# loli/medpy

Hardware: NVIDIA H100
Metric: Mvoxels/sec to min-cut (higher is better)
Workload: dtype f64

## Files before the change

### include/medpy_b200_graphcut.h

```cpp
#ifndef MEDPY_B200_GRAPHCUT_H
#define MEDPY_B200_GRAPHCUT_H

#include <stddef.h>
#include <stdint.h>

#ifdef __cplusplus
extern "C" {
#endif

#define MGC_ABI_VERSION 3
#define MGC_MAX_NDIM 4

#define MGC_OK 0
#define MGC_E_ARG (-1)
#define MGC_E_CUDA (-2)
#define MGC_E_NOMEM (-3)
#define MGC_E_STATE (-4)
#define MGC_E_WEIGHT (-5)
#define MGC_E_NOCONV (-6)
#define MGC_E_LABELS (-7)

#define MGC_F32 0
#define MGC_F64 1
#define MGC_U8 2
#define MGC_I16 3
#define MGC_I32 4

#define MGC_MEM_HOST 0
#define MGC_MEM_DEVICE 1

#define MGC_BOUNDARY_DIFFERENCE_LINEAR 0
#define MGC_BOUNDARY_DIFFERENCE_EXPONENTIAL 1
#define MGC_BOUNDARY_DIFFERENCE_DIVISION 2
#define MGC_BOUNDARY_DIFFERENCE_POWER 3
#define MGC_BOUNDARY_MAXIMUM_LINEAR 4
#define MGC_BOUNDARY_MAXIMUM_EXPONENTIAL 5
#define MGC_BOUNDARY_MAXIMUM_DIVISION 6
#define MGC_BOUNDARY_MAXIMUM_POWER 7

#define MGC_SOURCE 0
#define MGC_SINK 1

typedef struct mgc_graph mgc_graph;

typedef struct mgc_array {
    const void* data;
    int32_t dtype;
    int32_t mem;
    int64_t strides[MGC_MAX_NDIM];
} mgc_array;

typedef struct mgc_stats {
    int64_t n_voxels;
    int64_t push_sweeps;
    int64_t global_relabels;
    int64_t relabel_sweeps;
    int64_t kernel_launches;
    int64_t active_last;
    double ms_terms;
    double ms_solve;
    double ms_readout;
    double flow_const;
    double energy;
    int64_t device_bytes;
    double ms_push;
    double ms_relabel;
    double ms_boundary;
    double ms_init;
    int64_t tiles_materialised;
    double ms_caps;
    int64_t seed_folds;
    double ms_seeds;
    double ms_seeds_host;
    int64_t tiles_deferred;
    int64_t tiles_dropped;
    int64_t relabel_passes;
    double ms_relabel_first;
    int64_t relabel_passes_first;
    int64_t build_blocks_refused;
} mgc_stats;


int mgc_create(int32_t ndim, const int64_t* shape, int32_t device, mgc_graph** out);
int mgc_create_slab(int32_t ndim, const int64_t* shape, int64_t z0, int64_t z1, int32_t device, mgc_graph** out);
void mgc_destroy(mgc_graph* g);
int mgc_reset(mgc_graph* g);
const char* mgc_last_error(const mgc_graph* g);
int mgc_abi_version(void);
int mgc_host_alloc(size_t bytes, void** out);
void mgc_host_free(void* p);
int mgc_trim_pools(void);
#define MGC_OPT_DEFER_WEIGHT_CHECK 1
#define MGC_OPT_WARM 2
#define MGC_OPT_KEEP_DEVICE_INPUTS 3
int mgc_set_option(mgc_graph* g, int32_t option, int64_t value);
int mgc_check(mgc_graph* g);
int mgc_set_stream(mgc_graph* g, void* cuda_stream);
int mgc_synchronize(mgc_graph* g);


int mgc_add_regional_probability(mgc_graph* g, const mgc_array* prob, double alpha, int32_t compute_dtype);
int mgc_add_tweights_dense(mgc_graph* g, const mgc_array* src, const mgc_array* snk);
int mgc_add_markers(mgc_graph* g, const mgc_array* fg, const mgc_array* bg);


int mgc_add_boundary(mgc_graph* g, int32_t kind, const mgc_array* image, double sigma,
                     const double* spacing, double norm);
int mgc_add_nweights_dense(mgc_graph* g, int32_t axis, const mgc_array* fwd, const mgc_array* bwd);


typedef struct mgc_voxel_terms {
    const mgc_array* prob;
    double alpha;
    int32_t compute_dtype;
    int32_t boundary_kind;
    const mgc_array* image;
    double sigma;
    const double* spacing;
    double norm;
    const mgc_array* fg;
    const mgc_array* bg;
    const uint32_t* fg_bits;
    const uint32_t* bg_bits;
    int32_t bits_mem;
    const volatile int64_t* bits_ready_words;
} mgc_voxel_terms;
int mgc_build_voxel_graph(mgc_graph* g, const mgc_voxel_terms* terms);
int mgc_can_fuse(const mgc_graph* g);


int mgc_maxflow(mgc_graph* g, double* energy);
int mgc_add_seeds(mgc_graph* g, const int64_t* fg_ids, int64_t n_fg, const int64_t* bg_ids, int64_t n_bg, int32_t mem);
int mgc_remove_seeds(mgc_graph* g, const int64_t* fg_ids, int64_t n_fg, const int64_t* bg_ids, int64_t n_bg, int32_t mem);
int mgc_add_tweights_warm(mgc_graph* g, const int64_t* ids, const double* src, const double* snk, int64_t count, int32_t mem);
int mgc_add_nweights_warm(mgc_graph* g, const int64_t* i, const int64_t* j, const double* cap, const double* rev_cap,
                          int64_t count, int32_t mem);
int mgc_add_nweights_dense_warm(mgc_graph* g, int32_t axis, const mgc_array* fwd, const mgc_array* bwd);
int mgc_remove_nweights_warm(mgc_graph* g, const int64_t* i, const int64_t* j, const double* cap, const double* rev_cap,
                             int64_t count, int32_t mem);
int mgc_remove_nweights_dense_warm(mgc_graph* g, int32_t axis, const mgc_array* fwd, const mgc_array* bwd);
int mgc_get_mask(mgc_graph* g, uint8_t* out, int32_t mem);
int mgc_what_segment(mgc_graph* g, int64_t node, int32_t* segment);
int mgc_get_edge(mgc_graph* g, int64_t i, int64_t j, double* cap);
int mgc_get_trcap(mgc_graph* g, int64_t node, double* trcap);
int mgc_get_node_num(const mgc_graph* g, int64_t* n);
int mgc_get_arc_num(const mgc_graph* g, int64_t* n);
int mgc_get_stats(const mgc_graph* g, mgc_stats* out);


int mgc_gradient_magnitude_prewitt(int32_t ndim, const int64_t* shape, const mgc_array* image, float* out,
                                   int32_t out_mem, int32_t device);


int mgc_slab_plane_elems(const mgc_graph* g, int64_t* n);
int mgc_slab_begin(mgc_graph* g);
int mgc_slab_push(mgc_graph* g, int32_t n);
int mgc_slab_pack(mgc_graph* g, int32_t* h_lo, double* f_lo, int32_t* h_hi, double* f_hi);
int mgc_slab_unpack(mgc_graph* g, const int32_t* h_lo, const double* f_lo, const int32_t* h_hi, const double* f_hi,
                    int32_t* changed_dev);
int mgc_slab_relabel_begin(mgc_graph* g);
int mgc_slab_relabel_relax(mgc_graph* g, int32_t* changed_out);
int mgc_slab_count_active(mgc_graph* g, int64_t* active_out);
// ... 54 lines not shown
```

### medpy_b200/csrc/gc_api.cu

```cuda
#include "gc_handle.cuh"
#include "gc_api_kernels.cuh"
#include "gc_gradient.cuh"

#include <cmath>
#include <cstring>
#include <map>
#include <mutex>
#include <string>
#include <type_traits>
#include <vector>

thread_local std::string g_create_error;

namespace {
std::mutex g_pool_mu;
std::map<std::pair<int, size_t>, std::vector<void*>> g_pool;

size_t round_up(size_t b) { const size_t g = size_t(1) << 21; return (b + g - 1) / g * g; }

cudaError_t pool_alloc(int dev, size_t bytes, void** out)
{
    bytes = round_up(bytes);
    {
        std::lock_guard<std::mutex> lk(g_pool_mu);
        auto it = g_pool.find({dev, bytes});
        if (it != g_pool.end() && !it->second.empty()) {
            *out = it->second.back();
            it->second.pop_back();
            return cudaSuccess;
        }
    }
    cudaError_t e = cudaMalloc(out, bytes);
    if (e != cudaSuccess) {
        std::lock_guard<std::mutex> lk(g_pool_mu);
        for (auto& kv : g_pool) if (kv.first.first == dev) { for (void* p : kv.second) cudaFree(p); kv.second.clear(); }
        cudaGetLastError();
        e = cudaMalloc(out, bytes);
    }
    return e;
}

void pool_free(int dev, size_t bytes, void* p)
{
    if (!p) return;
    std::lock_guard<std::mutex> lk(g_pool_mu);
    g_pool[{dev, round_up(bytes)}].push_back(p);
}

std::map<size_t, std::vector<void*>> g_host_pool;
std::map<void*, size_t> g_host_live;

}

size_t dtype_size(int dt)
{
    switch (dt) {
        case MGC_F32: return 4;
        case MGC_F64: return 8;
        case MGC_U8: return 1;
        case MGC_I16: return 2;
        case MGC_I32: return 4;
        default: return 0;
    }
}

int alloc_buf(mgc_graph* g, size_t bytes, void** out)
{
    void* p = nullptr;
    cudaError_t e = pool_alloc(g->device, bytes, &p);
    if (e != cudaSuccess) {
        cudaGetLastError();
        g->err = std::string("device allocation of ") + std::to_string(bytes) + " bytes failed: " + cudaGetErrorString(e);
        return MGC_E_NOMEM;
    }
    g->owned_bufs.push_back({p, bytes});
    g->device_bytes += (int64_t)round_up(bytes);
    *out = p;
    return MGC_OK;
}

int ensure_scratch(mgc_graph* g, Buf& b, size_t bytes)
{
    if (b.bytes >= bytes) return MGC_OK;
    if (b.p) {
        if (g->stream) cudaStreamSynchronize(g->stream);
        if (g->up_stream) cudaStreamSynchronize(g->up_stream);
        pool_free(g->device, b.bytes, b.p);
        g->device_bytes -= (int64_t)round_up(b.bytes);
    }
    b.p = nullptr; b.bytes = 0;
    void* p = nullptr;
    cudaError_t e = pool_alloc(g->device, bytes, &p);
    if (e != cudaSuccess) { cudaGetLastError(); g->err = "scratch allocation failed"; return MGC_E_NOMEM; }
    b.p = p; b.bytes = bytes;
    g->device_bytes += (int64_t)round_up(bytes);
    return MGC_OK;
}

namespace {
template <typename E>
int gather_launch(mgc_graph* g, const char* src, const Strides4& st, E* dst)
{
    const int Z = g->L.dim[0], Y = g->L.dim[1], X = g->L.dim[2];
    if (g->nd == 3 && Z > 1 && X > 1 && Y <= 65535 && (Z + 31) / 32 <= 65535 &&
        st.s[0] == (long long)sizeof(E) && (Y == 1 || st.s[1] == (long long)sizeof(E) * Z) && st.s[2] == (long long)sizeof(E) * Z * Y) {
        const dim3 grid((unsigned)((X + 31) / 32), (unsigned)Y, (unsigned)((Z + 31) / 32));
        k_gather_fortran3<E><<<grid, 256, 0, g->stream>>>(Z, Y, X, reinterpret_cast<const E*>(src), dst);
        g->st.kernel_launches++;
        return MGC_OK;
    }
    if (g->nd == 3) k_gather<E, 3><<<nblocks(g), 256, 0, g->stream>>>(g->L, src, st, dst);
    else            k_gather<E, 4><<<nblocks(g), 256, 0, g->stream>>>(g->L, src, st, dst);
    g->st.kernel_launches++;
    return MGC_OK;
}
}

int upload(mgc_graph* g, void* dst, const void* src, size_t bytes, int slot)
{
    if (g->slot_used[slot]) CK(cudaStreamWaitEvent(g->up_stream, g->ev_slot[slot], 0));
    CK(cudaMemcpyAsync(dst, src, bytes, cudaMemcpyHostToDevice, g->up_stream));
    CK(cudaEventRecord(g->ev_up, g->up_stream));
    CK(cudaStreamWaitEvent(g->stream, g->ev_up, 0));
    CK(cudaEventSynchronize(g->ev_up));
    return MGC_OK;
}

void slots_release(mgc_graph* g, unsigned mask)
{
    for (int i = 0; i < 5; ++i)
        if (mask & (1u << i)) { cudaEventRecord(g->ev_slot[i], g->stream); g->slot_used[i] = true; }
}

int stage_input(mgc_graph* g, const mgc_array* a, int slot, const void** out)
{
    const size_t es = dtype_size(a->dtype);
    if (!es) FAIL(MGC_E_ARG, "unsupported dtype");
    if (!a->data) FAIL(MGC_E_ARG, "null array");
    Strides4 st{};
    bool contiguous = true;
    long long span = (long long)es;
    long long expect = (long long)es;
    for (int d = g->nd - 1; d >= 0; --d) {
        long long s = 0;
        int ud = d - g->shift;
        if (ud >= 0) s = (long long)a->strides[ud];
        if (g->L.dim[d] > 1) {
            if (s <= 0) FAIL(MGC_E_ARG, "array strides must be positive (pass a contiguous copy)");
            if (s != expect) contiguous = false;
            span += (long long)(g->L.dim[d] - 1) * s;
        } else {
            s = 0;
        }
        st.s[d] = s;
        expect *= g->L.dim[d];
    }
    const size_t bytes = (size_t)g->L.n * es;
    if (contiguous && a->mem == MGC_MEM_DEVICE) { *out = a->data; return MGC_OK; }
    int rc = ensure_scratch(g, g->scratch[slot], bytes);
    if (rc) return rc;
    if (contiguous) {
        rc = upload(g, g->scratch[slot].p, a->data, bytes, slot);
        if (rc) return rc;
        *out = g->scratch[slot].p;
        return MGC_OK;
    }
    const char* src = (const char*)a->data;
    if (a->mem == MGC_MEM_HOST) {
        rc = ensure_scratch(g, g->raw, (size_t)span);
        if (rc) return rc;
        rc = upload(g, g->raw.p, a->data, (size_t)span, 3);
        if (rc) return rc;
        src = (const char*)g->raw.p;
    }
    else if (g->slot_used[slot]) CK(cudaStreamWaitEvent(g->stream, g->ev_slot[slot], 0));
    switch (a->dtype) {
        case MGC_F32: gather_launch<float>(g, src, st, (float*)g->scratch[slot].p); break;
        case MGC_F64: gather_launch<double>(g, src, st, (double*)g->scratch[slot].p); break;
        case MGC_U8: gather_launch<uint8_t>(g, src, st, (uint8_t*)g->scratch[slot].p); break;
        case MGC_I16: gather_launch<int16_t>(g, src, st, (int16_t*)g->scratch[slot].p); break;
        case MGC_I32: gather_launch<int32_t>(g, src, st, (int32_t*)g->scratch[slot].p); break;
    }
    CK(cudaGetLastError());
    if (a->mem == MGC_MEM_HOST) { CK(cudaEventRecord(g->ev_slot[3], g->stream)); g->slot_used[3] = true; }
    *out = g->scratch[slot].p;
    return MGC_OK;
}

void sum_partials(mgc_graph* g, const double* partials, unsigned n, double* out)
{
    k_sum_partials<<<1, 256, 0, g->stream>>>(partials, n, out);
}

namespace {
int finish_flow_const(mgc_graph* g)
{
    sum_partials(g, g->partials, rblocks(g), g->d_scalars);
    g->st.kernel_launches++;
    CK(cudaGetLastError());
    return MGC_OK;
}

void invalidate(mgc_graph* g)
{
    g->lazy_built = false;
    g->caps_img = nullptr;
    g->caps_tin.prob = nullptr;
    g->state_init = false;
    g->warm_state = false;
    g->solved = false;
    g->host_mask_valid = false;
}
}

void resolve_term_span(mgc_graph* g)
{
    if (!g->terms_open) return;
    if (cudaEventSynchronize(g->ev_terms[1]) == cudaSuccess) {
        float ms = 0;
        if (cudaEventElapsedTime(&ms, g->ev_terms[0], g->ev_terms[1]) == cudaSuccess) g->st.ms_terms += ms;
        if (g->boundary_timed && cudaEventElapsedTime(&ms, g->ev_b[0], g->ev_b[1]) == cudaSuccess) g->st.ms_boundary = ms;
        g->boundary_timed = false;
    }
    g->terms_open = false;
}

int check_pending(mgc_graph* g)
{
    if (!g->bad_pending) return MGC_OK;
    g->bad_pending = false;
    CK(cudaEventSynchronize(g->ev_bad));
    if (*g->h_bad) FAIL(MGC_E_WEIGHT, "Negative or zero weights are not allowed.");
    return MGC_OK;
}

namespace {
int create_impl(int32_t ndim, const int64_t* shape, int64_t z0, int64_t z1, bool slab, int32_t device, mgc_graph** out)
{
    if (!out) return MGC_E_ARG;
    *out = nullptr;
    if (ndim < 1 || ndim > MGC_MAX_NDIM || !shape) { g_create_error = "ndim must be 1..4"; return MGC_E_ARG; }
    int ndev = 0;
    cudaError_t e = cudaGetDeviceCount(&ndev);
    if (e != cudaSuccess || ndev == 0) {
        cudaGetLastError();
        g_create_error = std::string("no usable CUDA device (this library has no CPU path): ") + cudaGetErrorString(e);
        return MGC_E_CUDA;
    }
    if (device < 0) cudaGetDevice(&device);
    if (device >= ndev) { g_create_error = "bad device ordinal"; return MGC_E_ARG; }
    e = cudaSetDevice(device);
    if (e != cudaSuccess) { g_create_error = cudaGetErrorString(e); return MGC_E_CUDA; }

    mgc_graph* g = new mgc_graph();
    g->device = device;
    g->user_ndim = ndim;
    g->nd = ndim == 4 ? 4 : 3;
    g->shift = g->nd - ndim;
    for (int d = 0; d < ndim; ++d) {
        if (shape[d] < 1) { g_create_error = "extents must be >= 1"; delete g; return MGC_E_ARG; }
        g->user_shape[d] = shape[d];
    }
    int64_t dims[4] = {1, 1, 1, 1};
    for (int d = 0; d < ndim; ++d) dims[d + g->shift] = shape[d];
    g->slab = slab;
    int own0 = 0, own1 = (int)dims[0];
    if (slab) {
        if (g->shift != 0 || z0 < 0 || z1 > shape[0] || z0 >= z1) { g_create_error = "bad slab"; delete g; return MGC_E_ARG; }
        g->global_dim0 = shape[0]; g->z0 = z0; g->z1 = z1;
        g->ghost_lo = z0 > 0; g->ghost_hi = z1 < shape[0];
        dims[0] = (z1 - z0) + (g->ghost_lo ? 1 : 0) + (g->ghost_hi ? 1 : 0);
        own0 = g->ghost_lo ? 1 : 0;
        own1 = own0 + (int)(z1 - z0);
    }
    int64_t n = 1;
    for (int d = 0; d < g->nd; ++d) n *= dims[d];
    if (n >= (int64_t(1) << 31)) { g_create_error = "lattice too large for one device handle (>= 2^31 voxels)"; delete g; return MGC_E_ARG; }
    g->L.nd = g->nd;
    unsigned s = (unsigned)n;
    for (int d = 0; d < 4; ++d) { g->L.dim[d] = 1; g->L.stride[d] = 1; }
    for (int d = 0; d < g->nd; ++d) { g->L.dim[d] = (int)dims[d]; s /= (unsigned)dims[d]; g->L.stride[d] = s; }
    for (int d = 0; d < 4; ++d) {
        const unsigned long long st = g->L.stride[d];
        g->L.magic[d] = st <= 1 ? 0ull : (~0ull / st) + 1ull;
    }
    g->L.n = (unsigned)n;
    g->L.plane = g->L.stride[0];
    g->L.own0 = own0; g->L.own1 = own1;

    int rc = MGC_OK;
    const size_t nb = (size_t)n;
    void* p = nullptr;
    for (int k = 0; k < 2 * g->nd && !rc; ++k) { rc = alloc_buf(g, nb * sizeof(double), &p); g->S.cap[k] = (double*)p; }
    if (!rc) { rc = alloc_buf(g, nb * sizeof(double), &p); g->S.excess = (double*)p; }
    if (!rc) { rc = alloc_buf(g, nb * sizeof(double), &p); g->S.sink = (double*)p; }
    if (!rc) { rc = alloc_buf(g, nb * sizeof(double), &p); g->S.tr = (double*)p; }
    if (!rc) { rc = alloc_buf(g, nb * sizeof(int), &p); g->S.height = (int*)p; }
    if (!rc) { rc = alloc_buf(g, nb, &p); g->S.rmask = (uint8_t*)p; }
    if (!rc) { rc = alloc_buf(g, nb, &p); g->mask_dev = (uint8_t*)p; }
    g->n_partials = nblocks(g);
    if (g->nd == 3) {
        const unsigned nbuild = (unsigned)((g->L.dim[0] + 7) / 8) * (unsigned)((g->L.dim[1] + 7) / 8) * (unsigned)((g->L.dim[2] + 31) / 32);
        if (nbuild > g->n_partials) g->n_partials = nbuild;
        if (!rc) { rc = alloc_buf(g, (size_t)nbuild * sizeof(int), &p); g->build_refused = (int*)p; }
    }
    if (!rc) { rc = alloc_buf(g, (size_t)g->n_partials * sizeof(double), &p); g->partials = (double*)p; }
    if (!rc) { rc = alloc_buf(g, 3 * 1024 * sizeof(double), &p); g->minmax_buf = p; }
    if (!rc) { rc = alloc_buf(g, 64, &p); g->d_scalars = (double*)p; }
    if (!rc) { rc = alloc_buf(g, 64, &p); g->d_flags = (int*)p; }
    if (!rc) { rc = alloc_buf(g, 64, &p); g->d_count = (unsigned long long*)p; }
    if (!rc && g->nd == 3) {
        for (int d = 0; d < 3; ++d) g->TL.nt[d] = (g->L.dim[d] + TILE - 1) / TILE;
        g->TL.ntiles = g->TL.nt[0] * g->TL.nt[1] * g->TL.nt[2];
        const size_t tb = (size_t)g->TL.ntiles * sizeof(int);
// ... 45 lines not shown
    for (auto& ev : g->ev_chunk) cudaEventCreateWithFlags(&ev, cudaEventDisableTiming);
    for (auto& ev : g->ev_terms) cudaEventCreate(&ev);
    if (const char* f0 = getenv("MEDPY_GC_DEBUG")) g->debug_checks = atoi(f0) != 0;
    if (const char* f3 = getenv("MEDPY_GC_FIRST_TEST")) g->skip_first_test = atoi(f3) == 0;
    if (const char* f5 = getenv("MEDPY_GC_FIRST_CAP")) g->first_cap = atoi(f5) >= 2 ? atoi(f5) : 0;
    if (const char* f1 = getenv("MEDPY_GC_FUSE")) g->fuse_build = atoi(f1) != 0;
    if (const char* f4 = getenv("MEDPY_GC_LAZY_CAPS")) g->lazy_caps = atoi(f4) != 0;
    if (const char* f2 = getenv("MEDPY_GC_CHUNKS")) if (atoi(f2) > 0) g->build_chunks = atoi(f2);
    cudaEventCreateWithFlags(&g->ev_bad, cudaEventDisableTiming);
    for (auto& ev : g->ev_b) cudaEventCreate(&ev);
    { void* hp = nullptr; g->h_bad = (mgc_host_alloc(64, &hp) == MGC_OK) ? (int*)hp : nullptr; }
    g->st.n_voxels = (int64_t)n;
    rc = mgc_reset(g);
    if (rc) { g_create_error = g->err; mgc_destroy(g); return rc; }
    *out = g;
    return MGC_OK;
}

template <typename E, int ND, bool FRESH>
void boundary_launch_nd(mgc_graph* g, const E* img, const BoundaryParams& P)
{
    const dim3 grid(nblocks(g)), block(256);
    if (P.fn == 1 && P.inv_spacing_on == 0.0 && (sizeof(E) == 4 || sizeof(E) == 8) && !std::is_integral<E>::value) {
        if (P.use_max) k_boundary<E, ND, double, FRESH, 1, 1, 0><<<grid, block, 0, g->stream>>>(g->L, g->S, img, P, g->d_flags);
        else           k_boundary<E, ND, double, FRESH, 1, 0, 0><<<grid, block, 0, g->stream>>>(g->L, g->S, img, P, g->d_flags);
        return;
    }
    k_boundary<E, ND, double, FRESH><<<grid, block, 0, g->stream>>>(g->L, g->S, img, P, g->d_flags);
}

template <typename E>
int boundary_launch(mgc_graph* g, const E* img, const BoundaryParams& P)
{
    if (g->caps_fresh) {
        if (g->nd == 3) boundary_launch_nd<E, 3, true>(g, img, P);
        else            boundary_launch_nd<E, 4, true>(g, img, P);
    } else {
        if (g->nd == 3) boundary_launch_nd<E, 3, false>(g, img, P);
        else            boundary_launch_nd<E, 4, false>(g, img, P);
    }
    g->caps_fresh = false;
    g->st.kernel_launches++;
    return MGC_OK;
}

template <typename E>
int minmax_launch(mgc_graph* g, const E* img)
{
    unsigned nb = g->n_partials < 1024u ? g->n_partials : 1024u;
    E* pm = (E*)g->minmax_buf;
    E* px = pm + 1024;
    E* pa = px + 1024;
    k_minmax_partial<E><<<nb, 256, 0, g->stream>>>(img, g->L.n, pm, px, pa);
    k_minmax_final<E><<<1, 32, 0, g->stream>>>(pm, px, pa, nb, g->d_scalars + 2);
    g->st.kernel_launches += 2;
    return MGC_OK;
}
}

int boundary_params(mgc_graph* g, int kind, int dtype, const void* img, double sigma, const double* spacing, double norm, BoundaryParams* out)
{
    BoundaryParams P{};
    P.fn = kind & 3;
    P.use_max = (kind >= 4 && kind != MGC_BOUNDARY_MAXIMUM_DIVISION) ? 1 : 0;
    P.sigma = (P.fn == 1) ? pow(sigma, 2) : sigma;
    P.inv_sigma2 = (P.fn == 1 && P.sigma != 0.0) ? 1.0 / P.sigma : 0.0;
    P.inv_spacing_on = spacing ? 1.0 : 0.0;
    for (int d = 0; d < 4; ++d) P.spacing[d] = 1.0;
    if (spacing) for (int d = 0; d < g->user_ndim; ++d) P.spacing[d + g->shift] = spacing[d];
    P.norm = norm;
    if (P.fn == 0 && std::isnan(norm)) {
        if (g->slab) FAIL(MGC_E_ARG, "z-slab handles need the global normaliser of the linear terms");
        int rc = MGC_OK;
        switch (dtype) {
            case MGC_F32: rc = minmax_launch<float>(g, (const float*)img); break;
            case MGC_F64: rc = minmax_launch<double>(g, (const double*)img); break;
            case MGC_U8: rc = minmax_launch<uint8_t>(g, (const uint8_t*)img); break;
            case MGC_I16: rc = minmax_launch<int16_t>(g, (const int16_t*)img); break;
            case MGC_I32: rc = minmax_launch<int32_t>(g, (const int32_t*)img); break;
        }
        if (rc) return rc;
        double mm[2];
        CK(cudaMemcpyAsync(mm, g->d_scalars + 2, sizeof(mm), cudaMemcpyDeviceToHost, g->stream));
        CK(cudaStreamSynchronize(g->stream));
        P.norm = (kind == MGC_BOUNDARY_MAXIMUM_LINEAR) ? mm[1] : mm[0];
    }
    *out = P;
    return MGC_OK;
}

template <typename E, int ND>
static cudaError_t gradient_launch(const int64_t* shape, const E* img, float* out, long long n)
{
    GradCtx<ND> G;
    long long st = 1;
    for (int d = ND - 1; d >= 0; --d) { G.dim[d] = (int)shape[d]; G.stride[d] = st; st *= shape[d]; }
    k_gradient_magnitude<E, ND><<<(unsigned)((n + 255) / 256), 256>>>(G, n, img, out);
    return cudaGetLastError();
}

template <typename E>
static cudaError_t gradient_dispatch(int nd, const int64_t* shape, const E* img, float* out, long long n)
{
    switch (nd) {
        case 1: return gradient_launch<E, 1>(shape, img, out, n);
        case 2: return gradient_launch<E, 2>(shape, img, out, n);
        case 3: return gradient_launch<E, 3>(shape, img, out, n);
        default: return gradient_launch<E, 4>(shape, img, out, n);
    }
}

extern "C" {

int mgc_abi_version(void) { return MGC_ABI_VERSION; }

const char* mgc_last_error(const mgc_graph* g) { return g ? g->err.c_str() : g_create_error.c_str(); }

int mgc_create(int32_t ndim, const int64_t* shape, int32_t device, mgc_graph** out)
{
    return create_impl(ndim, shape, 0, 0, false, device, out);
}

int mgc_create_slab(int32_t ndim, const int64_t* shape, int64_t z0, int64_t z1, int32_t device, mgc_graph** out)
{
    if (ndim < 3) { g_create_error = "z-slab handles need ndim >= 3"; return MGC_E_ARG; }
    return create_impl(ndim, shape, z0, z1, true, device, out);
}

void mgc_destroy(mgc_graph* g)
{
    if (!g) return;
    cudaSetDevice(g->device);
    if (g->stream) cudaStreamSynchronize(g->stream);
    for (auto& b : g->owned_bufs) pool_free(g->device, b.bytes, b.p);
    for (auto& b : g->scratch) if (b.p) pool_free(g->device, b.bytes, b.p);
    if (g->raw.p) pool_free(g->device, g->raw.bytes, g->raw.p);
    if (g->img_copy.p) pool_free(g->device, g->img_copy.bytes, g->img_copy.p);
    if (g->prob_copy.p) pool_free(g->device, g->prob_copy.bytes, g->prob_copy.p);
    for (auto& b : g->mark_planes) if (b.p) pool_free(g->device, b.bytes, b.p);
    if (g->fold_buf.p) pool_free(g->device, g->fold_buf.bytes, g->fold_buf.p);
    for (auto& ev : g->ev_fold) if (ev) cudaEventDestroy(ev);
    for (auto& ev : g->ev) if (ev) cudaEventDestroy(ev);
    for (auto& ev : g->caps_ev) if (ev) cudaEventDestroy(ev);
    for (auto& ev : g->ev_slot) if (ev) cudaEventDestroy(ev);
    for (auto& ev : g->ev_terms) if (ev) cudaEventDestroy(ev);
    for (auto& ev : g->ev_chunk) if (ev) cudaEventDestroy(ev);
    if (g->ev_up) cudaEventDestroy(g->ev_up);
    if (g->ev_bad) cudaEventDestroy(g->ev_bad);
    for (auto& ev : g->ev_b) if (ev) cudaEventDestroy(ev);
    for (auto& ev : g->ph_events) if (ev) cudaEventDestroy(ev);
    if (g->h_bad) mgc_host_free(g->h_bad);
    if (g->h_stat) mgc_host_free(g->h_stat);
    slab_comm_release(g);
    if (g->up_stream) { cudaStreamSynchronize(g->up_stream); cudaStreamDestroy(g->up_stream); }
    if (g->own_stream && g->stream) cudaStreamDestroy(g->stream);
    delete g;
}

int mgc_reset(mgc_graph* g)
{
    if (!g) return MGC_E_ARG;
    CK(cudaSetDevice(g->device));
    g->caps_fresh = true;
    g->tr_fresh = true;
    g->caps_lazy = false;
    CK(cudaMemsetAsync(g->d_scalars, 0, 64, g->stream));
    CK(cudaMemsetAsync(g->d_flags, 0, 64, g->stream));
    invalidate(g);
    g->flow_started = false;
    g->has_nlinks = false;
    g->energy = 0.0;
    int64_t n = g->st.n_voxels;
    g->st = mgc_stats{};
    g->st.n_voxels = n;
    g->terms_open = false;
    g->bad_pending = false;
    return MGC_OK;
}

int mgc_gradient_magnitude_prewitt(int32_t ndim, const int64_t* shape, const mgc_array* image, float* out,
                                   int32_t out_mem, int32_t device)
{
    if (ndim < 1 || ndim > 4 || !shape || !image || !image->data || !out) { g_create_error = "bad arguments"; return MGC_E_ARG; }
    const size_t es = dtype_size(image->dtype);
    if (!es) { g_create_error = "unsupported dtype"; return MGC_E_ARG; }
    int ndev = 0;
    if (cudaGetDeviceCount(&ndev) != cudaSuccess || ndev == 0) {
        cudaGetLastError();
        g_create_error = "no usable CUDA device (this library has no CPU path)";
        return MGC_E_CUDA;
    }
    if (device < 0) cudaGetDevice(&device);
    cudaSetDevice(device);
    long long n = 1;
    bool contiguous = true;
    long long expect = (long long)es;
    for (int d = ndim - 1; d >= 0; --d) {
        if (shape[d] < 1) { g_create_error = "extents must be >= 1"; return MGC_E_ARG; }
        if (shape[d] > 1 && image->strides[d] != expect) contiguous = false;
        expect *= shape[d];
        n *= shape[d];
    }
    if (!contiguous) { g_create_error = "gradient input must be C-contiguous (the host layer copies otherwise)"; return MGC_E_ARG; }
    void* d_in = nullptr;
    void* d_out = nullptr;
    const size_t in_bytes = (size_t)n * es, out_bytes = (size_t)n * sizeof(float);
    cudaError_t e = cudaSuccess;
    if (image->mem == MGC_MEM_HOST) {
        if ((e = pool_alloc(device, in_bytes, &d_in)) != cudaSuccess) { cudaGetLastError(); g_create_error = "device allocation failed"; return MGC_E_NOMEM; }
        e = cudaMemcpy(d_in, image->data, in_bytes, cudaMemcpyHostToDevice);
    }
    const void* src = image->mem == MGC_MEM_HOST ? d_in : image->data;
    float* dst = out;
    if (e == cudaSuccess && out_mem == MGC_MEM_HOST) {
        if ((e = pool_alloc(device, out_bytes, &d_out)) == cudaSuccess) dst = (float*)d_out;
    }
    if (e == cudaSuccess) {
        switch (image->dtype) {
            case MGC_F32: e = gradient_dispatch<float>(ndim, shape, (const float*)src, dst, n); break;
            case MGC_F64: e = gradient_dispatch<double>(ndim, shape, (const double*)src, dst, n); break;
            case MGC_U8: e = gradient_dispatch<uint8_t>(ndim, shape, (const uint8_t*)src, dst, n); break;
            case MGC_I16: e = gradient_dispatch<int16_t>(ndim, shape, (const int16_t*)src, dst, n); break;
            default: e = gradient_dispatch<int32_t>(ndim, shape, (const int32_t*)src, dst, n); break;
        }
    }
    if (e == cudaSuccess && out_mem == MGC_MEM_HOST) e = cudaMemcpy(out, d_out, out_bytes, cudaMemcpyDeviceToHost);
    if (e == cudaSuccess) e = cudaDeviceSynchronize();
    if (d_in) pool_free(device, in_bytes, d_in);
    if (d_out) pool_free(device, out_bytes, d_out);
    if (e != cudaSuccess) { cudaGetLastError(); g_create_error = std::string("gradient kernel failed: ") + cudaGetErrorString(e); return MGC_E_CUDA; }
    return MGC_OK;
}

int mgc_host_alloc(size_t bytes, void** out)
{
    if (!out || !bytes) return MGC_E_ARG;
    const size_t rb = round_up(bytes);
    std::lock_guard<std::mutex> lk(g_pool_mu);
    auto it = g_host_pool.find(rb);
    void* p = nullptr;
    if (it != g_host_pool.end() && !it->second.empty()) { p = it->second.back(); it->second.pop_back(); }
    else if (cudaHostAlloc(&p, rb, cudaHostAllocDefault) != cudaSuccess) { cudaGetLastError(); g_create_error = "pinned host allocation failed"; return MGC_E_NOMEM; }
    g_host_live[p] = rb;
    *out = p;
    return MGC_OK;
}

void mgc_host_free(void* p)
{
    if (!p) return;
    std::lock_guard<std::mutex> lk(g_pool_mu);
    auto it = g_host_live.find(p);
    if (it == g_host_live.end()) return;
    g_host_pool[it->second].push_back(p);
    g_host_live.erase(it);
}

int mgc_trim_pools(void)
{
    std::lock_guard<std::mutex> lk(g_pool_mu);
    int cur = 0;
    cudaGetDevice(&cur);
    for (auto& kv : g_pool) {
        if (kv.second.empty()) continue;
        cudaSetDevice(kv.first.first);
        for (void* p : kv.second) cudaFree(p);
        kv.second.clear();
    }
    cudaSetDevice(cur);
    for (auto& kv : g_host_pool) { for (void* p : kv.second) cudaFreeHost(p); kv.second.clear(); }
    cudaGetLastError();
    return MGC_OK;
}

int mgc_set_option(mgc_graph* g, int32_t option, int64_t value)
{
    if (!g) return MGC_E_ARG;
    if (option == MGC_OPT_DEFER_WEIGHT_CHECK) { g->defer_check = value != 0; return MGC_OK; }
    if (option == MGC_OPT_KEEP_DEVICE_INPUTS) { g->keep_device_inputs = value != 0; return MGC_OK; }
    if (option == MGC_OPT_WARM) {
        const bool on = value != 0;
        if (on != g->warm_opt && g->flow_started && !g->lazy_built)
            FAIL(MGC_E_STATE, "MGC_OPT_WARM is set before the first solve (the residual source capacities are recorded at "
                              "its start): reset() the handle and rebuild the graph to change it");
        g->warm_opt = on;
        return MGC_OK;
    }
    FAIL(MGC_E_ARG, "unknown option");
}

int mgc_check(mgc_graph* g)
{
    if (!g) return MGC_E_ARG;
    return check_pending(g);
}

int mgc_set_stream(mgc_graph* g, void* cuda_stream)
{
    if (!g) return MGC_E_ARG;
    CK(cudaStreamSynchronize(g->stream));
    if (g->own_stream) { cudaStreamDestroy(g->stream); g->own_stream = false; }
    g->stream = (cudaStream_t)cuda_stream;
    return MGC_OK;
}

int mgc_synchronize(mgc_graph* g)
{
    if (!g) return MGC_E_ARG;
    CK(cudaStreamSynchronize(g->stream));
    return MGC_OK;
}

int mgc_add_regional_probability(mgc_graph* g, const mgc_array* prob, double alpha, int32_t compute_dtype)
{
    if (!g || !prob) return MGC_E_ARG;
    if (g->flow_started) FAIL(MGC_E_STATE, "the graph has been solved (its capacities hold residuals): reset() it before adding terms");
    if (prob->dtype != MGC_F32 && prob->dtype != MGC_F64) FAIL(MGC_E_ARG, "probability map must be float32 or float64");
    if (compute_dtype != MGC_F32 && compute_dtype != MGC_F64) FAIL(MGC_E_ARG, "compute dtype must be float32 or float64");
    CK(cudaSetDevice(g->device));
    { int rc0 = push_state_all(g); if (rc0) return rc0; }
    TermSpan t(g);
    const void* p = nullptr;
    int rc = stage_input(g, prob, 0, &p);
    if (rc) return rc;
    rc = check_pending(g);
    if (rc) return rc;
    if (prob->dtype == MGC_F32 && (g->L.n % 4u) == 0u && ((uintptr_t)p % 16u) == 0u)
        k_regional_f32x4<double><<<rblocks(g), 256, 0, g->stream>>>(g->L, g->S, (const float4*)p, alpha, compute_dtype == MGC_F32, g->tr_fresh ? 1 : 0, g->partials);
    else if (prob->dtype == MGC_F32)
        k_regional<float, double><<<rblocks(g), 256, 0, g->stream>>>(g->L, g->S, (const float*)p, alpha, compute_dtype == MGC_F32, g->tr_fresh ? 1 : 0, g->partials);
    else
        k_regional<double, double><<<rblocks(g), 256, 0, g->stream>>>(g->L, g->S, (const double*)p, alpha, 0, g->tr_fresh ? 1 : 0, g->partials);
    g->tr_fresh = false;
    g->st.kernel_launches++;
    CK(cudaGetLastError());
    rc = finish_flow_const(g);
    if (rc) return rc;
    invalidate(g);
    t.stop(1u);
    return MGC_OK;
}

int mgc_add_tweights_dense(mgc_graph* g, const mgc_array* src, const mgc_array* snk)
{
    if (!g || !src || !snk) return MGC_E_ARG;
    if (g->flow_started) FAIL(MGC_E_STATE, "the graph has been solved (its capacities hold residuals): reset() it before adding terms");
    if (src->dtype != MGC_F64 || snk->dtype != MGC_F64) FAIL(MGC_E_ARG, "dense t-weights must be float64");
    CK(cudaSetDevice(g->device));
    { int rc0 = push_state_all(g); if (rc0) return rc0; }
    TermSpan t(g);
    const void *ps = nullptr, *pk = nullptr;
    int rc = stage_input(g, src, 0, &ps);
    if (rc) return rc;
    rc = stage_input(g, snk, 1, &pk);
    if (rc) return rc;
    rc = check_pending(g);
    if (rc) return rc;
    k_tweights_dense<double><<<rblocks(g), 256, 0, g->stream>>>(g->L, g->S, (const double*)ps, (const double*)pk, g->tr_fresh ? 1 : 0, g->partials);
    g->tr_fresh = false;
    g->st.kernel_launches++;
    CK(cudaGetLastError());
    rc = finish_flow_const(g);
    if (rc) return rc;
    invalidate(g);
    t.stop(3u);
    return MGC_OK;
}

int mgc_add_markers(mgc_graph* g, const mgc_array* fg, const mgc_array* bg)
{
    if (!g) return MGC_E_ARG;
    if (!fg && !bg) return MGC_OK;
    if (g->flow_started) FAIL(MGC_E_STATE, "the graph has been solved (its capacities hold residuals): reset() it before adding terms");
    if ((fg && fg->dtype != MGC_U8) || (bg && bg->dtype != MGC_U8)) FAIL(MGC_E_ARG, "markers must be uint8 / bool");
    CK(cudaSetDevice(g->device));
    { int rc0 = push_state_all(g); if (rc0) return rc0; }
    TermSpan t(g);
    const void *pf = nullptr, *pb = nullptr;
    int rc = MGC_OK;
    if (fg) { rc = stage_input(g, fg, 1, &pf); if (rc) return rc; }
    if (bg) { rc = stage_input(g, bg, 4, &pb); if (rc) return rc; }
    rc = check_pending(g);
    if (rc) return rc;
    const bool vec16 = !g->tr_fresh && (g->L.n % 16u) == 0u && ((uintptr_t)pf % 16u) == 0u && ((uintptr_t)pb % 16u) == 0u;
    if (vec16)
        k_markers16<double><<<rblocks(g), 256, 0, g->stream>>>(g->L, g->S, (const uint4*)pf, (const uint4*)pb, g->partials);
    else
        k_markers<double><<<rblocks(g), 256, 0, g->stream>>>(g->L, g->S, (const uint8_t*)pf, (const uint8_t*)pb, g->tr_fresh ? 1 : 0, g->partials);
    g->tr_fresh = false;
    g->st.kernel_launches++;
    CK(cudaGetLastError());
    rc = finish_flow_const(g);
    if (rc) return rc;
    invalidate(g);
    t.stop(0x12u);
    return MGC_OK;
}

int mgc_add_boundary(mgc_graph* g, int32_t kind, const mgc_array* image, double sigma, const double* spacing, double norm)
{
    if (!g || !image) return MGC_E_ARG;
    if (kind < 0 || kind > 7) FAIL(MGC_E_ARG, "unknown boundary term");
    if (g->flow_started) FAIL(MGC_E_STATE, "the graph has been solved (its capacities hold residuals): reset() it before adding terms");
    CK(cudaSetDevice(g->device));
    { int rc0 = check_pending(g); if (rc0) return rc0; }
    { int rc0 = push_state_all(g); if (rc0) return rc0; }
    TermSpan t(g);
    const void* img = nullptr;
    int rc = stage_input(g, image, 2, &img);
    if (rc) return rc;
    BoundaryParams P{};
    rc = boundary_params(g, kind, image->dtype, img, sigma, spacing, norm, &P);
    if (rc) return rc;
    CK(cudaMemsetAsync(g->d_flags, 0, sizeof(int), g->stream));
    cudaEventRecord(g->ev_b[0], g->stream);
    switch (image->dtype) {
        case MGC_F32: boundary_launch<float>(g, (const float*)img, P); break;
        case MGC_F64: boundary_launch<double>(g, (const double*)img, P); break;
        case MGC_U8: boundary_launch<uint8_t>(g, (const uint8_t*)img, P); break;
        case MGC_I16: boundary_launch<int16_t>(g, (const int16_t*)img, P); break;
        case MGC_I32: boundary_launch<int32_t>(g, (const int32_t*)img, P); break;
    }
    cudaEventRecord(g->ev_b[1], g->stream);
    CK(cudaGetLastError());
    invalidate(g);
    g->has_nlinks = true;
    g->boundary_timed = true;
    if (g->defer_check && g->h_bad && image->mem == MGC_MEM_HOST) {
        CK(cudaMemcpyAsync(g->h_bad, g->d_flags, sizeof(int), cudaMemcpyDeviceToHost, g->stream));
        CK(cudaEventRecord(g->ev_bad, g->stream));
        g->bad_pending = true;
        t.stop(4u);
        return MGC_OK;
    }
    int bad = 0;
    CK(cudaMemcpyAsync(&bad, g->d_flags, sizeof(int), cudaMemcpyDeviceToHost, g->stream));
    t.stop(4u);
    CK(cudaStreamSynchronize(g->stream));
    if (bad) FAIL(MGC_E_WEIGHT, "Negative or zero weights are not allowed.");
    return MGC_OK;
}

int mgc_add_nweights_dense(mgc_graph* g, int32_t axis, const mgc_array* fwd, const mgc_array* bwd)
{
    if (!g || !fwd || !bwd) return MGC_E_ARG;
    if (g->flow_started) FAIL(MGC_E_STATE, "the graph has been solved (its capacities hold residuals): reset() it before adding terms");
    if (axis < 0 || axis >= g->user_ndim) FAIL(MGC_E_ARG, "bad axis");
    if (fwd->dtype != MGC_F64 || bwd->dtype != MGC_F64) FAIL(MGC_E_ARG, "dense n-weights must be float64");
    CK(cudaSetDevice(g->device));
    { int rc0 = check_pending(g); if (rc0) return rc0; }
    { int rc0 = push_state_all(g); if (rc0) return rc0; }
    TermSpan t(g);
    const void *pf = nullptr, *pb = nullptr;
    int rc = stage_input(g, fwd, 0, &pf);
    if (rc) return rc;
    rc = stage_input(g, bwd, 1, &pb);
    if (rc) return rc;
    if (g->caps_fresh) {
        const size_t nbz = (size_t)g->L.n;
        for (int k = 0; k < 2 * g->nd; ++k) CK(cudaMemsetAsync(g->S.cap[k], 0, nbz * sizeof(double), g->stream));
        g->caps_fresh = false;
    }
    CK(cudaMemsetAsync(g->d_flags, 0, sizeof(int), g->stream));
    const int ca = axis + g->shift;
    if (g->nd == 3) k_nweights_dense<3, double><<<nblocks(g), 256, 0, g->stream>>>(g->L, g->S, ca, (const double*)pf, (const double*)pb, g->d_flags);
    else            k_nweights_dense<4, double><<<nblocks(g), 256, 0, g->stream>>>(g->L, g->S, ca, (const double*)pf, (const double*)pb, g->d_flags);
    g->st.kernel_launches++;
    CK(cudaGetLastError());
    int bad = 0;
    CK(cudaMemcpyAsync(&bad, g->d_flags, sizeof(int), cudaMemcpyDeviceToHost, g->stream));
    t.stop(3u);
    CK(cudaStreamSynchronize(g->stream));
    invalidate(g);
    g->has_nlinks = true;
    if (bad) FAIL(MGC_E_WEIGHT, "Negative or zero weights are not allowed.");
    return MGC_OK;
}

int mgc_get_mask(mgc_graph* g, uint8_t* out, int32_t mem)
{
    if (!g || !out) return MGC_E_ARG;
    if (!g->solved) FAIL(MGC_E_STATE, "call maxflow first");
    CK(cudaSetDevice(g->device));
    const size_t owned_n = (size_t)(g->L.own1 - g->L.own0) * g->L.plane;
    const uint8_t* src = g->mask_dev + (size_t)g->L.own0 * g->L.plane;
    CK(cudaMemcpyAsync(out, src, owned_n, mem == MGC_MEM_DEVICE ? cudaMemcpyDeviceToDevice : cudaMemcpyDeviceToHost, g->stream));
    CK(cudaStreamSynchronize(g->stream));
    return MGC_OK;
}

int mgc_what_segment(mgc_graph* g, int64_t node, int32_t* segment)
{
    if (!g || !segment) return MGC_E_ARG;
    if (!g->solved) FAIL(MGC_E_STATE, "call maxflow first");
    if (node < 0 || node >= (int64_t)g->L.n) FAIL(MGC_E_ARG, "node id out of range");
    if (!g->host_mask_valid) {
        g->host_mask.resize(g->L.n);
        CK(cudaMemcpyAsync(g->host_mask.data(), g->mask_dev, g->L.n, cudaMemcpyDeviceToHost, g->stream));
        CK(cudaStreamSynchronize(g->stream));
        g->host_mask_valid = true;
    }
    *segment = g->host_mask[(size_t)node] ? MGC_SOURCE : MGC_SINK;
    return MGC_OK;
}

int mgc_get_edge(mgc_graph* g, int64_t i, int64_t j, double* cap)
{
    if (!g || !cap) return MGC_E_ARG;
    const int64_t n = (int64_t)g->L.n;
    if (i < 0 || j < 0 || i >= n || j >= n || i == j) FAIL(MGC_E_ARG, "bad node ids");
    *cap = 0.0;
    if (g->caps_fresh) return MGC_OK;
    CK(cudaSetDevice(g->device));
    { int rc0 = push_state_all(g); if (rc0) return rc0; }
    int c[4] = {0, 0, 0, 0};
    unsigned r = (unsigned)i;
    for (int d = 0; d < g->nd; ++d) { c[d] = (int)(r / g->L.stride[d]); r %= g->L.stride[d]; }
    for (int k = 0; k < 2 * g->nd; ++k) {
        const int d = k >> 1;
        const int64_t off = (k & 1) ? (int64_t)g->L.stride[d] : -(int64_t)g->L.stride[d];
        const int cn = c[d] + ((k & 1) ? 1 : -1);
        if (cn < 0 || cn >= g->L.dim[d]) continue;
        if (i + off == j) {
            CK(cudaMemcpyAsync(cap, g->S.cap[k] + i, sizeof(double), cudaMemcpyDeviceToHost, g->stream));
            CK(cudaStreamSynchronize(g->stream));
            caps_resolve(g);
            return MGC_OK;
        }
    }
    return MGC_OK;
}

int mgc_get_trcap(mgc_graph* g, int64_t node, double* trcap)
{
    if (!g || !trcap) return MGC_E_ARG;
    if (node < 0 || node >= (int64_t)g->L.n) FAIL(MGC_E_ARG, "node id out of range");
    if (g->tr_fresh) { *trcap = 0.0; return MGC_OK; }
    CK(cudaSetDevice(g->device));
    { int rc0 = push_state_all(g); if (rc0) return rc0; }
    if (!g->state_init || !g->flow_started) {
        CK(cudaMemcpyAsync(trcap, g->S.tr + node, sizeof(double), cudaMemcpyDeviceToHost, g->stream));
        CK(cudaStreamSynchronize(g->stream));
        return MGC_OK;
    }
    double e = 0, s = 0;
    uint8_t rm = 0x80u;
    CK(cudaMemcpyAsync(&e, g->S.excess + node, sizeof(double), cudaMemcpyDeviceToHost, g->stream));
    CK(cudaMemcpyAsync(&s, g->S.sink + node, sizeof(double), cudaMemcpyDeviceToHost, g->stream));
    if (g->nd == 3) CK(cudaMemcpyAsync(&rm, g->S.rmask + node, 1, cudaMemcpyDeviceToHost, g->stream));
    CK(cudaStreamSynchronize(g->stream));
    if (!(rm & 0x80u)) s = 0;
    double tr = 0;
    CK(cudaMemcpyAsync(&tr, g->S.tr + node, sizeof(double), cudaMemcpyDeviceToHost, g->stream));
    CK(cudaStreamSynchronize(g->stream));
    *trcap = (tr < 0 && -tr - s > 0) ? -(-tr - s) : e;
    return MGC_OK;
}

int mgc_get_node_num(const mgc_graph* g, int64_t* n)
{
    if (!g || !n) return MGC_E_ARG;
    *n = (int64_t)g->L.n;
    return MGC_OK;
}

int mgc_get_arc_num(const mgc_graph* g, int64_t* n)
{
    if (!g || !n) return MGC_E_ARG;
    int64_t e = 0;
    if (g->has_nlinks)
        for (int d = 0; d < g->nd; ++d)
            if (g->L.dim[d] > 1) e += ((int64_t)g->L.n / g->L.dim[d]) * (g->L.dim[d] - 1);
    *n = 2 * e;
    return MGC_OK;
}

int mgc_get_stats(const mgc_graph* g, mgc_stats* out)
{
    if (!g || !out) return MGC_E_ARG;
    *out = g->st;
    out->device_bytes = g->device_bytes;
    return MGC_OK;
}

}
```

### medpy_b200/csrc/gc_build.cuh

```cuda
#pragma once
#include <climits>
#include <type_traits>
#include "gc_terms.cuh"
#include "gc_tiles.cuh"
#include "gc_tma.cuh"

#define BUILD_TZ 8
#define BUILD_TY 8
#define BUILD_TX 32
#define BUILD_THREADS 256
#define BUILD_TIN_OFFSET(img_pad) ((((img_pad) + (2 * 9 * 32 + 2 * 8 * 33 + 8 * 32 + 8 * 8) * 8 + 8 + 32 + 64) + 127) / 128 * 128)
template <typename E> struct BuildBox {
    static constexpr int PAD = 16 / (int)sizeof(E);
    static constexpr int BX = (PAD + 33 + PAD - 1) / PAD * PAD;
};
#define BUILD_HY 10
#define BUILD_HZ 10

struct BuildMaps {
    CUtensorMap img, prob, fg, bg;
};

struct BuildArgs {
    const void* img;
// ... 695 lines not shown
        const int lx = tid & 31, ly = tid >> 5;
        const bool col_in = y0 + ly < L.dim[1] && x0 + lx < L.dim[2];
        double msum = 0.0;
#pragma unroll
        for (int lz = 0; lz < BUILD_TZ; ++lz) {
            const int cz2 = z0 + lz;
            if (col_in && cz2 < L.dim[0] && cz2 >= L.own0 && cz2 < L.own1)
                msum = __dadd_rn(msum, s_mm[(lz * BUILD_TY + ly) * BUILD_TX + (lx ^ ly)]);
        }
#pragma unroll
        for (int o = 16; o > 0; o >>= 1) msum = __dadd_rn(msum, __shfl_down_sync(0xffffffffu, msum, o));
        double* s_red = reinterpret_cast<double*>(s_scr);
        if (lx == 0) s_red[ly] = msum;
        __syncthreads();
        if (tid == 0) {
            double t = s_red[0];
#pragma unroll
            for (int w = 1; w < 8; ++w) t = __dadd_rn(t, s_red[w]);
            partials[((A.z_tile0 + (int)blockIdx.z) * (int)gridDim.y + (int)blockIdx.y) * (int)gridDim.x + (int)blockIdx.x] = t;
        }
    }
    if (tid < 4) {
        const int tx = (x0 >> 3) + tid, tyy = y0 >> 3, tzz = z0 >> 3;
        if (tx < TL.nt[2] && tyy < TL.nt[1] && tzz < TL.nt[0]) {
            const int t = (tzz * TL.nt[1] + tyy) * TL.nt[2] + tx;
            const int any_needs = s_flags[tid], any_exc = s_flags[4 + tid];
            rflag[t] = any_needs;
            if (any_needs) rl.items[atomicAdd(rl.count, 1)] = t;
            pflag[t] = any_exc;
            A.cmat[t] = 0;
            if (any_exc) {
                const WorkList& pl = ((tzz + tyy + tx) & 1) ? pl1 : pl0;
                pl.items[atomicAdd(pl.count, 1)] = t;
            }
        }
    }
}

__device__ __forceinline__ unsigned tile_pairs(const Lattice& L, const TileCtx& c)
{
    const int gz = c.tz * TILE + c.lz, gy = c.ty * TILE + c.ly, gx = c.tx * TILE + c.lx;
    return (gz > 0 ? 1u : 0u) | (gz + 1 < L.dim[0] ? 2u : 0u) | (gy > 0 ? 4u : 0u) | (gy + 1 < L.dim[1] ? 8u : 0u) |
           (gx > 0 ? 16u : 0u) | (gx + 1 < L.dim[2] ? 32u : 0u);
}

__device__ __forceinline__ void lazy_tin_load(const Lattice& L, const LazyTin& tin, const TileCtx& c, double& p, unsigned& fb)
{
    const int gz = c.tz * TILE + c.lz, gy = c.ty * TILE + c.ly, gx = c.tx * TILE + c.lx;
    if (tin.prob) p = tin.prob_f64 ? reinterpret_cast<const double*>(tin.prob)[c.v] : (double)reinterpret_cast<const float*>(tin.prob)[c.v];
    const unsigned w = ((unsigned)gz * (unsigned)L.dim[1] + (unsigned)gy) * (unsigned)tin.words + ((unsigned)gx >> 5);
    if (tin.fg) fb |= (tin.fg[w] >> (gx & 31)) & 1u;
    if (tin.bg) fb |= ((tin.bg[w] >> (gx & 31)) & 1u) << 1;
}

__device__ __forceinline__ double lazy_tr(const LazyTin& tin, double p, unsigned fb)
{
    double tr = 0.0;
    tlink_replay<double>(tr, tin.prob != nullptr, p, tin.compute_f32 != 0, tin.alpha, fb);
    return tr;
}

__device__ __forceinline__ bool lazy_has_excess(const Lattice& L, const LazyTin& tin, const TileCtx& c)
{
    double p = 0.0;
    unsigned fb = 0u;
    lazy_tin_load(L, tin, c, p, fb);
    return source_active(lazy_tr(tin, p, fb), tile_pairs(L, c));
}

template <typename T>
__device__ __forceinline__ bool voxel_active(const Lattice& L, const State<T>& S, const LazyTin& tin, const TileCtx& c, int h, bool mat)
{
    if (!c.own || h >= MGC_HINF) return false;
    return mat ? S.excess[c.v] > 0 : lazy_has_excess(L, tin, c);
}

#define PUSH_WINDOW 8
#define FIRST_RELABEL_CAP 12
#define WIN_GMIN 0
#define WIN_NOW 1
#define WIN_DEFERRED 2
#define WIN_DROPPED 3
#define WIN_NDROP 4
```

### medpy_b200/csrc/gc_build_api.cu

```cuda
#include "gc_handle.cuh"

#include <atomic>
#include <cmath>
#include <cstdlib>
#include <thread>
#include <type_traits>
#include <utility>

namespace {
bool make_image_map(mgc_graph* g, const void* img, int dtype, CUtensorMap* out)
{
    tmap_encode_fn encode = tensor_map_encoder();
    if (!encode) return false;
    const size_t es = dtype_size(dtype);
    const cuuint64_t X = (cuuint64_t)g->L.dim[2], Y = (cuuint64_t)g->L.dim[1], Z = (cuuint64_t)g->L.dim[0];
    if ((X * es) % 16 || ((uintptr_t)img & 15)) return false;
    CUtensorMapDataType dt;
    switch (dtype) {
        case MGC_F32: dt = CU_TENSOR_MAP_DATA_TYPE_FLOAT32; break;
        case MGC_F64: dt = CU_TENSOR_MAP_DATA_TYPE_FLOAT64; break;
        case MGC_U8: dt = CU_TENSOR_MAP_DATA_TYPE_UINT8; break;
        case MGC_I16: dt = CU_TENSOR_MAP_DATA_TYPE_UINT16; break;
        default: dt = CU_TENSOR_MAP_DATA_TYPE_INT32; break;
    }
// ... 175 lines not shown
                   !(( t->boundary_kind & 3) == 0 && std::isnan(t->norm));
    if (t->prob) chunked = chunked && t->prob->mem == MGC_MEM_HOST && c_contiguous(g, t->prob);
    if (t->fg) chunked = chunked && t->fg->mem == MGC_MEM_HOST && c_contiguous(g, t->fg);
    if (t->bg) chunked = chunked && t->bg->mem == MGC_MEM_HOST && c_contiguous(g, t->bg);
    if (has_bits) chunked = chunked && t->bits_mem == MGC_MEM_HOST;

    const void *d_img = nullptr, *d_prob = nullptr, *d_fg = nullptr, *d_bg = nullptr;
    int rc = MGC_OK;
    if (!chunked) {
        rc = stage_input(g, t->image, 2, &d_img); if (rc) return rc;
        if (t->prob) { rc = stage_input(g, t->prob, 0, &d_prob); if (rc) return rc; }
        if (t->fg) { rc = stage_input(g, t->fg, 1, &d_fg); if (rc) return rc; }
        if (t->bg) { rc = stage_input(g, t->bg, 4, &d_bg); if (rc) return rc; }
        if (has_bits) {
            if (t->bits_ready_words && t->bits_mem == MGC_MEM_HOST) {
                while (*t->bits_ready_words < (int64_t)words) std::this_thread::yield();
                std::atomic_thread_fence(std::memory_order_acquire);
            }
            const uint32_t* src[2] = {t->fg_bits, t->bg_bits};
            const void** dst[2] = {&d_fg, &d_bg};
            const int slot[2] = {1, 4};
            for (int i = 0; i < 2; ++i) {
                if (!src[i]) continue;
                if (t->bits_mem == MGC_MEM_DEVICE) { *dst[i] = src[i]; continue; }
                rc = ensure_scratch(g, g->scratch[slot[i]], words * 4); if (rc) return rc;
                rc = upload(g, g->scratch[slot[i]].p, src[i], words * 4, slot[i]); if (rc) return rc;
                *dst[i] = g->scratch[slot[i]].p;
            }
        }
    } else {
        rc = ensure_scratch(g, g->scratch[2], n * es_img); if (rc) return rc;
        if (t->prob) { rc = ensure_scratch(g, g->scratch[0], n * es_prob); if (rc) return rc; }
        if (t->fg || t->fg_bits) { rc = ensure_scratch(g, g->scratch[1], has_bits ? words * 4 : n); if (rc) return rc; }
        if (t->bg || t->bg_bits) { rc = ensure_scratch(g, g->scratch[4], has_bits ? words * 4 : n); if (rc) return rc; }
        d_img = g->scratch[2].p;
        if (t->prob) d_prob = g->scratch[0].p;
        if (t->fg || t->fg_bits) d_fg = g->scratch[1].p;
        if (t->bg || t->bg_bits) d_bg = g->scratch[4].p;
        const int slots[4] = {0, 1, 2, 4};
        for (int i = 0; i < 4; ++i) if (g->slot_used[slots[i]]) CK(cudaStreamWaitEvent(g->up_stream, g->ev_slot[slots[i]], 0));
    }

    BoundaryParams P{};
    rc = boundary_params(g, t->boundary_kind, t->image->dtype, d_img, t->sigma, t->spacing, t->norm, &P);
    if (rc) return rc;

    BuildArgs A{};
    A.img = d_img;
    A.prob = d_prob;
    A.prob_f64 = (t->prob && t->prob->dtype == MGC_F64) ? 1 : 0;
    A.compute_f32 = (t->prob && t->compute_dtype == MGC_F32) ? 1 : 0;
    A.alpha = t->alpha;
    if (has_bits) { A.fg_bits = (const unsigned*)d_fg; A.bg_bits = (const unsigned*)d_bg; }
    else { A.fg = (const uint8_t*)d_fg; A.bg = (const uint8_t*)d_bg; }
    BuildMaps imap{};
    A.use_tma = make_image_map(g, d_img, t->image->dtype, &imap.img) ? 1 : 0;
    if (const char* e = getenv("MEDPY_GC_BUILD_TMA")) if (atoi(e) == 0) A.use_tma = 0;
    int tin_tma = A.use_tma;
    if (const char* e = getenv("MEDPY_GC_BUILD_TMA")) if (atoi(e) == 2) tin_tma = 0;
    if (tin_tma) {
        if (d_prob && make_block_map(g, d_prob, t->prob->dtype, &imap.prob)) A.tma_prob = 1;
        if (!has_bits) {
            if (d_fg && make_block_map(g, d_fg, MGC_U8, &imap.fg)) A.tma_mark |= 1;
            if (d_bg && make_block_map(g, d_bg, MGC_U8, &imap.bg)) A.tma_mark |= 2;
        }
    }
    if (const char* e = getenv("MEDPY_GC_BUILD_DBG")) A.dbg = atoi(e);
    const bool lazy = can_lazy(g);
    const int mark_words = (g->L.dim[2] + 31) / 32;
    enum { COPIED, STAGED, BORROWED };
    auto source_of = [&](const mgc_array* a, const void* d, int slot) {
        if (d == g->scratch[slot].p) return STAGED;
        return (g->keep_device_inputs && a->mem == MGC_MEM_DEVICE && d == a->data) ? BORROWED : COPIED;
    };
    const int img_src = lazy ? source_of(t->image, d_img, 2) : COPIED;
    const int prob_src = (lazy && t->prob && !(A.dbg & 1)) ? source_of(t->prob, d_prob, 0) : COPIED;
    if (lazy) {
        if (img_src == COPIED) { rc = ensure_scratch(g, g->img_copy, n * es_img); if (rc) return rc; A.img_copy = g->img_copy.p; }
        if (t->prob && prob_src == COPIED) { rc = ensure_scratch(g, g->prob_copy, n * es_prob); if (rc) return rc; A.prob_copy = g->prob_copy.p; }
        const size_t plane_bytes = (size_t)g->L.dim[0] * (size_t)g->L.dim[1] * (size_t)mark_words * 4;
        if (t->fg || t->fg_bits) { rc = ensure_scratch(g, g->mark_planes[0], plane_bytes); if (rc) return rc; A.fg_plane = (unsigned*)g->mark_planes[0].p; }
        if (t->bg || t->bg_bits) { rc = ensure_scratch(g, g->mark_planes[1], plane_bytes); if (rc) return rc; A.bg_plane = (unsigned*)g->mark_planes[1].p; }
        A.cmat = g->cmat;
        CK(cudaMemsetAsync(g->d_flags + 3, 0, sizeof(int), g->stream));
        CK(cudaMemsetAsync(g->win_ctl + WIN_NDROP, 0, sizeof(int), g->stream));
    }

    CK(cudaMemsetAsync(g->d_tcount, 0, 256, g->stream));
    CK(cudaMemsetAsync(g->d_flags, 0, sizeof(int), g->stream));
    CK(cudaMemsetAsync(g->d_flags + 7, 0, sizeof(int), g->stream));
    { int rcd = dirty_clear(g); if (rcd) return rcd; }
    g->pl_sel[0] = g->pl_sel[1] = 0;
    cudaEventRecord(g->ev_b[0], g->stream);
    if (!chunked) {
        A.z_tile0 = 0;
        rc = build_launch_any(g, lazy, t->image->dtype, imap, A, P, nzt);
        if (rc) return rc;
    } else {
        int nchunks = g->build_chunks < nzt ? g->build_chunks : nzt;
        const int per = (nzt + nchunks - 1) / nchunks;
        nchunks = (nzt + per - 1) / per;
        const char* h_img = (const char*)t->image->data;
        int prev_l0 = 0, prev_nl = 0;
        for (int c = 0; c < nchunks; ++c) {
            const int l0 = c * per, l1 = (l0 + per < nzt) ? l0 + per : nzt;
            const size_t z0 = (size_t)l0 * BUILD_TZ, z1 = ((size_t)l1 * BUILD_TZ < (size_t)Z) ? (size_t)l1 * BUILD_TZ : (size_t)Z;
            const size_t v0 = z0 * plane, nv = (z1 - z0) * plane;
            CK(cudaMemcpyAsync((char*)g->scratch[2].p + v0 * es_img, h_img + v0 * es_img, nv * es_img, cudaMemcpyHostToDevice, g->up_stream));
            if (c > 0) {
                CK(cudaEventRecord(g->ev_chunk[c & 1], g->up_stream));
                CK(cudaStreamWaitEvent(g->stream, g->ev_chunk[c & 1], 0));
                A.z_tile0 = prev_l0;
                rc = build_launch_any(g, lazy, t->image->dtype, imap, A, P, prev_nl);
                if (rc) { cudaStreamSynchronize(g->up_stream); return rc; }
            }
            if (t->prob) CK(cudaMemcpyAsync((char*)g->scratch[0].p + v0 * es_prob, (const char*)t->prob->data + v0 * es_prob, nv * es_prob, cudaMemcpyHostToDevice, g->up_stream));
            if (has_bits) {
                const size_t w0 = v0 / 32, w1 = (v0 + nv + 31) / 32;
                if (t->bits_ready_words) {
                    const int64_t need = (int64_t)(w1 < words ? w1 : words);
                    while (*t->bits_ready_words < need) std::this_thread::yield();
                    std::atomic_thread_fence(std::memory_order_acquire);
                }
                if (t->fg_bits) CK(cudaMemcpyAsync((uint32_t*)g->scratch[1].p + w0, t->fg_bits + w0, (w1 - w0) * 4, cudaMemcpyHostToDevice, g->up_stream));
                if (t->bg_bits) CK(cudaMemcpyAsync((uint32_t*)g->scratch[4].p + w0, t->bg_bits + w0, (w1 - w0) * 4, cudaMemcpyHostToDevice, g->up_stream));
            } else {
                if (t->fg) CK(cudaMemcpyAsync((char*)g->scratch[1].p + v0, (const char*)t->fg->data + v0, nv, cudaMemcpyHostToDevice, g->up_stream));
                if (t->bg) CK(cudaMemcpyAsync((char*)g->scratch[4].p + v0, (const char*)t->bg->data + v0, nv, cudaMemcpyHostToDevice, g->up_stream));
            }
            prev_l0 = l0; prev_nl = l1 - l0;
        }
        CK(cudaEventRecord(g->ev_up, g->up_stream));
        CK(cudaStreamWaitEvent(g->stream, g->ev_up, 0));
        A.z_tile0 = prev_l0;
        rc = build_launch_any(g, lazy, t->image->dtype, imap, A, P, prev_nl);
        if (rc) { cudaStreamSynchronize(g->up_stream); return rc; }
        CK(cudaEventSynchronize(g->ev_up));
    }
    cudaEventRecord(g->ev_b[1], g->stream);
    {
        const unsigned nbuild = (unsigned)nzt * (unsigned)((g->L.dim[1] + BUILD_TY - 1) / BUILD_TY) * (unsigned)((g->L.dim[2] + BUILD_TX - 1) / BUILD_TX);
        sum_partials(g, g->partials, nbuild, g->d_scalars);
        g->st.kernel_launches++;
        CK(cudaGetLastError());
    }
    g->caps_fresh = false;
    g->tr_fresh = false;
    g->caps_lazy = lazy;
    g->lazy_built = lazy;
    g->warm_state = false;
    g->st.seed_folds = 0;
    g->st.ms_seeds = 0.0;
    g->st.ms_seeds_host = 0.0;
    g->caps_dtype = t->image->dtype;
    g->caps_P = P;
    if (img_src == STAGED) std::swap(g->scratch[2], g->img_copy);
    if (prob_src == STAGED) std::swap(g->scratch[0], g->prob_copy);
    g->caps_img = !lazy ? nullptr : (img_src == BORROWED ? d_img : g->img_copy.p);
    const void* caps_prob = !(lazy && t->prob) ? nullptr : (prob_src == BORROWED ? d_prob : g->prob_copy.p);
    g->caps_tin = LazyTin{caps_prob, A.prob_f64, A.compute_f32, A.alpha, A.fg_plane, A.bg_plane, mark_words};
    g->has_nlinks = true;
    g->boundary_timed = true;
    g->state_init = true;
    g->solved = false;
    g->host_mask_valid = false;
    g->labels_fresh = true;
    g->sweep_mode = -1;
    g->init_timed = false;
    g->st.ms_init = 0.0;
    span.stop(0x17u);
    if (g->defer_check && g->h_bad) {
        CK(cudaMemcpyAsync(g->h_bad, g->d_flags, sizeof(int), cudaMemcpyDeviceToHost, g->stream));
        CK(cudaEventRecord(g->ev_bad, g->stream));
        g->bad_pending = true;
        return MGC_OK;
    }
    int bad = 0;
    CK(cudaMemcpyAsync(&bad, g->d_flags, sizeof(int), cudaMemcpyDeviceToHost, g->stream));
    CK(cudaStreamSynchronize(g->stream));
    if (bad) FAIL(MGC_E_WEIGHT, "Negative or zero weights are not allowed.");
    return MGC_OK;
}

}
```

### medpy_b200/csrc/gc_fold.cu

```cuda
#include "gc_handle.cuh"
#include "gc_nlinks_remove.cuh"

#include <cub/cub.cuh>

#include <algorithm>
#include <chrono>
#include <functional>
#include <map>
#include <mutex>
#include <tuple>
#include <type_traits>
#include <vector>

int warm_prepare(mgc_graph* g)
{
    if (!warm_wanted(g) || g->warm_state) return MGC_OK;
    if (g->flow_started) FAIL(MGC_E_STATE, "MGC_OPT_WARM was set after the first solve: reset() the graph and rebuild it");
    if (!g->state_init || g->nd == 4) {
        int rc = materialise_zeros(g);
        if (rc) return rc;
        return init_tiles(g);
    }
    Nvtx range("mgc:warm_convert");
    unsigned grid = nblocks(g);
// ... 37 lines not shown
    if (sort == FOLD_SORT_PAIRS) e = cub::DeviceRadixSort::SortPairs(tmp, tb, keys, skeys, vals, svals, n, 0, end_bit, s);
    if (!tmp && sort != FOLD_SCAN) *bytes = tb;
    return e;
}

static cudaError_t fold_scan(void* tmp, size_t* bytes, int* head, int* pos, int n, cudaStream_t s)
{
    size_t tb = *bytes;
    const cudaError_t e = cub::DeviceScan::InclusiveSum(tmp, tb, head, pos, n, s);
    if (!tmp) *bytes = std::max(*bytes, tb);
    return e;
}

static int cub_launches(mgc_graph* g, const std::tuple<int, int, int, int, int>& key,
                        const std::function<cudaError_t(cudaStream_t)>& enqueue, int* out)
{
    static std::mutex mu;
    static std::map<int, cudaStream_t> streams;
    static std::map<std::tuple<int, int, int, int, int>, int> counts;
    std::lock_guard<std::mutex> lock(mu);
    auto it = counts.find(key);
    if (it != counts.end()) { *out = it->second; return MGC_OK; }
    cudaStream_t& s = streams[g->device];
    if (!s) CK(cudaStreamCreateWithFlags(&s, cudaStreamNonBlocking));
    cudaGraph_t graph = nullptr;
    cudaError_t e = cudaStreamBeginCapture(s, cudaStreamCaptureModeRelaxed);
    if (e == cudaSuccess) {
        const cudaError_t e2 = enqueue(s);
        e = cudaStreamEndCapture(s, &graph);
        if (e == cudaSuccess) e = e2;
    }
    size_t nn = 0;
    std::vector<cudaGraphNode_t> nodes;
    if (e == cudaSuccess) e = cudaGraphGetNodes(graph, nullptr, &nn);
    if (e == cudaSuccess) { nodes.resize(nn); e = cudaGraphGetNodes(graph, nodes.data(), &nn); }
    int k = 0;
    for (size_t i = 0; e == cudaSuccess && i < nn; ++i) {
        cudaGraphNodeType t;
        e = cudaGraphNodeGetType(nodes[i], &t);
        if (e == cudaSuccess && t == cudaGraphNodeTypeKernel) ++k;
    }
    if (graph) cudaGraphDestroy(graph);
    CK(e);
    if (counts.size() > 4096) counts.clear();
    counts[key] = k;
    *out = k;
    return MGC_OK;
}

template <typename Key>
static int fold_cub_launches(mgc_graph* g, int sort, int n, int end_bit, void* tmp, size_t tmp_bytes, Key* keys, Key* skeys,
                             int* vals, int* svals, int* head, int* pos, int* out)
{
    return cub_launches(g, std::make_tuple(g->device, sort, (int)sizeof(Key), n, end_bit), [&](cudaStream_t s) {
        size_t tb = tmp_bytes;
        const cudaError_t e1 = fold_sort(sort, tmp, &tb, keys, skeys, vals, svals, n, end_bit, s);
        tb = tmp_bytes;
        return e1 == cudaSuccess ? fold_scan(tmp, &tb, head, pos, n, s) : e1;
    }, out);
}

static cudaError_t tails_sort(void* tmp, size_t* bytes, const unsigned* tails, unsigned* stails, int count, int end_bit,
                              cudaStream_t s)
{
    return cub::DeviceRadixSort::SortKeys(tmp, *bytes, tails, stails, count, 0, end_bit, s);
}

static int warm_check(mgc_graph* g, bool* eager)
{
    *eager = false;
    if (!g->slab && g->lazy_built && g->state_init && g->nd == 3) return MGC_OK;
    if (warm_wanted(g)) { *eager = true; return MGC_OK; }
    FAIL(MGC_E_STATE, "a warm re-solve needs a lazily built 3-D handle (mgc_build_voxel_graph on a 1-D..3-D lattice with a "
                      "boundary term, tile solver, lazy capacities); on this handle reset() it and rebuild the graph with "
                      "the seeds instead");
}

static int fold_items(mgc_graph* g, int* d_ctl, int* tiles, const std::function<int(unsigned, int)>& fold,
                      const char* nonfinite, const char* negative, const std::function<int()>* check)
{
    CK(cudaEventRecord(g->ev_fold[1], g->stream));
    int h_ctl[2] = {0, 0};
    CK(cudaMemcpyAsync(h_ctl, d_ctl, sizeof(h_ctl), cudaMemcpyDeviceToHost, g->stream));
    CK(cudaStreamSynchronize(g->stream));
    if (h_ctl[1] & FOLD_ERR_RANGE) FAIL(MGC_E_ARG, "node id out of range");
    if (h_ctl[1] & FOLD_ERR_PAIR) FAIL(MGC_E_ARG, "node ids are not lattice neighbours");
    if (h_ctl[1] & FOLD_ERR_NONFINITE) FAIL(MGC_E_ARG, nonfinite);
    if (h_ctl[1] & FOLD_ERR_NEGATIVE) FAIL(MGC_E_WEIGHT, negative);
    const int ni = h_ctl[0];
    if (ni == 0) return MGC_OK;
    const bool eager = !g->lazy_built;
    if (eager) {
        int rc = warm_prepare(g);
        if (rc) return rc;
    }
    if (check) {
        int rc = (*check)();
        if (rc) return rc;
        int bits = 0;
        CK(cudaMemcpyAsync(&bits, d_ctl + 1, sizeof(int), cudaMemcpyDeviceToHost, g->stream));
        CK(cudaStreamSynchronize(g->stream));
        if (bits & FOLD_ERR_PAIRSUM)
            FAIL(MGC_E_WEIGHT, "an n-link decrement exceeds what its arc pair holds: r(i->j) + r(j->i), which equals "
                               "c(i->j) + c(j->i), is below cap + rev_cap");
    }
    CK(cudaEventRecord(g->ev_fold[2], g->stream));
    if (g->caps_lazy) {
        int rc;
        for (int color = 0; color < 2; ++color) { rc = caps_launch(g, pl(g, color, g->pl_sel[color])); if (rc) return rc; }
        rc = caps_launch(g, WorkList{g->drop_items, g->win_ctl + WIN_NDROP});
        if (rc) return rc;
        CK(cudaMemsetAsync(g->win_ctl + WIN_NDROP, 0, sizeof(int), g->stream));
        rc = caps_launch(g, WorkList{tiles, d_ctl + 2});
        if (rc) return rc;
    }
    unsigned grid = (unsigned)((ni + 255) / 256);
    if (grid > REDUCE_BLOCKS) grid = REDUCE_BLOCKS;
    { int rc = fold(grid, ni); if (rc) return rc; }
    sum_partials(g, g->partials, grid, g->d_scalars);
    CK(cudaMemsetAsync(g->d_tcount, 0, 256, g->stream));
    CK(cudaMemsetAsync(g->pflag, 0, (size_t)g->TL.ntiles * sizeof(int), g->stream));
    g->pl_sel[0] = g->pl_sel[1] = 0;
    {
        unsigned lgrid = (unsigned)g->n_ctas * 4u;
        if (lgrid > (unsigned)g->TL.ntiles) lgrid = (unsigned)g->TL.ntiles;
        if (g->nd == 4) k_seed_lists4<<<lgrid, T4_VOX, 0, g->stream>>>(g->L, g->TL4, g->S, g->pflag, pl(g, 0, 0), pl(g, 1, 0));
        else k_seed_lists<<<lgrid, TILE_VOX, 0, g->stream>>>(g->L, g->TL, g->S, eager ? nullptr : g->cmat, g->pflag,
                                                             pl(g, 0, 0), pl(g, 1, 0));
    }
    g->st.kernel_launches += 3;
    CK(cudaGetLastError());
    CK(cudaEventRecord(g->ev_fold[3], g->stream));
    CK(cudaEventSynchronize(g->ev_fold[3]));
    {
        float ms0 = 0, ms1 = 0;
        if (cudaEventElapsedTime(&ms0, g->ev_fold[0], g->ev_fold[1]) == cudaSuccess &&
            cudaEventElapsedTime(&ms1, g->ev_fold[2], g->ev_fold[3]) == cudaSuccess)
            g->st.ms_seeds += ms0 + ms1;
        g->st.ms_caps -= caps_resolve(g);
    }
    g->labels_fresh = false;
    g->sweep_mode = -1;
    g->solved = false;
    g->host_mask_valid = false;
    g->st.seed_folds++;
    return MGC_OK;
}

struct FoldCall {
    const char* range;
    const char* bad;
    const char* too_many;
    const char* negative;
    int64_t count;
    int32_t mem;
    bool dense;
    const void* in[4];
    int64_t in_n[4];
    const mgc_array* arrays[2];
    int sort;
    int key_shift;
    int axis;
    bool item_flows;
};

template <typename Key, typename Item>
struct FoldBufs {
    int* ctl;
    const void* in[4];
    Key* keys;
    Key* skeys;
    int* vals;
    int* svals;
    int* head;
    int* pos;
    int* tflag;
    int* tiles;
    Item* items;
    unsigned* tbits;
    unsigned* tails;
    double* dx;
    unsigned* stails;
    void* tmp;
    size_t tmp_bytes;
};

struct Bump {
    char* base;
    size_t used;
    template <typename T>
    T* take(size_t count)
    {
        T* p = base ? (T*)(base + used) : nullptr;
        used += (count * sizeof(T) + 15) / 16 * 16;
        return p;
    }
};

template <typename Key, typename Item, typename Group, typename Fold, typename Check = std::nullptr_t>
static int fold_run(mgc_graph* g, const FoldCall& c, Group&& group, Fold&& fold, Check&& check = nullptr)
{
    constexpr bool arcs = std::is_same<Item, NlinkItem>::value;
    if (!g) return MGC_E_ARG;
    if (c.bad) FAIL(MGC_E_ARG, c.bad);
    if (c.count > (int64_t)INT32_MAX) FAIL(MGC_E_ARG, c.too_many);
    if (c.mem != MGC_MEM_HOST && c.mem != MGC_MEM_DEVICE) FAIL(MGC_E_ARG, "bad memory space");
    bool eager = false;
    { int rc0 = warm_check(g, &eager); if (rc0) return rc0; }
    if (c.dense && c.count && c.count != (int64_t)g->L.n) FAIL(MGC_E_ARG, "the dense form takes one weight pair per voxel");
    CK(cudaSetDevice(g->device));
    { int rc0 = check_pending(g); if (rc0) return rc0; }
    const void* in[4] = {c.in[0], c.in[1], c.in[2], c.in[3]};
    for (int k = 0; k < 2; ++k)
        if (c.arrays[k]) { int rc0 = stage_input(g, c.arrays[k], k, &in[2 + k]); if (rc0) return rc0; }
    int rc = MGC_OK;
    if (c.count) {
        const auto host_t0 = std::chrono::steady_clock::now();
        const int n = (int)c.count;
        const int end_bit = bits_for(((uint64_t)g->L.n << c.key_shift) - 1ull);
        size_t tmp_bytes = 0;
        CK(fold_sort(c.sort, nullptr, &tmp_bytes, (Key*)nullptr, (Key*)nullptr, nullptr, nullptr, n, end_bit, g->stream));
        CK(fold_scan(nullptr, &tmp_bytes, nullptr, nullptr, n, g->stream));
        if (c.item_flows) {
            size_t tb = 0;
            CK(tails_sort(nullptr, &tb, nullptr, nullptr, (int)std::min(2 * (size_t)n, (size_t)g->L.n),
                          bits_for(g->L.n), g->stream));
            tmp_bytes = std::max(tmp_bytes, tb);
// ... 326 lines not shown
```

### medpy_b200/csrc/gc_handle.cuh

```cuda
#pragma once
#include "gc_host.hpp"
#include "gc_common.cuh"
#include "gc_terms.cuh"
#include "gc_tiles.cuh"
#include "gc_tiles4.cuh"
#include "gc_tma.cuh"
#include "gc_build.cuh"

#include <nccl.h>
#include <nvtx3/nvToolsExt.h>

#include <cstdint>
#include <string>
#include <type_traits>
#include <vector>

struct Buf {
    void* p = nullptr;
    size_t bytes = 0;
};

struct mgc_graph {
    int device = 0;
    int user_ndim = 0;
    int nd = 3;
    int shift = 0;
    int64_t user_shape[4] = {1, 1, 1, 1};
    Lattice L{};
    bool slab = false;
    bool ghost_lo = false, ghost_hi = false;
    int64_t global_dim0 = 0, z0 = 0, z1 = 0;

    State<double> S{};
    std::vector<Buf> owned_bufs;
    Buf scratch[5];
    Buf raw;
    uint8_t* mask_dev = nullptr;
    double* partials = nullptr;
    unsigned n_partials = 0;
    void* minmax_buf = nullptr;
    double* d_scalars = nullptr;
    int* d_flags = nullptr;
    unsigned long long* d_count = nullptr;
    int64_t device_bytes = 0;

    cudaStream_t stream = nullptr;
    bool own_stream = false;
    cudaEvent_t ev[6] = {};
    cudaStream_t up_stream = nullptr;
    cudaEvent_t ev_up = nullptr;
    cudaEvent_t ev_slot[5] = {};
    bool slot_used[5] = {false, false, false, false, false};
    cudaEvent_t ev_chunk[2] = {};
    cudaEvent_t ev_terms[2] = {};
    bool terms_open = false;
    bool defer_check = false;
    bool bad_pending = false;
    int* h_bad = nullptr;
    cudaEvent_t ev_bad = nullptr;
    cudaEvent_t ev_b[2] = {};

    bool init_timed = false;
    bool boundary_timed = false;
    bool caps_fresh = true;
    bool tr_fresh = true;
    bool state_init = false;
    bool flow_started = false;
    bool debug_checks = false;
    double debug_excess0 = 0.0;
    bool fuse_build = true;
    bool build_refuse_all = false;
    int* build_refused = nullptr;
    bool lazy_caps = true;
    bool caps_lazy = false;
    bool lazy_built = false;
    bool warm_opt = false;
    bool warm_state = false;
    int* cmat = nullptr;
    int* caps_list = nullptr;
    Buf img_copy;
    Buf prob_copy;
    Buf mark_planes[2];
    const void* caps_img = nullptr;
    bool keep_device_inputs = false;
    Buf fold_buf;
    cudaEvent_t ev_fold[4] = {};
    int caps_dtype = MGC_F32;
    BoundaryParams caps_P{};
    LazyTin caps_tin{};
    std::vector<cudaEvent_t> caps_ev;
    size_t caps_ev_used = 0;
    int build_chunks = 8;
    bool solved = false;
    bool has_nlinks = false;
    double energy = 0.0;
    std::vector<uint8_t> host_mask;
    bool host_mask_valid = false;

    Tiles TL{};
    Tiles4 TL4{};
    uint8_t* smask = nullptr;
    int* pflag = nullptr;
    int* rflag = nullptr;
    int* rl_items[2] = {nullptr, nullptr};
    int* pl_items[2][2] = {{nullptr, nullptr}, {nullptr, nullptr}};
    int* d_tcount = nullptr;
    int pl_sel[2] = {0, 0};
    int* win_tmin = nullptr;
    int* win_items = nullptr;
    int* win_ctl = nullptr;
    int* drop_items = nullptr;
    bool labels_fresh = false;
    int n_ctas = 264;
    int coop_bfs_grid = 0;
    bool use_tma = false;
    PushMaps maps{};
    int tile_iters = 8;
    int tile_iters_first = 4;
    int iters_now = 8;
    int passes0 = 1, passes_max = 32;
    bool skip_first_test = true;
    int first_cap = FIRST_RELABEL_CAP;
    bool labels_capped = false;
    int relp_last = 0;
    bool relp_pending = false;
    int sweep_mode = -1;
    bool use_sweeps = true;
    int sweep_frac = 8;
    int sweep_rounds_min = 1;
    int sweep_rounds_max = 4;
    int sweep_done_frac = 16;

    int64_t max_rounds = 100000;

    ncclComm_t comm = nullptr;
    int comm_rank = 0, comm_world = 1;
    char* msg[4] = {nullptr, nullptr, nullptr, nullptr};
    size_t msg_h_bytes = 0, msg_bytes = 0;
    long long* d_stat = nullptr;
    long long* h_stat = nullptr;
    double* d_esum = nullptr;
    int64_t slab_exchanges = 0, slab_relabel_rounds = 0, slab_push_passes = 0, slab_global_relabels = 0;
    std::vector<cudaEvent_t> ph_events;
    std::vector<int> ph_kind;
    size_t ph_used = 0;
    double slab_phase_ms[6] = {0, 0, 0, 0, 0, 0};

    mgc_stats st{};
    std::string err;
};

extern thread_local std::string g_create_error;
size_t dtype_size(int dt);
int alloc_buf(mgc_graph* g, size_t bytes, void** out);
int ensure_scratch(mgc_graph* g, Buf& b, size_t bytes);
int upload(mgc_graph* g, void* dst, const void* src, size_t bytes, int slot);
void slots_release(mgc_graph* g, unsigned mask);
int stage_input(mgc_graph* g, const mgc_array* a, int slot, const void** out);
void sum_partials(mgc_graph* g, const double* partials, unsigned n, double* out);
void resolve_term_span(mgc_graph* g);
int check_pending(mgc_graph* g);
int boundary_params(mgc_graph* g, int kind, int dtype, const void* img, double sigma, const double* spacing, double norm, BoundaryParams* out);

typedef CUresult (*tmap_encode_fn)(CUtensorMap*, CUtensorMapDataType, cuuint32_t, void*, const cuuint64_t*, const cuuint64_t*,
                                   const cuuint32_t*, const cuuint32_t*, CUtensorMapInterleave, CUtensorMapSwizzle,
                                   CUtensorMapL2promotion, CUtensorMapFloatOOBfill);
tmap_encode_fn tensor_map_encoder();
int tile_solver_options(mgc_graph* g);
void push_tma_setup(mgc_graph* g);
int materialise_zeros(mgc_graph* g);
int caps_launch(mgc_graph* g, WorkList wl);
int push_state_all(mgc_graph* g);
double caps_resolve(mgc_graph* g);
int dirty_clear(mgc_graph* g);
int init_tiles(mgc_graph* g);
int relabel_tiles_begin(mgc_graph* g);
int relabel_tiles_run(mgc_graph* g, int* any, bool want_any = true, bool first = false);
int push_tiles(mgc_graph* g, int passes);
int count_active_tiles_enqueue(mgc_graph* g, unsigned long long* dst);
int count_active_tiles(mgc_graph* g, int64_t* out);
int readout(mgc_graph* g, double* energy_part);

int warm_prepare(mgc_graph* g);

void slab_comm_release(mgc_graph* g);

struct Nvtx {
    explicit Nvtx(const char* name) { nvtxRangePushA(name); }
    ~Nvtx() { nvtxRangePop(); }
};

inline unsigned nblocks(const mgc_graph* g) { return (g->L.n + 255u) / 256u; }
inline unsigned rblocks(const mgc_graph* g) { const unsigned nb = nblocks(g); return nb < REDUCE_BLOCKS ? nb : REDUCE_BLOCKS; }

inline WorkList rl(mgc_graph* g, int i) { return WorkList{g->rl_items[i], g->d_tcount + i}; }
inline WorkList pl(mgc_graph* g, int color, int buf) { return WorkList{g->pl_items[color][buf], g->d_tcount + 2 + color * 2 + buf}; }
inline int* cursor(mgc_graph* g) { return g->d_tcount + 8; }

inline bool warm_wanted(const mgc_graph* g) { return g->warm_opt && !g->slab && !g->lazy_built; }

struct TermSpan {
    mgc_graph* g;
    explicit TermSpan(mgc_graph* g_) : g(g_)
    {
        if (!g->terms_open) { cudaEventRecord(g->ev_terms[0], g->stream); g->terms_open = true; }
    }
    void stop(unsigned slot_mask) { slots_release(g, slot_mask); cudaEventRecord(g->ev_terms[1], g->stream); }
};

template <typename E_, int FN_, int USE_MAX_, int SPACING_>
struct LazyTerm {
    using E = E_;
    static constexpr int FN = FN_, USE_MAX = USE_MAX_, SPACING = SPACING_;
};

template <typename F>
void lazy_dispatch(const mgc_graph* g, F&& f)
{
    auto by_dtype = [&](auto e) {
        using E = decltype(e);
        const BoundaryParams& P = g->caps_P;
        if constexpr (!std::is_integral<E>::value) {
            if (P.fn == 1 && P.inv_spacing_on == 0.0) {
                if (P.use_max) f(LazyTerm<E, 1, 1, 0>{});
                else           f(LazyTerm<E, 1, 0, 0>{});
                return;
            }
        }
        f(LazyTerm<E, -1, -1, -1>{});
    };
    switch (g->caps_dtype) {
        case MGC_F32: by_dtype(float{}); break;
        case MGC_F64: by_dtype(double{}); break;
        case MGC_U8: by_dtype(uint8_t{}); break;
        case MGC_I16: by_dtype(int16_t{}); break;
        default: by_dtype(int32_t{}); break;
    }
}
```

### medpy_b200/csrc/gc_pybind.cpp

```cpp
#include <pybind11/numpy.h>
#include <pybind11/pybind11.h>
#include <pybind11/stl.h>

#include <algorithm>
#include <atomic>
#include <cmath>
#include <cstring>
#include <memory>
#include <stdexcept>
#include <thread>
#include <string>
#include <vector>

#if defined(__x86_64__)
#include <immintrin.h>
#endif

#include "../../include/medpy_b200_graphcut.h"
#include "host_pack.hpp"

namespace py = pybind11;

namespace {

void check(int rc, const mgc_graph* g)
{
    if (rc == MGC_OK) return;
    std::string msg = mgc_last_error(g);
    if (msg.empty()) msg = "medpy_b200 graph-cut error " + std::to_string(rc);
    if (rc == MGC_E_ARG || rc == MGC_E_WEIGHT) throw py::value_error(msg);
    throw std::runtime_error(msg);
}

int dtype_code(const std::string& kind_size)
{
    if (kind_size == "f4") return MGC_F32;
    if (kind_size == "f8") return MGC_F64;
    if (kind_size == "u1" || kind_size == "b1") return MGC_U8;
    if (kind_size == "i2") return MGC_I16;
    if (kind_size == "i4") return MGC_I32;
    return -1;
}

struct ArrayRef {
    mgc_array a{};
    py::object keep;
    std::vector<int64_t> shape;
};

ArrayRef make_ref(const py::object& obj, int want_dtype , const char* what)
{
    ArrayRef r;
    if (py::hasattr(obj, "__cuda_array_interface__")) {
        py::dict d = obj.attr("__cuda_array_interface__");
        py::tuple data = d["data"];
        r.a.data = reinterpret_cast<const void*>(data[0].cast<uintptr_t>());
        r.a.mem = MGC_MEM_DEVICE;
        std::string ts = d["typestr"].cast<std::string>();
        r.a.dtype = dtype_code(ts.substr(1));
        py::tuple shp = d["shape"];
        for (auto s : shp) r.shape.push_back(s.cast<int64_t>());
        size_t es = (size_t)std::stoi(ts.substr(2));
        if (d.contains("strides") && !d["strides"].is_none()) {
            py::tuple st = d["strides"];
            for (size_t i = 0; i < st.size() && i < MGC_MAX_NDIM; ++i) r.a.strides[i] = st[i].cast<int64_t>();
        } else {
            int64_t acc = (int64_t)es;
            for (int i = (int)r.shape.size() - 1; i >= 0; --i) { if (i < MGC_MAX_NDIM) r.a.strides[i] = acc; acc *= r.shape[i]; }
        }
        r.keep = obj;
    } else {
        py::array arr = py::array::ensure(obj);
        if (!arr) throw py::value_error(std::string(what) + ": expected an array");
        std::string ks(1, arr.dtype().kind());
        ks += std::to_string(arr.dtype().itemsize());
        r.a.dtype = dtype_code(ks);
        r.a.data = arr.data();
        r.a.mem = MGC_MEM_HOST;
        for (py::ssize_t i = 0; i < arr.ndim(); ++i) {
            r.shape.push_back(arr.shape(i));
            if (i < MGC_MAX_NDIM) r.a.strides[i] = arr.strides(i);
        }
        r.keep = arr;
    }
    if (r.a.dtype < 0) throw py::value_error(std::string(what) + ": unsupported dtype");
    if (want_dtype >= 0 && r.a.dtype != want_dtype) throw py::value_error(std::string(what) + ": wrong dtype");
    return r;
}

class PyGraph {
public:
    PyGraph(const std::vector<int64_t>& shape, int device) : shape_(shape)
    {
        int rc = mgc_create((int32_t)shape.size(), shape.data(), device, &g_);
        if (rc != MGC_OK) { std::string m = mgc_last_error(nullptr); if (rc == MGC_E_ARG) throw py::value_error(m); throw std::runtime_error(m); }
    }
    PyGraph(const std::vector<int64_t>& shape, int64_t z0, int64_t z1, int device) : shape_(shape)
    {
        int rc = mgc_create_slab((int32_t)shape.size(), shape.data(), z0, z1, device, &g_);
        if (rc != MGC_OK) { std::string m = mgc_last_error(nullptr); if (rc == MGC_E_ARG) throw py::value_error(m); throw std::runtime_error(m); }
        shape_[0] = (z1 - z0) + (z0 > 0 ? 1 : 0) + (z1 < shape[0] ? 1 : 0);
        owned_planes_ = z1 - z0;
    }
    ~PyGraph() { if (g_) mgc_destroy(g_); }
    PyGraph(const PyGraph&) = delete;
    PyGraph& operator=(const PyGraph&) = delete;

    void check_shape(const ArrayRef& r, const char* what) const
    {
        if (r.shape != shape_) throw py::value_error(std::string(what) + ": shape does not match the graph's lattice");
    }

    void add_regional_probability(const py::object& prob, double alpha, bool compute_f32)
    {
        ArrayRef r = make_ref(prob, -1, "probability_map");
        check_shape(r, "probability_map");
        check_inputs();
        int rc;
        { py::gil_scoped_release rel; rc = mgc_add_regional_probability(g_, &r.a, alpha, compute_f32 ? MGC_F32 : MGC_F64); }
        check(rc, g_);
        held_live_ = false;
    }
    void add_tweights_dense(const py::object& src, const py::object& snk)
    {
        ArrayRef a = make_ref(src, MGC_F64, "src"), b = make_ref(snk, MGC_F64, "snk");
        check_shape(a, "src"); check_shape(b, "snk");
        check_inputs();
        int rc;
        { py::gil_scoped_release rel; rc = mgc_add_tweights_dense(g_, &a.a, &b.a); }
        check(rc, g_);
        held_live_ = false;
    }
    void add_markers(const py::object& fg, const py::object& bg)
    {
        ArrayRef a, b;
        bool hf = !fg.is_none(), hb = !bg.is_none();
        if (hf) { a = make_ref(fg, MGC_U8, "fg_markers"); check_shape(a, "fg_markers"); }
// ... 166 lines not shown
        if (a.mem != b.mem || a.mem != c.mem || a.mem != r.mem)
            throw py::value_error("i, j, cap and rev_cap must all be host or all be device arrays");
        check_inputs();
        int rc;
        {
            py::gil_scoped_release rel;
            rc = fold(g_, (const int64_t*)a.p, (const int64_t*)b.p, (const double*)c.p, (const double*)r.p, a.n, a.mem);
        }
        check(rc, g_);
    }
    void add_nweights_dense_warm(int axis, const py::object& fwd, const py::object& bwd)
    {
        fold_nweights_dense(axis, fwd, bwd, mgc_add_nweights_dense_warm);
    }
    void remove_nweights_dense_warm(int axis, const py::object& fwd, const py::object& bwd)
    {
        fold_nweights_dense(axis, fwd, bwd, mgc_remove_nweights_dense_warm);
    }
    void fold_nweights_dense(int axis, const py::object& fwd, const py::object& bwd,
                             int (*fold)(mgc_graph*, int32_t, const mgc_array*, const mgc_array*))
    {
        ArrayRef a = make_ref(fwd, MGC_F64, "fwd"), b = make_ref(bwd, MGC_F64, "bwd");
        check_shape(a, "fwd"); check_shape(b, "bwd");
        check_inputs();
        int rc;
        { py::gil_scoped_release rel; rc = fold(g_, axis, &a.a, &b.a); }
        check(rc, g_);
    }
    double maxflow()
    {
        check_inputs();
        double e = 0;
        int rc;
        { py::gil_scoped_release rel; rc = mgc_maxflow(g_, &e); }
        check(rc, g_);
        return e;
    }
    py::array_t<uint8_t> get_mask()
    {
        std::vector<py::ssize_t> shp(shape_.begin(), shape_.end());
        if (owned_planes_ >= 0) shp[0] = owned_planes_;
        size_t n = 1;
        for (auto d : shp) n *= (size_t)d;
        void* mem = nullptr;
        if (mgc_host_alloc(n ? n : 1, &mem) != MGC_OK) throw std::runtime_error("pinned host allocation failed");
        py::capsule owner(mem, [](void* p) { mgc_host_free(p); });
        int rc;
        { py::gil_scoped_release rel; rc = mgc_get_mask(g_, (uint8_t*)mem, MGC_MEM_HOST); }
        check(rc, g_);
        return py::array_t<uint8_t>(shp, (const uint8_t*)mem, owner);
    }
    void get_mask_into(uintptr_t device_ptr)
    {
        int rc;
        { py::gil_scoped_release rel; rc = mgc_get_mask(g_, reinterpret_cast<uint8_t*>(device_ptr), MGC_MEM_DEVICE); }
        check(rc, g_);
    }
    int what_segment(int64_t i) { int32_t s = 0; check(mgc_what_segment(g_, i, &s), g_); return s; }
    double get_edge(int64_t i, int64_t j) { check_inputs(); double c = 0; check(mgc_get_edge(g_, i, j, &c), g_); return c; }
    double get_trcap(int64_t i) { check_inputs(); double c = 0; check(mgc_get_trcap(g_, i, &c), g_); return c; }
    int64_t get_node_num() { int64_t n = 0; check(mgc_get_node_num(g_, &n), g_); return n; }
    int64_t get_arc_num() { int64_t n = 0; check(mgc_get_arc_num(g_, &n), g_); return n; }
    void reset() { check(mgc_reset(g_), g_); held_live_ = false; }
    void set_option(int option, long long value) { check(mgc_set_option(g_, option, value), g_); }
    void check_deferred() { int rc; { py::gil_scoped_release rel; rc = mgc_check(g_); } check(rc, g_); }
    void set_stream(uintptr_t s) { check(mgc_set_stream(g_, reinterpret_cast<void*>(s)), g_); }
    void synchronize() { int rc; { py::gil_scoped_release rel; rc = mgc_synchronize(g_); } check(rc, g_); }
    py::dict stats()
    {
        mgc_stats s{};
        check(mgc_get_stats(g_, &s), g_);
        py::dict d;
        d["n_voxels"] = s.n_voxels; d["push_sweeps"] = s.push_sweeps; d["global_relabels"] = s.global_relabels;
        d["relabel_sweeps"] = s.relabel_sweeps; d["kernel_launches"] = s.kernel_launches; d["active_last"] = s.active_last;
        d["ms_terms"] = s.ms_terms; d["ms_solve"] = s.ms_solve; d["ms_readout"] = s.ms_readout;
        d["ms_push"] = s.ms_push; d["ms_relabel"] = s.ms_relabel; d["ms_boundary"] = s.ms_boundary; d["ms_init"] = s.ms_init;
        d["flow_const"] = s.flow_const; d["energy"] = s.energy; d["device_bytes"] = s.device_bytes;
        d["tiles_materialised"] = s.tiles_materialised; d["ms_caps"] = s.ms_caps;
        d["seed_folds"] = s.seed_folds; d["ms_seeds"] = s.ms_seeds; d["ms_seeds_host"] = s.ms_seeds_host;
        d["tiles_deferred"] = s.tiles_deferred; d["tiles_dropped"] = s.tiles_dropped;
        d["relabel_passes"] = s.relabel_passes; d["ms_relabel_first"] = s.ms_relabel_first;
        d["relabel_passes_first"] = s.relabel_passes_first;
        d["build_blocks_refused"] = s.build_blocks_refused;
        return d;
    }
    int64_t slab_plane_elems() { int64_t n = 0; check(mgc_slab_plane_elems(g_, &n), g_); return n; }
    void slab_begin() { int rc; { py::gil_scoped_release rel; rc = mgc_slab_begin(g_); } check(rc, g_); }
    void slab_push(int n) { int rc; { py::gil_scoped_release rel; rc = mgc_slab_push(g_, n); } check(rc, g_); }
    void slab_pack(uintptr_t hlo, uintptr_t flo, uintptr_t hhi, uintptr_t fhi)
    {
        int rc;
        { py::gil_scoped_release rel; rc = mgc_slab_pack(g_, (int32_t*)hlo, (double*)flo, (int32_t*)hhi, (double*)fhi); }
        check(rc, g_);
    }
    void slab_unpack(uintptr_t hlo, uintptr_t flo, uintptr_t hhi, uintptr_t fhi, uintptr_t changed_dev)
    {
        int rc;
        { py::gil_scoped_release rel; rc = mgc_slab_unpack(g_, (const int32_t*)hlo, (const double*)flo, (const int32_t*)hhi, (const double*)fhi, (int32_t*)changed_dev); }
        check(rc, g_);
    }
    void slab_count_active_dev(uintptr_t count_dev)
    {
        int rc;
        { py::gil_scoped_release rel; rc = mgc_slab_count_active_dev(g_, (unsigned long long*)count_dev); }
        check(rc, g_);
    }
    void slab_relabel_begin() { int rc; { py::gil_scoped_release rel; rc = mgc_slab_relabel_begin(g_); } check(rc, g_); }
    int slab_relabel_relax(bool want_changed)
    {
        int32_t c = 0;
        int rc;
        { py::gil_scoped_release rel; rc = mgc_slab_relabel_relax(g_, want_changed ? &c : nullptr); }
        check(rc, g_);
        return c;
    }
    int64_t slab_count_active() { int64_t a = 0; int rc; { py::gil_scoped_release rel; rc = mgc_slab_count_active(g_, &a); } check(rc, g_); return a; }
    double slab_finish() { double e = 0; int rc; { py::gil_scoped_release rel; rc = mgc_slab_finish(g_, &e); } check(rc, g_); return e; }

    static py::bytes slab_comm_unique_id()
    {
        char id[128];
        int rc = mgc_slab_comm_unique_id(id);
        if (rc != MGC_OK) throw std::runtime_error(mgc_last_error(nullptr));
        return py::bytes(id, 128);
    }
    void slab_comm_init(int rank, int world, const py::bytes& id)
    {
        std::string s = id;
        if (s.size() != 128) throw py::value_error("the NCCL unique id has 128 bytes");
        int rc;
        { py::gil_scoped_release rel; rc = mgc_slab_comm_init(g_, rank, world, s.data()); }
        check(rc, g_);
    }
    double slab_solve()
    {
        double e = 0;
        int rc;
        { py::gil_scoped_release rel; rc = mgc_slab_solve(g_, &e); }
        check(rc, g_);
        return e;
    }
    py::dict slab_solve_stats()
    {
        int64_t a = 0, b = 0, c = 0, d = 0;
        check(mgc_slab_solve_stats(g_, &a, &b, &c, &d), g_);
        py::dict out;
        out["exchanges"] = a; out["relabel_rounds"] = b; out["push_passes"] = c; out["global_relabels"] = d;
        double ph[6] = {0, 0, 0, 0, 0, 0};
        check(mgc_slab_solve_phase_ms(g_, ph), g_);
        py::dict phase;
        phase["local_bfs_ms"] = ph[0]; phase["exchange_ms"] = ph[1]; phase["stop_test_ms"] = ph[2]; phase["push_ms"] = ph[3];
        phase["readout_ms"] = ph[4]; phase["host_blocked_ms"] = ph[5];
        out["phase_ms"] = phase;
        return out;
    }

    std::vector<int64_t> shape() const { return shape_; }

private:
    struct Held { py::object obj; int64_t version; };
    static int64_t version_of(const py::object& o)
    {
        return py::hasattr(o, "_version") ? o.attr("_version").cast<int64_t>() : -1;
    }
    void hold_inputs(std::vector<Held> hold)
    {
// ... 324 lines not shown
```

### medpy_b200/csrc/gc_slab.cu

```cuda
#include "gc_handle.cuh"
#include "gc_slab_kernels.cuh"

#include <dlfcn.h>

#include <chrono>
#include <cstring>
#include <mutex>
#include <string>
#include <type_traits>

namespace {
struct NcclApi {
    ncclResult_t (*GetUniqueId)(ncclUniqueId*) = nullptr;
    ncclResult_t (*CommInitRank)(ncclComm_t*, int, ncclUniqueId, int) = nullptr;
    ncclResult_t (*CommDestroy)(ncclComm_t) = nullptr;
    ncclResult_t (*CommAbort)(ncclComm_t) = nullptr;
    ncclResult_t (*CommGetAsyncError)(ncclComm_t, ncclResult_t*) = nullptr;
    const char* (*GetErrorString)(ncclResult_t) = nullptr;
    ncclResult_t (*AllReduce)(const void*, void*, size_t, ncclDataType_t, ncclRedOp_t, ncclComm_t, cudaStream_t) = nullptr;
    ncclResult_t (*Send)(const void*, size_t, ncclDataType_t, int, ncclComm_t, cudaStream_t) = nullptr;
    ncclResult_t (*Recv)(void*, size_t, ncclDataType_t, int, ncclComm_t, cudaStream_t) = nullptr;
    ncclResult_t (*GroupStart)() = nullptr;
    ncclResult_t (*GroupEnd)() = nullptr;
    bool ok = false;
// ... 145 lines not shown
    const unsigned P = g->L.plane;
    const unsigned nb = (P + 255u) / 256u;
    if (g->ghost_lo && h_lo) {
        const size_t border = (size_t)g->L.own0 * P, ghost = border - P;
        k_slab_pack<double><<<nb, 256, 0, g->stream>>>(P, g->S.height + border, g->S.excess + ghost, h_lo, f_lo);
        g->st.kernel_launches++;
    }
    if (g->ghost_hi && h_hi) {
        const size_t border = (size_t)(g->L.own1 - 1) * P, ghost = border + P;
        k_slab_pack<double><<<nb, 256, 0, g->stream>>>(P, g->S.height + border, g->S.excess + ghost, h_hi, f_hi);
        g->st.kernel_launches++;
    }
    CK(cudaGetLastError());
    return MGC_OK;
}

int mgc_slab_unpack(mgc_graph* g, const int32_t* h_lo, const double* f_lo, const int32_t* h_hi, const double* f_hi,
                    int32_t* changed_dev)
{
    if (!g) return MGC_E_ARG;
    CK(cudaSetDevice(g->device));
    const unsigned P = g->L.plane;
    const unsigned nb = (P + 255u) / 256u;
    for (int side = 0; side < 2; ++side) {
        const bool have = side == 0 ? (g->ghost_lo && h_lo) : (g->ghost_hi && h_hi);
        if (!have) continue;
        const int zb = side == 0 ? g->L.own0 : g->L.own1 - 1;
        const int zg = side == 0 ? zb - 1 : zb + 1;
        const int k = side == 0 ? 0 : 1;
        const int32_t* hin = side == 0 ? h_lo : h_hi;
        const double* fin = side == 0 ? f_lo : f_hi;
        if (g->nd == 4)
            k_slab_unpack_tiles4<double><<<nb, 256, 0, g->stream>>>(g->L, g->TL4, g->S, zg, zb, k, hin, fin, g->rflag, rl(g, 0), rl(g, 1),
                                                                   g->d_tcount + CTL_RLCUR, g->pflag, pl(g, 0, g->pl_sel[0]),
                                                                   pl(g, 1, g->pl_sel[1]), changed_dev);
        else
            k_slab_unpack_tiles<double><<<nb, 256, 0, g->stream>>>(g->L, g->TL, g->S, zg, zb, k, hin, fin, g->rflag, rl(g, 0), rl(g, 1),
                                                                  g->d_tcount + CTL_RLCUR, g->pflag, pl(g, 0, g->pl_sel[0]),
                                                                  pl(g, 1, g->pl_sel[1]), changed_dev);
        g->st.kernel_launches++;
    }
    CK(cudaGetLastError());
    return MGC_OK;
}

int mgc_slab_relabel_begin(mgc_graph* g)
{
    if (!g) return MGC_E_ARG;
    if (!g->state_init) FAIL(MGC_E_STATE, "call mgc_slab_begin first");
    CK(cudaSetDevice(g->device));
    g->st.global_relabels++;
    return relabel_tiles_begin(g);
}

int mgc_slab_relabel_relax(mgc_graph* g, int32_t* changed_out)
{
    if (!g) return MGC_E_ARG;
    CK(cudaSetDevice(g->device));
    int any = 0;
    const int rc = relabel_tiles_run(g, &any, changed_out != nullptr);
    if (rc) return rc;
    if (changed_out) *changed_out = any ? 1 : 0;
    return MGC_OK;
}

int mgc_slab_count_active(mgc_graph* g, int64_t* active_out)
{
    if (!g || !active_out) return MGC_E_ARG;
    CK(cudaSetDevice(g->device));
    return count_active_tiles(g, active_out);
}

int mgc_slab_count_active_dev(mgc_graph* g, unsigned long long* count_dev)
{
    if (!g || !count_dev) return MGC_E_ARG;
    CK(cudaSetDevice(g->device));
    return count_active_tiles_enqueue(g, count_dev);
}

int mgc_slab_finish(mgc_graph* g, double* energy_part)
{
    if (!g || !energy_part) return MGC_E_ARG;
    CK(cudaSetDevice(g->device));
    int rc = readout(g, energy_part);
    if (rc) return rc;
    g->energy = *energy_part;
    g->st.energy = g->energy;
    g->solved = true;
    return MGC_OK;
}


int mgc_slab_comm_unique_id(void* out128)
{
    if (!out128) return MGC_E_ARG;
    NcclApi& N = nccl_api();
    if (!N.ok) { g_create_error = "libnccl.so.2 could not be loaded"; return MGC_E_CUDA; }
    static_assert(sizeof(ncclUniqueId) == 128, "ncclUniqueId is 128 bytes");
    ncclUniqueId id;
    if (N.GetUniqueId(&id) != ncclSuccess) { g_create_error = "ncclGetUniqueId failed"; return MGC_E_CUDA; }
    memcpy(out128, &id, sizeof(id));
    return MGC_OK;
}

int mgc_slab_comm_init(mgc_graph* g, int32_t rank, int32_t world, const void* unique_id128)
{
    if (!g || !unique_id128 || world < 1 || rank < 0 || rank >= world) return MGC_E_ARG;
    if (!g->slab) FAIL(MGC_E_STATE, "not a z-slab handle");
    NcclApi& N = nccl_api();
    if (!N.ok) FAIL(MGC_E_CUDA, "libnccl.so.2 could not be loaded");
    CK(cudaSetDevice(g->device));
    if ((rank > 0) != g->ghost_lo || (rank < world - 1) != g->ghost_hi) FAIL(MGC_E_ARG, "rank / world do not match the slab's position");
    slab_comm_release(g);
    ncclUniqueId id;
    memcpy(&id, unique_id128, sizeof(id));
    NK(N.CommInitRank(&g->comm, world, id, rank));
    g->comm_rank = rank; g->comm_world = world;
    const size_t P = g->L.plane;
    g->msg_h_bytes = (P * 4 + 7) / 8 * 8;
    g->msg_bytes = g->msg_h_bytes + P * 8;
    void* p = nullptr;
    for (int i = 0; i < 4; ++i) if (!g->msg[i]) { int rc = alloc_buf(g, g->msg_bytes, &p); if (rc) return rc; g->msg[i] = (char*)p; CK(cudaMemsetAsync(p, 0, g->msg_bytes, g->stream)); }
    if (!g->d_stat) { int rc = alloc_buf(g, 64, &p); if (rc) return rc; g->d_stat = (long long*)p; }
    if (!g->d_esum) { int rc = alloc_buf(g, 64, &p); if (rc) return rc; g->d_esum = (double*)p; }
    if (!g->h_stat) { void* hp = nullptr; if (mgc_host_alloc(64, &hp) != MGC_OK) FAIL(MGC_E_NOMEM, "pinned host allocation failed"); g->h_stat = (long long*)hp; }
    return MGC_OK;
}

int mgc_slab_solve(mgc_graph* g, double* energy_total)
{
    if (!g || !energy_total) return MGC_E_ARG;
    if (!g->slab || !g->comm) FAIL(MGC_E_STATE, "call mgc_slab_comm_init first");
    NcclApi& N = nccl_api();
    CK(cudaSetDevice(g->device));
    int rc = mgc_slab_begin(g);
    if (rc) return rc;
    g->slab_exchanges = g->slab_relabel_rounds = g->slab_push_passes = g->slab_global_relabels = 0;
    for (double& x : g->slab_phase_ms) x = 0.0;
    g->ph_used = 0; g->ph_kind.clear();
    auto timed_sync = [&]() -> cudaError_t {
        const auto t0 = std::chrono::steady_clock::now();
        const cudaError_t e = cudaStreamSynchronize(g->stream);
        g->slab_phase_ms[5] += std::chrono::duration<double, std::milli>(std::chrono::steady_clock::now() - t0).count();
        return e;
    };
    int passes = g->passes0 > 0 ? g->passes0 : 1;
    const int passes_cap = g->passes_max < 8 ? g->passes_max : 8;
    int64_t rounds = 0;
    for (;;) {
        phase_begin(g, 0);
        rc = mgc_slab_relabel_begin(g);
        phase_end(g);
        if (rc) return rc;
        for (;;) {
            CK(cudaMemsetAsync(g->d_stat, 0, 3 * sizeof(long long), g->stream));
            for (int k = 0; k < 2; ++k) {
                phase_begin(g, 0);
                rc = mgc_slab_relabel_relax(g, nullptr);
                phase_end(g);
                if (rc) return rc;
                rc = slab_exchange(g, g->d_stat + k, true);
                if (rc) return rc;
                g->slab_relabel_rounds++;
            }
            phase_begin(g, 2);
            rc = mgc_slab_count_active_dev(g, (unsigned long long*)(g->d_stat + 2));
            if (rc) return rc;
            if (g->comm_world > 1) NK(N.AllReduce(g->d_stat, g->d_stat, 3, ncclInt64, ncclSum, g->comm, g->stream));
            CK(cudaMemcpyAsync(g->h_stat, g->d_stat, 3 * sizeof(long long), cudaMemcpyDeviceToHost, g->stream));
            phase_end(g);
            CK(timed_sync());
            rc = slab_comm_poll(g);
            if (rc) return rc;
            if (g->h_stat[1] == 0) break;
        }
        g->slab_global_relabels++;
        if (g->h_stat[2] == 0) break;
        if (++rounds > g->max_rounds) FAIL(MGC_E_NOCONV, "push-relabel did not converge within the round cap");
        for (int p = 0; p < passes; ++p) {
            phase_begin(g, 3);
            rc = mgc_slab_push(g, 1);
            phase_end(g);
            if (rc) return rc;
            rc = slab_exchange(g, nullptr, false);
            if (rc) return rc;
            g->slab_push_passes++;
        }
        passes = passes * 2 > passes_cap ? passes_cap : passes * 2;
    }
    double part = 0.0;
    phase_begin(g, 4);
    rc = mgc_slab_finish(g, &part);
    if (rc) return rc;
    CK(cudaMemcpyAsync(g->d_esum, &part, sizeof(double), cudaMemcpyHostToDevice, g->stream));
    if (g->comm_world > 1) NK(N.AllReduce(g->d_esum, g->d_esum, 1, ncclFloat64, ncclSum, g->comm, g->stream));
    CK(cudaMemcpyAsync(energy_total, g->d_esum, sizeof(double), cudaMemcpyDeviceToHost, g->stream));
    phase_end(g);
    CK(timed_sync());
    phase_resolve(g);
    return slab_comm_poll(g);
}

int mgc_slab_solve_phase_ms(const mgc_graph* g, double* out6)
{
    if (!g || !out6) return MGC_E_ARG;
    for (int i = 0; i < 6; ++i) out6[i] = g->slab_phase_ms[i];
    return MGC_OK;
}

int mgc_slab_solve_stats(const mgc_graph* g, int64_t* exchanges, int64_t* relabel_rounds, int64_t* push_passes, int64_t* global_relabels)
{
    if (!g) return MGC_E_ARG;
    if (exchanges) *exchanges = g->slab_exchanges;
    if (relabel_rounds) *relabel_rounds = g->slab_relabel_rounds;
    if (push_passes) *push_passes = g->slab_push_passes;
    if (global_relabels) *global_relabels = g->slab_global_relabels;
    return MGC_OK;
}

}
```

### medpy_b200/csrc/gc_solve.cu

```cuda
#include "gc_handle.cuh"
#include "gc_solver.cuh"
#include "gc_persist.cuh"
#include "gc_sweep.cuh"
#include "gc_solve_kernels.cuh"

#include <cmath>
#include <cstdio>
#include <cstdlib>
#include <string>

tmap_encode_fn tensor_map_encoder()
{
    static tmap_encode_fn encode = nullptr;
    if (!encode) {
        void* fn = nullptr;
        cudaDriverEntryPointQueryResult qres;
        if (cudaGetDriverEntryPoint("cuTensorMapEncodeTiled", &fn, cudaEnableDefault, &qres) != cudaSuccess || !fn) {
            cudaGetLastError();
            return nullptr;
        }
        encode = (tmap_encode_fn)fn;
    }
    return encode;
}

namespace {
bool make_push_maps(mgc_graph* g)
{
    tmap_encode_fn encode = tensor_map_encoder();
    if (!encode) return false;
    const cuuint64_t X = (cuuint64_t)g->L.dim[2], Y = (cuuint64_t)g->L.dim[1], Z = (cuuint64_t)g->L.dim[0];
    if (X % 2) return false;
    const cuuint64_t dims[3] = {X, Y, Z};
    const cuuint64_t strides[2] = {X * 8, X * Y * 8};
    const cuuint32_t box[3] = {TILE, TILE, TILE};
    const cuuint32_t estr[3] = {1, 1, 1};
    for (int p = 0; p < TMA_PLANES; ++p) {
        void* base = p < 6 ? (void*)g->S.cap[p] : (void*)g->S.excess;
        if (((uintptr_t)base) & 15) return false;
        if (encode(&g->maps.m[p], CU_TENSOR_MAP_DATA_TYPE_FLOAT64, 3, base, dims, strides, box, estr, CU_TENSOR_MAP_INTERLEAVE_NONE,
                   CU_TENSOR_MAP_SWIZZLE_NONE, CU_TENSOR_MAP_L2_PROMOTION_NONE, CU_TENSOR_MAP_FLOAT_OOB_FILL_NONE) != CUDA_SUCCESS)
            return false;
    }
    return true;
}
}

int tile_solver_options(mgc_graph* g)
{
    const void* bfs = g->nd == 4 ? (const void*)k_bfs_coop4 : (const void*)k_bfs_coop;
    const int bfs_threads = g->nd == 4 ? T4_VOX : TILE_VOX;
    g->n_ctas = 2 * cached_sm_count(g->device);
    if (const char* e1 = getenv("MEDPY_GC_ITERS")) if (atoi(e1) > 0) g->tile_iters = g->tile_iters_first = atoi(e1);
    if (const char* e2 = getenv("MEDPY_GC_PASSES0")) if (atoi(e2) > 0) g->passes0 = atoi(e2);
    if (const char* e3 = getenv("MEDPY_GC_PASSES_MAX")) if (atoi(e3) > 0) g->passes_max = atoi(e3);
    if (const char* e7 = getenv("MEDPY_GC_SWEEP")) g->use_sweeps = atoi(e7) != 0;
    if (const char* e8 = getenv("MEDPY_GC_SWEEP_FRAC")) if (atoi(e8) > 0) g->sweep_frac = atoi(e8);
    if (const char* e9 = getenv("MEDPY_GC_SWEEP_ROUNDS")) if (atoi(e9) > 0) g->sweep_rounds_max = atoi(e9);
    if (const char* e11 = getenv("MEDPY_GC_SWEEP_MIN_ROUNDS")) if (atoi(e11) > 0) g->sweep_rounds_min = atoi(e11);
    if (const char* e10 = getenv("MEDPY_GC_SWEEP_DONE_FRAC")) if (atoi(e10) > 0) g->sweep_done_frac = atoi(e10);
    if (const char* e12 = getenv("MEDPY_GC_BUILD_REFUSE_ALL")) g->build_refuse_all = atoi(e12) != 0;
    int coop = 0, nb = 0;
    cudaDeviceGetAttribute(&coop, cudaDevAttrCooperativeLaunch, g->device);
    if (!coop || cudaOccupancyMaxActiveBlocksPerMultiprocessor(&nb, bfs, bfs_threads, 0) != cudaSuccess || nb < 1) {
        cudaGetLastError();
        FAIL(MGC_E_CUDA, "the cooperative BFS of the tile solver cannot be launched on this device (no co-resident CTA)");
    }
    g->coop_bfs_grid = nb * cached_sm_count(g->device);
    return MGC_OK;
}

void push_tma_setup(mgc_graph* g)
{
    const char* e6 = getenv("MEDPY_GC_TMA");
    const size_t smem = 2 * TMA_STAGE_BYTES + 6 * TILE_VOX * sizeof(double) + 1024 * sizeof(int) + 64;
    if ((!e6 || atoi(e6) != 0) && make_push_maps(g) &&
        cudaFuncSetAttribute(k_push_tile_tma<double>, cudaFuncAttributeMaxDynamicSharedMemorySize, (int)smem) == cudaSuccess)
        g->use_tma = true;
    else
        cudaGetLastError();
}

int materialise_zeros(mgc_graph* g)
{
    const size_t nb = (size_t)g->L.n;
    if (g->caps_fresh) {
        for (int k = 0; k < 2 * g->nd; ++k) CK(cudaMemsetAsync(g->S.cap[k], 0, nb * sizeof(double), g->stream));
        g->caps_fresh = false;
    }
    if (g->tr_fresh) {
        CK(cudaMemsetAsync(g->S.tr, 0, nb * sizeof(double), g->stream));
        g->tr_fresh = false;
    }
    return MGC_OK;
}

int caps_launch(mgc_graph* g, WorkList wl)
{
    if (g->caps_ev_used + 2 > g->caps_ev.size()) g->caps_ev.resize(g->caps_ev_used + 2, nullptr);
    for (size_t i = g->caps_ev_used; i < g->caps_ev_used + 2; ++i) if (!g->caps_ev[i]) CK(cudaEventCreate(&g->caps_ev[i]));
    CK(cudaEventRecord(g->caps_ev[g->caps_ev_used], g->stream));
    CK(cudaMemsetAsync(g->d_flags + 4, 0, 2 * sizeof(int), g->stream));
    k_caps_claim<<<(unsigned)g->n_ctas * 4u, 256, 0, g->stream>>>(g->TL, g->cmat, wl, g->caps_list, g->d_flags + 4);
    int* count = g->d_flags + 4;
    int* done = g->d_flags + 3;
    lazy_dispatch(g, [&](auto t) {
        using T = decltype(t);
        k_caps_tiles<typename T::E, T::FN, T::USE_MAX, T::SPACING><<<(unsigned)g->n_ctas, TILE_VOX, 0, g->stream>>>(
            g->L, g->TL, g->S, (const typename T::E*)g->caps_img, g->caps_P, g->caps_tin, g->caps_list, count, count + 1, done);
    });
    CK(cudaEventRecord(g->caps_ev[g->caps_ev_used + 1], g->stream));
    g->caps_ev_used += 2;
    g->st.kernel_launches += 2;
    CK(cudaGetLastError());
    return MGC_OK;
}

int push_state_all(mgc_graph* g)
{
    if (!g->caps_lazy) return MGC_OK;
    g->caps_lazy = false;
    return caps_launch(g, WorkList{nullptr, nullptr});
}

double caps_resolve(mgc_graph* g)
{
    double total = 0.0;
    if (g->caps_ev_used && cudaEventSynchronize(g->caps_ev[g->caps_ev_used - 1]) == cudaSuccess) {
        for (size_t i = 0; i + 1 < g->caps_ev_used; i += 2) {
            float ms = 0;
            if (cudaEventElapsedTime(&ms, g->caps_ev[i], g->caps_ev[i + 1]) == cudaSuccess) total += ms;
        }
    }
    g->caps_ev_used = 0;
    g->st.ms_caps += total;
    return total;
}

namespace {
int read_tcount(mgc_graph* g, int idx, int* out)
{
    CK(cudaMemcpyAsync(out, g->d_tcount + idx, sizeof(int), cudaMemcpyDeviceToHost, g->stream));
    CK(cudaStreamSynchronize(g->stream));
    return MGC_OK;
}
}

int dirty_clear(mgc_graph* g)
{
    if (g->nd == 3 && g->TL.dflag) {
        CK(cudaMemsetAsync(g->TL.dflag, 0, (size_t)g->TL.ntiles * sizeof(int), g->stream));
        CK(cudaMemsetAsync(g->TL.dcount, 0, sizeof(int), g->stream));
    }
    return MGC_OK;
}

int init_tiles(mgc_graph* g)
{
    Nvtx range("mgc:init_state");
    { int rc0 = push_state_all(g); if (rc0) return rc0; }
    CK(cudaMemsetAsync(g->d_tcount, 0, 256, g->stream));
    g->pl_sel[0] = g->pl_sel[1] = 0;
    const bool warm = warm_wanted(g);
    cudaEventRecord(g->ev[4], g->stream);
    if (g->nd == 4) {
        if (warm) k_init_tile4<double, true><<<g->TL4.ntiles, T4_VOX, 0, g->stream>>>(g->L, g->TL4, g->S, g->smask, g->rflag, rl(g, 0),
                                                                                     g->pflag, pl(g, 0, 0), pl(g, 1, 0));
        else k_init_tile4<double><<<g->TL4.ntiles, T4_VOX, 0, g->stream>>>(g->L, g->TL4, g->S, g->smask, g->rflag, rl(g, 0), g->pflag,
                                                                           pl(g, 0, 0), pl(g, 1, 0));
    } else if (warm) {
        k_init_tile<double, true><<<g->TL.ntiles, TILE_VOX, 0, g->stream>>>(g->L, g->TL, g->S, g->rflag, rl(g, 0), g->pflag,
                                                                            pl(g, 0, 0), pl(g, 1, 0));
    } else {
        k_init_tile<double><<<g->TL.ntiles, TILE_VOX, 0, g->stream>>>(g->L, g->TL, g->S, g->rflag, rl(g, 0), g->pflag,
                                                                      pl(g, 0, 0), pl(g, 1, 0));
    }
    cudaEventRecord(g->ev[5], g->stream);
    g->init_timed = true;
    g->st.kernel_launches++;
    CK(cudaGetLastError());
    g->state_init = true;
    g->labels_fresh = true;
    g->sweep_mode = -1;
    if (warm) {
        g->warm_state = true;
        g->flow_started = true;
    }
    return dirty_clear(g);
}

int relabel_tiles_begin(mgc_graph* g)
{
    if (g->labels_fresh) {
        g->labels_fresh = false;
        CK(cudaMemsetAsync(g->d_tcount + CTL_RLCUR, 0, sizeof(int), g->stream));
        return MGC_OK;
    }
    CK(cudaMemsetAsync(g->d_tcount, 0, 2 * sizeof(int), g->stream));
    CK(cudaMemsetAsync(g->rflag, 0, (size_t)g->TL.ntiles * sizeof(int), g->stream));
    if (g->nd == 4) {
        k_relabel_reset4<<<g->TL4.ntiles, T4_VOX, 0, g->stream>>>(g->L, g->TL4, g->S.rmask, g->smask, g->S.height, g->rflag, rl(g, 0));
    } else {
        if (g->TL.dflag && g->sweep_mode == 0) {
            k_relabel_reset_list<<<g->n_ctas * 2, TILE_VOX, 0, g->stream>>>(g->L, g->TL, g->S.rmask, g->S.height, g->rflag, rl(g, 0));
            CK(cudaMemsetAsync(g->TL.dcount, 0, sizeof(int), g->stream));
        } else {
            const unsigned nruns = (unsigned)g->L.dim[0] * (unsigned)g->L.dim[1] * (unsigned)g->TL.nt[2];
            unsigned grid = (nruns + 255u) / 256u;
            if (grid > (unsigned)g->n_ctas * 8u) grid = (unsigned)g->n_ctas * 8u;
            k_relabel_reset<<<grid, 256, 0, g->stream>>>(g->L, g->TL, g->S.rmask, g->S.height, g->rflag, rl(g, 0));
            int rcd = dirty_clear(g);
            if (rcd) return rcd;
        }
    }
    g->st.kernel_launches++;
    CK(cudaMemsetAsync(g->d_tcount + CTL_RLCUR, 0, sizeof(int), g->stream));
    CK(cudaGetLastError());
    return MGC_OK;
}

namespace {
int relabel_sweep_round(mgc_graph* g, int* pending, bool with_check)
{
    const int last = g->nd - 1;
    for (int a = 0; a < last; ++a) {
        if (g->L.dim[a] < 2) continue;
        const unsigned nlines = g->L.n / (unsigned)g->L.dim[a];
        k_sweep_axis<<<(nlines + 255u) / 256u, 256, 0, g->stream>>>(g->L, g->S.rmask, g->S.height, a);
        g->st.kernel_launches++;
    }
    if (g->L.dim[last] >= 2 && g->L.dim[last] <= SWEEP_SHORT) {
        const unsigned nrows = g->L.n / (unsigned)g->L.dim[last];
        k_sweep_rows_short<<<(nrows + 255u) / 256u, 256, 0, g->stream>>>(g->L, g->S.rmask, g->S.height);
        g->st.kernel_launches++;
    } else if (g->L.dim[last] >= 2) {
        const unsigned nrows = g->L.n / (unsigned)g->L.dim[last];
        unsigned grid = (nrows + SWEEP_WARPS - 1) / SWEEP_WARPS;
        const unsigned cap = (unsigned)cached_sm_count(g->device) * 16u;
        if (grid > cap) grid = cap;
        k_sweep_rows<<<grid, 32 * SWEEP_WARPS, 0, g->stream>>>(g->L, g->S.rmask, g->S.height);
        g->st.kernel_launches++;
    }
    g->st.relabel_sweeps++;
    if (!with_check) { CK(cudaGetLastError()); return MGC_OK; }
    CK(cudaMemsetAsync(g->d_tcount, 0, 2 * sizeof(int), g->stream));
    CK(cudaMemsetAsync(g->rflag, 0, (size_t)g->TL.ntiles * sizeof(int), g->stream));
    if (g->nd == 4) k_relabel_check4<<<nblocks(g), 256, 0, g->stream>>>(g->L, g->TL4, g->S.rmask, g->S.height, g->rflag, rl(g, 0));
    else            k_relabel_check<<<nblocks(g), 256, 0, g->stream>>>(g->L, g->TL, g->S.rmask, g->S.height, g->rflag, rl(g, 0));
    g->st.kernel_launches++;
    CK(cudaMemsetAsync(g->d_tcount + CTL_RLCUR, 0, sizeof(int), g->stream));
    CK(cudaGetLastError());
    return read_tcount(g, 0, pending);
}
}

int relabel_tiles_run(mgc_graph* g, int* any, bool want_any, bool first)
{
    *any = 0;
    g->relp_last = 0;
    g->relp_pending = false;
    if (g->use_sweeps && g->TL.ntiles >= 64 && g->sweep_mode != 0) {
        int pending = 0;
        int rc = read_tcount(g, 0, &pending);
        if (rc) return rc;
        if (g->sweep_mode < 0) g->sweep_mode = pending > g->TL.ntiles / g->sweep_frac ? 1 : 0;
        if (pending > g->TL.ntiles / g->sweep_frac) {
            *any = 1;
            int prev = g->TL.ntiles + 1;
            const int rmin = g->sweep_rounds_min < g->sweep_rounds_max ? g->sweep_rounds_min : g->sweep_rounds_max;
            for (int r = 0; r < g->sweep_rounds_max; ++r) {
                const bool check = r + 1 >= rmin;
                rc = relabel_sweep_round(g, &pending, check);
                if (rc) return rc;
                if (!check) continue;
                if (pending <= g->TL.ntiles / g->sweep_done_frac) break;
                if ((long long)pending * 4 > (long long)prev * 3) break;
                prev = pending;
            }
        }
    }
    const bool capped = first && g->first_cap >= 2 && g->sweep_mode == 0 && g->nd == 3 && !g->slab;
    int cap = capped ? g->first_cap : MGC_HINF;
    g->labels_capped = capped;
    CK(cudaMemsetAsync(g->d_tcount + CTL_CURSOR, 0, sizeof(int), g->stream));
    int* it0 = g->rl_items[0]; int* it1 = g->rl_items[1];
    if (g->nd == 4) {
        void* args4[] = {&g->L, &g->TL4, &g->S.rmask, &g->S.height, &g->rflag, &it0, &it1, &g->d_tcount};
        CK(cudaLaunchCooperativeKernel((void*)k_bfs_coop4, dim3(g->coop_bfs_grid), dim3(T4_VOX), args4, 0, g->stream));
    } else {
        void* args[] = {&g->L, &g->TL, &g->S.rmask, &g->S.height, &g->rflag, &it0, &it1, &g->d_tcount, &cap};
        CK(cudaLaunchCooperativeKernel((void*)k_bfs_coop, dim3(g->coop_bfs_grid), dim3(TILE_VOX), args, 0, g->stream));
    }
    g->st.kernel_launches++;
    g->st.relabel_sweeps++;
    if (want_any) {
        int relp = 0;
        CK(cudaMemcpyAsync(&relp, g->d_tcount + CTL_RELP, sizeof(int), cudaMemcpyDeviceToHost, g->stream));
        CK(cudaStreamSynchronize(g->stream));
        if (relp != 0) *any = 1;
        g->relp_last = relp;
        g->st.relabel_passes += relp;
    } else {
        g->relp_pending = true;
    }
    return MGC_OK;
}

namespace {
int relabel_passes_fetch(mgc_graph* g, bool* enqueued)
{
    *enqueued = false;
    if (!g->relp_pending) return MGC_OK;
    if (!g->h_bad) { g->relp_pending = false; return MGC_OK; }
    CK(cudaMemcpyAsync(g->h_bad + 4, g->d_tcount + CTL_RELP, sizeof(int), cudaMemcpyDeviceToHost, g->stream));
    *enqueued = true;
    return MGC_OK;
}

int relabel_passes_collect(mgc_graph* g)
{
    if (g->relp_pending) {
        g->relp_last = ((volatile int*)g->h_bad)[4];
        g->st.relabel_passes += g->relp_last;
        g->relp_pending = false;
    }
    return g->relp_last;
}

const int* lazy_cmat(const mgc_graph* g) { return g->caps_lazy ? g->cmat : nullptr; }

int window_filter(mgc_graph* g, int color, int a, WorkList* now)
{
    const WorkList cur = pl(g, color, a);
    *now = WorkList{g->win_items, g->win_ctl + WIN_NOW};
    CK(cudaMemsetAsync(g->win_ctl + WIN_GMIN, 0x7f, sizeof(int), g->stream));
    CK(cudaMemsetAsync(g->win_ctl + WIN_NOW, 0, sizeof(int), g->stream));
    k_window_min<double><<<g->n_ctas * 2, TILE_VOX, 0, g->stream>>>(g->L, g->TL, g->S, lazy_cmat(g), g->caps_tin, cur, g->win_tmin, g->win_ctl);
    k_window_split<<<g->n_ctas, 256, 0, g->stream>>>(cur, g->win_tmin, lazy_cmat(g), g->pflag, *now, pl(g, color, 1 - a),
                                                     g->drop_items, g->win_ctl, g->labels_capped ? 1 : 0);
    g->st.kernel_launches += 2;
    CK(cudaGetLastError());
    return MGC_OK;
}

int push_color(mgc_graph* g, int color)
{
    g->flow_started = true;
    const int a = g->pl_sel[color], oa = g->pl_sel[1 - color];
    WorkList cur = pl(g, color, a);
    if (g->sweep_mode == 0 && g->nd == 3 && !g->slab) {
        const int rc = window_filter(g, color, a, &cur);
        if (rc) return rc;
    }
    if (g->caps_lazy) {
        const int rc = g->sweep_mode == 1 ? push_state_all(g) : caps_launch(g, cur);
        if (rc) return rc;
    }
    CK(cudaMemsetAsync(cursor(g), 0, sizeof(int), g->stream));
    const int capped = g->labels_capped ? 1 : 0;
    if (g->nd == 4) {
        k_push_tile4<double><<<g->n_ctas, T4_VOX, 0, g->stream>>>(g->L, g->TL4, g->S, g->smask, g->iters_now, g->pflag, cur,
                                                                  cursor(g), pl(g, color, 1 - a), pl(g, 1 - color, oa));
    } else if (g->use_tma) {
        const size_t smem = 2 * TMA_STAGE_BYTES + 6 * TILE_VOX * sizeof(double) + 1024 * sizeof(int) + 64;
        k_push_tile_tma<double><<<g->n_ctas, TILE_VOX, smem, g->stream>>>(g->L, g->TL, g->S, g->maps, g->iters_now, g->pflag,
                                                                          cur, cursor(g), pl(g, color, 1 - a),
                                                                          pl(g, 1 - color, oa), capped);
    } else
    k_push_tile<double><<<g->n_ctas, TILE_VOX, 0, g->stream>>>(g->L, g->TL, g->S, g->iters_now, g->pflag, cur,
                                                               cursor(g), pl(g, color, 1 - a), pl(g, 1 - color, oa), capped);
    CK(cudaMemsetAsync(g->d_tcount + 2 + color * 2 + a, 0, sizeof(int), g->stream));
    g->pl_sel[color] = 1 - a;
    g->st.kernel_launches++;
    return MGC_OK;
}

int push_passes(mgc_graph* g, int passes)
{
    for (int p = 0; p < passes; ++p) {
        int rc = push_color(g, 0);
        if (rc) return rc;
        rc = push_color(g, 1);
        if (rc) return rc;
    }
    g->st.push_sweeps += passes;
    CK(cudaGetLastError());
    return MGC_OK;
}
}

int push_tiles(mgc_graph* g, int passes)
{
    Nvtx range("mgc:push_passes");
    cudaEventRecord(g->ev[2], g->stream);
    int rc = push_passes(g, passes);
    if (rc) return rc;
    if (g->slab) return MGC_OK;
    cudaEventRecord(g->ev[3], g->stream);
    CK(cudaEventSynchronize(g->ev[3]));
    { float ms = 0; cudaEventElapsedTime(&ms, g->ev[2], g->ev[3]); g->st.ms_push += (double)ms - caps_resolve(g); }
    return MGC_OK;
}

int count_active_tiles_enqueue(mgc_graph* g, unsigned long long* dst)
{
    CK(cudaMemsetAsync(dst, 0, sizeof(unsigned long long), g->stream));
    if (g->nd == 4) {
        for (int color = 0; color < 2; ++color)
            k_count_active_tiles4<double><<<g->n_ctas * 2, T4_VOX, 0, g->stream>>>(g->L, g->TL4, g->S, pl(g, color, g->pl_sel[color]), dst);
        g->st.kernel_launches += 2;
    } else {
        k_count_active_tiles2<double><<<g->n_ctas * 2, TILE_VOX, 0, g->stream>>>(g->L, g->TL, g->S, lazy_cmat(g), g->caps_tin,
                                                                                 pl(g, 0, g->pl_sel[0]), pl(g, 1, g->pl_sel[1]), dst);
        g->st.kernel_launches++;
    }
    CK(cudaGetLastError());
    return MGC_OK;
}

int count_active_tiles(mgc_graph* g, int64_t* out)
{
    int rc = count_active_tiles_enqueue(g, g->d_count);
    if (rc) return rc;
    unsigned long long c = 0;
    CK(cudaMemcpyAsync(&c, g->d_count, sizeof(c), cudaMemcpyDeviceToHost, g->stream));
    CK(cudaStreamSynchronize(g->stream));
    *out = (int64_t)c;
    g->st.active_last = (int64_t)c;
    return MGC_OK;
}

namespace {
int debug_invariants(mgc_graph* g, bool after)
{
    if (!g->debug_checks) return MGC_OK;
    { int rc0 = push_state_all(g); if (rc0) return rc0; }
    double* d = g->d_scalars + 4;
    CK(cudaMemsetAsync(d, 0, 3 * sizeof(double), g->stream));
    if (g->nd == 3) k_debug_invariants<3, double, true><<<nblocks(g), 256, 0, g->stream>>>(g->L, g->S, d);
    else            k_debug_invariants<4, double, false><<<nblocks(g), 256, 0, g->stream>>>(g->L, g->S, d);
    double h[3] = {0, 0, 0};
    CK(cudaMemcpyAsync(h, d, sizeof(h), cudaMemcpyDeviceToHost, g->stream));
    CK(cudaStreamSynchronize(g->stream));
    if (h[2] != 0.0) {
        g->err = "debug check: " + std::to_string((long long)h[2]) + " invariant violation(s) (negative capacity / excess, absorbed flow out of range or stale residual mask)";
        return MGC_E_STATE;
    }
    if (!after) { g->debug_excess0 = h[0] + h[1]; return MGC_OK; }
    const double scale = fabs(g->debug_excess0) > 1.0 ? fabs(g->debug_excess0) : 1.0;
    if (!g->slab && !(fabs(h[0] + h[1] - g->debug_excess0) <= 1e-9 * scale)) {
        char buf[200];
        snprintf(buf, sizeof(buf), "debug check: flow not conserved: excess %.17g + absorbed %.17g != initial %.17g", h[0], h[1], g->debug_excess0);
        g->err = buf;
        return MGC_E_STATE;
    }
    return MGC_OK;
}

int solve_tiles(mgc_graph* g)
{
    int rc = materialise_zeros(g);
    if (rc) return rc;
    if (!g->state_init) {
        rc = init_tiles(g);
        if (rc) return rc;
    }
    if (g->win_ctl) CK(cudaMemsetAsync(g->win_ctl + WIN_DEFERRED, 0, 2 * sizeof(int), g->stream));
    int passes = g->passes0;
    int64_t rounds = 0;
    bool push_open = false;
    int passes_done = 0;
    unsigned long long active_fallback = 0;
    unsigned long long* h_active = g->h_bad ? (unsigned long long*)g->h_bad + 1 : &active_fallback;
    for (;;) {
        cudaEventRecord(g->ev[2], g->stream);
        {
            Nvtx range("mgc:global_relabel");
            rc = relabel_tiles_begin(g);
            if (rc) return rc;
            int any = 0;
            rc = relabel_tiles_run(g, &any, false, rounds == 0 && g->skip_first_test);
            if (rc) return rc;
        }
        cudaEventRecord(g->ev[3], g->stream);
        g->st.global_relabels++;
        bool relp_copy = false;
        rc = relabel_passes_fetch(g, &relp_copy);
        if (rc) return rc;
        const bool test = rounds > 0 || !g->skip_first_test;
        if (test) {
            rc = count_active_tiles_enqueue(g, g->d_count);
            if (rc) return rc;
            CK(cudaMemcpyAsync(h_active, g->d_count, sizeof(unsigned long long), cudaMemcpyDeviceToHost, g->stream));
        }
        CK(cudaEventSynchronize(g->ev[3]));
        if (test || relp_copy) CK(cudaStreamSynchronize(g->stream));
        float ms = 0;
        const double caps_ms = caps_resolve(g);
        if (g->init_timed) {
            if (cudaEventElapsedTime(&ms, g->ev[4], g->ev[5]) == cudaSuccess) g->st.ms_init = ms;
            g->init_timed = false;
        }
        cudaEventElapsedTime(&ms, g->ev[2], g->ev[3]);
        const double t_rel = ms;
        g->st.ms_relabel += ms;
        const int relp = relabel_passes_collect(g);
        if (rounds == 0) { g->st.ms_relabel_first += ms; g->st.relabel_passes_first += relp; }
        double t_pass = 0.0;
        if (push_open) {
            cudaEventElapsedTime(&ms, g->ev[4], g->ev[5]);
            const double push_ms = (double)ms - caps_ms;
            g->st.ms_push += push_ms;
            t_pass = push_ms / (passes_done > 0 ? passes_done : 1);
            push_open = false;
            int want = t_pass > 1e-4 ? (int)(t_rel / t_pass + 0.999) : passes * 2;
            if (want < 1) want = 1;
            if (want > passes * 2) want = passes * 2;
            passes = want > g->passes_max ? g->passes_max : want;
        }
        if (test) {
            g->st.active_last = (int64_t)*h_active;
            if (*h_active == 0ull) break;
        }
        if (++rounds > g->max_rounds) FAIL(MGC_E_NOCONV, "push-relabel did not converge within the round cap");
        g->iters_now = rounds == 1 ? g->tile_iters_first : g->tile_iters;
        {
            Nvtx range("mgc:push_passes");
            cudaEventRecord(g->ev[4], g->stream);
            rc = push_passes(g, passes);
            if (rc) return rc;
            cudaEventRecord(g->ev[5], g->stream);
            passes_done = passes;
            push_open = true;
        }
    }
    g->init_timed = false;
    return MGC_OK;
}
}

int readout(mgc_graph* g, double* energy_part)
{
    Nvtx range("mgc:readout");
    const bool clean = g->nd == 3 && !g->slab && g->TL.dflag && g->sweep_mode != 1 && g->L.dim[2] % 4 == 0;
    if (clean) k_readout<double, true, true><<<rblocks(g), 256, 0, g->stream>>>(g->L, g->S, g->mask_dev, g->partials, g->TL.dflag,
                                                                                g->TL.nt[1], g->TL.nt[2]);
    else if (g->nd == 3) k_readout<double, true><<<rblocks(g), 256, 0, g->stream>>>(g->L, g->S, g->mask_dev, g->partials);
    else                 k_readout<double, false><<<rblocks(g), 256, 0, g->stream>>>(g->L, g->S, g->mask_dev, g->partials);
    CK(cudaMemsetAsync(g->d_scalars + 1, 0, sizeof(double), g->stream));
    sum_partials(g, g->partials, rblocks(g), g->d_scalars + 1);
    g->st.kernel_launches += 2;
    double sc[2] = {0, 0};
    int fl[5] = {0, 0, 0, 0, 0};
    int win[2] = {0, 0};
    CK(cudaMemcpyAsync(sc, g->d_scalars, sizeof(sc), cudaMemcpyDeviceToHost, g->stream));
    CK(cudaMemcpyAsync(fl, g->d_flags + 3, sizeof(fl), cudaMemcpyDeviceToHost, g->stream));
    if (g->win_ctl) CK(cudaMemcpyAsync(win, g->win_ctl + WIN_DEFERRED, sizeof(win), cudaMemcpyDeviceToHost, g->stream));
    CK(cudaStreamSynchronize(g->stream));
    g->st.flow_const = sc[0];
    g->st.tiles_materialised = fl[0];
    g->st.build_blocks_refused = fl[4];
    g->st.tiles_deferred += win[0];
    g->st.tiles_dropped += win[1];
    *energy_part = sc[0] + sc[1];
    if (g->init_timed) {
        float ms = 0;
        if (cudaEventElapsedTime(&ms, g->ev[4], g->ev[5]) == cudaSuccess) g->st.ms_init = ms;
        g->init_timed = false;
    }
    return MGC_OK;
}

namespace {
struct Timer {
    mgc_graph* g;
    double* acc;
    Timer(mgc_graph* g_, double* acc_) : g(g_), acc(acc_) { cudaEventRecord(g->ev[0], g->stream); }
    void stop_sync()
    {
        cudaEventRecord(g->ev[1], g->stream);
        cudaEventSynchronize(g->ev[1]);
        float ms = 0;
        cudaEventElapsedTime(&ms, g->ev[0], g->ev[1]);
        *acc += ms;
    }
};
}

extern "C" {

int mgc_maxflow(mgc_graph* g, double* energy)
{
    if (!g) return MGC_E_ARG;
    if (g->slab) FAIL(MGC_E_STATE, "z-slab handles are stepped with mgc_slab_*");
    CK(cudaSetDevice(g->device));
    if (g->solved) { if (energy) *energy = g->energy; return MGC_OK; }
    { int rc0 = check_pending(g); if (rc0) return rc0; }
    resolve_term_span(g);
    {
        Timer t(g, &g->st.ms_solve);
        int rc = warm_prepare(g); if (rc) return rc;
        if (g->debug_checks) {
            rc = materialise_zeros(g); if (rc) return rc;
            if (!g->state_init) { rc = init_tiles(g); if (rc) return rc; }
            rc = debug_invariants(g, false); if (rc) return rc;
        }
        rc = solve_tiles(g);
        if (rc) return rc;
        rc = debug_invariants(g, true);
        if (rc) return rc;
        t.stop_sync();
    }
    {
        Timer t(g, &g->st.ms_readout);
        double e = 0.0;
        int rc = readout(g, &e);
        if (rc) return rc;
        g->energy = e;
        g->st.energy = e;
        t.stop_sync();
    }
    caps_resolve(g);
    g->solved = true;
    if (energy) *energy = g->energy;
    return MGC_OK;
}

}
```

### medpy_b200/csrc/gc_solve_kernels.cuh

```cuda
#pragma once
#include "gc_build.cuh"
#include "gc_tiles4.cuh"

__global__ void __launch_bounds__(256) k_relabel_reset(Lattice L, Tiles TL, const uint8_t* __restrict__ rmask,
                                                       int* __restrict__ height, int* __restrict__ rflag, WorkList rl)
{
    const unsigned ntx = (unsigned)TL.nt[2];
    const unsigned nruns = (unsigned)L.dim[0] * (unsigned)L.dim[1] * ntx;
    for (unsigned r = blockIdx.x * blockDim.x + threadIdx.x; r < nruns; r += gridDim.x * blockDim.x) {
        const unsigned tx = r % ntx, zy = r / ntx;
        const unsigned gy = zy % (unsigned)L.dim[1], gz = zy / (unsigned)L.dim[1];
        const unsigned x0 = tx * TILE;
        const int nx = (int)min((unsigned)TILE, (unsigned)L.dim[2] - x0);
        const unsigned base = gz * L.stride[0] + gy * L.stride[1] + x0;
        const bool own = (int)gz >= L.own0 && (int)gz < L.own1;
        int needs = 0;
        if (nx == TILE && (base & 7u) == 0u) {
            const uint2 m8 = *reinterpret_cast<const uint2*>(rmask + base);
            int h[8];
#pragma unroll
            for (int i = 0; i < 8; ++i) {
                const unsigned m = ((i < 4 ? m8.x : m8.y) >> (8 * (i & 3))) & 0xffu;
                h[i] = (own && (m & RM_SINK)) ? 1 : MGC_HINF;
                needs |= (own && (m & 0x3fu) != 0 && h[i] == MGC_HINF) ? 1 : 0;
// ... 100 lines not shown
        if (c.inb) r.own = img[c.v];
        if (tid < 384) {
            const int face = tid >> 6, fa = (tid >> 3) & 7, fb = tid & 7;
            int z, y, x;
            switch (face) {
                case 0: z = -1; y = fa; x = fb; break;
                case 1: z = TILE; y = fa; x = fb; break;
                case 2: z = fa; y = -1; x = fb; break;
                case 3: z = fa; y = TILE; x = fb; break;
                case 4: z = fa; y = fb; x = -1; break;
                default: z = fa; y = fb; x = TILE; break;
            }
            const int gz = c.tz * TILE + z, gy = c.ty * TILE + y, gx = c.tx * TILE + x;
            if (gz >= 0 && gy >= 0 && gx >= 0 && gz < L.dim[0] && gy < L.dim[1] && gx < L.dim[2])
                r.halo = img[(unsigned)gz * L.stride[0] + (unsigned)gy * L.stride[1] + (unsigned)gx];
        }
        return r;
    };
    auto halo_at = [&]() -> int {
        const int face = tid >> 6, fa = (tid >> 3) & 7, fb = tid & 7;
        switch (face) {
            case 0: return hidx(0, fa + 1, fb + 1);
            case 1: return hidx(TILE + 1, fa + 1, fb + 1);
            case 2: return hidx(fa + 1, 0, fb + 1);
            case 3: return hidx(fa + 1, TILE + 1, fb + 1);
            case 4: return hidx(fa + 1, fb + 1, 0);
            default: return hidx(fa + 1, fb + 1, TILE + 1);
        }
    };
    if (tid == 0) s_slot[0] = atomicAdd(cursor, 1);
    __syncthreads();
    int i = s_slot[0];
    Cells cur{(E)0, (E)0};
    if (i < n) cur = load(list[i]);
    for (int it = 1; i < n; ++it) {
        const int t = list[i];
        const TileCtx c = tile_ctx(L, TL, t);
        const int h = hidx(c.lz + 1, c.ly + 1, c.lx + 1);
        s_img[h] = cur.own;
        if (tid < 384) s_img[halo_at()] = cur.halo;
        if (tid == 0) s_slot[it & 1] = atomicAdd(cursor, 1);
        __syncthreads();
        double p = 0.0;
        unsigned fb = 0u;
        if (c.inb) lazy_tin_load(L, tin, c, p, fb);
        const int inext = s_slot[it & 1];
        Cells nxt{(E)0, (E)0};
        if (inext < n) nxt = load(list[inext]);
        const unsigned valid = c.inb ? tile_pairs(L, c) : 0u;
        const double a = build_val<E>(s_img[h], use_max);
        const E q[6] = {s_img[h - HALO_DIM * HALO_DIM], s_img[h + HALO_DIM * HALO_DIM], s_img[h - HALO_DIM],
                        s_img[h + HALO_DIM], s_img[h - 1], s_img[h + 1]};
        double cap[6];
        if (FN == 1 && SPACING == 0) {
            double t6[6];
#pragma unroll
            for (int k = 0; k < 6; ++k) {
                const double b = build_val<E>(q[k], use_max);
                t6[k] = ((valid >> k) & 1u) ? exp_term_arg(P, use_max ? fmax(a, b) : fabs(__dsub_rn(a, b))) : 0.0;
            }
            const bool ordinary = __all_sync(0xffffffffu, t6[0] <= 700.0 && t6[1] <= 700.0 && t6[2] <= 700.0 &&
                                                          t6[3] <= 700.0 && t6[4] <= 700.0 && t6[5] <= 700.0);
            exp_caps6(t6, ordinary, valid, cap);
        } else {
#pragma unroll
            for (int k = 0; k < 6; ++k)
                cap[k] = ((valid >> k) & 1u) ? build_weight<FN, E>(P, a, q[k], use_max, spacing, P.spacing[k >> 1]) : 0.0;
        }
        if (c.inb) {
            const double tr = lazy_tr(tin, p, fb);
            const double e = c.own ? source_excess(tr, cap) : 0.0;
#pragma unroll
            for (int k = 0; k < 6; ++k) S.cap[k][c.v] = cap[k];
            S.tr[c.v] = tr;
            S.excess[c.v] = e;
        }
        __syncthreads();
        cur = nxt;
        i = inext;
    }
}


template <typename T>
__global__ void __launch_bounds__(TILE_VOX) k_window_min(Lattice L, Tiles TL, State<T> S, const int* __restrict__ cmat, LazyTin tin,
                                                         WorkList cur, int* __restrict__ tmin, int* __restrict__ ctl)
{
    __shared__ int s_min[TILE_VOX / 32];
    const int n = *cur.count;
    for (int i = blockIdx.x; i < n; i += gridDim.x) {
        const int t = cur.items[i];
        const TileCtx c = tile_ctx(L, TL, t);
        const bool mat = !cmat || cmat[t] != 0;
        const int h = c.own ? S.height[c.v] : MGC_HINF;
        int lo = voxel_active<T>(L, S, tin, c, h, mat) ? h : MGC_HINF;
        lo = __reduce_min_sync(0xffffffffu, lo);
        if ((threadIdx.x & 31) == 0) s_min[threadIdx.x >> 5] = lo;
        __syncthreads();
        if (threadIdx.x < 32) {
            int m = threadIdx.x < TILE_VOX / 32 ? s_min[threadIdx.x] : MGC_HINF;
            m = __reduce_min_sync(0xffffffffu, m);
            if (threadIdx.x == 0) {
                tmin[i] = m;
                if (m < MGC_HINF) atomicMin(ctl + WIN_GMIN, m);
            }
        }
        __syncthreads();
    }
}

__device__ __forceinline__ unsigned warp_append(const WorkList& wl, bool take, int t)
{
    const int lane = threadIdx.x & 31;
    const unsigned b = __ballot_sync(0xffffffffu, take);
    int slot = 0;
    if (lane == 0 && b) slot = atomicAdd(wl.count, __popc(b));
    slot = __shfl_sync(0xffffffffu, slot, 0);
    if (take) wl.items[slot + __popc(b & ((1u << lane) - 1u))] = t;
    return b;
}

__global__ void __launch_bounds__(256) k_window_split(WorkList cur, const int* __restrict__ tmin, const int* __restrict__ cmat,
                                                      int* __restrict__ pflag, WorkList now, WorkList later,
                                                      int* __restrict__ drop_items, int* __restrict__ ctl, int labels_capped)
{
    const int n = *cur.count;
    const int gmin = ctl[WIN_GMIN];
    const int lane = threadIdx.x & 31;
    for (int base = (blockIdx.x * blockDim.x + threadIdx.x) & ~31; base < n; base += gridDim.x * blockDim.x) {
        const int i = base + lane;
        const int t = i < n ? cur.items[i] : -1;
        const int m = i < n ? tmin[i] : MGC_HINF;
        const bool act = t >= 0 && m < MGC_HINF;
        const bool drop = t >= 0 && !act && !labels_capped;
        if (drop) pflag[t] = 0;
        warp_append(now, act && m - gmin <= PUSH_WINDOW, t);
        const unsigned bl = warp_append(later, t >= 0 && !drop && !(act && m - gmin <= PUSH_WINDOW), t);
        warp_append(WorkList{drop_items, ctl + WIN_NDROP}, drop && cmat && cmat[t] == 0, t);
        const unsigned bd = __ballot_sync(0xffffffffu, drop);
        if (lane == 0) {
            if (bl) atomicAdd(ctl + WIN_DEFERRED, __popc(bl));
            if (bd) atomicAdd(ctl + WIN_DROPPED, __popc(bd));
        }
    }
}

template <typename T>
__global__ void __launch_bounds__(TILE_VOX) k_count_active_tiles2(Lattice L, Tiles TL, State<T> S, const int* __restrict__ cmat,
                                                                  LazyTin tin, WorkList wa, WorkList wb,
                                                                  unsigned long long* __restrict__ count)
{
    const int na = *(volatile int*)wa.count, nb = *(volatile int*)wb.count;
    const int n = na + nb;
    unsigned mine = 0;
    for (int i0 = blockIdx.x * 4; i0 < n; i0 += gridDim.x * 4) {
        T e[4];
        int h[4], t[4];
        bool own[4], lazy[4];
#pragma unroll
        for (int j = 0; j < 4; ++j) {
            const int i = i0 + j;
            own[j] = false; lazy[j] = false; e[j] = 0; h[j] = MGC_HINF; t[j] = -1;
            if (i < n) {
                t[j] = i < na ? wa.items[i] : wb.items[i - na];
                const TileCtx c = tile_ctx(L, TL, t[j]);
                own[j] = c.own;
                lazy[j] = cmat && cmat[t[j]] == 0;
                if (c.own) { h[j] = S.height[c.v]; if (!lazy[j]) e[j] = S.excess[c.v]; }
            }
        }
#pragma unroll
        for (int j = 0; j < 4; ++j) {
            if (own[j] && lazy[j] && h[j] < MGC_HINF) e[j] = lazy_has_excess(L, tin, tile_ctx(L, TL, t[j])) ? (T)1 : (T)0;
            mine += (own[j] && e[j] > 0 && h[j] < MGC_HINF) ? 1u : 0u;
        }
    }
#pragma unroll
    for (int o = 16; o > 0; o >>= 1) mine += __shfl_down_sync(0xffffffffu, mine, o);
    if ((threadIdx.x & 31) == 0 && mine) atomicAdd(count, (unsigned long long)mine);
}
```

### medpy_b200/csrc/gc_solver.cuh

```cuda
#pragma once
#include "gc_common.cuh"

template <typename T, bool LAZY, bool CLEAN = false>
__global__ void __launch_bounds__(256) k_readout(Lattice L, State<T> S, uint8_t* __restrict__ mask, double* __restrict__ partials,
                                                 const int* __restrict__ dflag = nullptr, int nty = 0, int ntx = 0)
{
    __shared__ double sh[8];
    double a = 0.0;
    const unsigned step = gridDim.x * blockDim.x;
    const unsigned n4 = L.n >> 2;
    for (unsigned q = blockIdx.x * blockDim.x + threadIdx.x; q < n4; q += step) {
        const unsigned v = q << 2;
        uchar4 m;
        unsigned rm = 0;
        bool clean = false;
        if (CLEAN) {
            rm = reinterpret_cast<const unsigned*>(S.rmask)[q];
            const unsigned gz = div_stride(L, v, 0), r = v - gz * L.stride[0];
            const unsigned gy = div_stride(L, r, 1), gx = r - gy * L.stride[1];
            clean = dflag[((int)(gz >> 3) * nty + (int)(gy >> 3)) * ntx + (int)(gx >> 3)] == 0;
        }
        if (clean) {
            const bool own = owned(L, v);
            m.x = (own && (rm & 0x40u)) ? 0 : 1; m.y = (own && ((rm >> 8) & 0x40u)) ? 0 : 1;
            m.z = (own && ((rm >> 16) & 0x40u)) ? 0 : 1; m.w = (own && ((rm >> 24) & 0x40u)) ? 0 : 1;
        } else {
            const int4 h = reinterpret_cast<const int4*>(S.height)[q];
            m.x = h.x >= MGC_HINF ? 1 : 0; m.y = h.y >= MGC_HINF ? 1 : 0;
            m.z = h.z >= MGC_HINF ? 1 : 0; m.w = h.w >= MGC_HINF ? 1 : 0;
        }
        reinterpret_cast<uchar4*>(mask)[q] = m;
        if (LAZY) {
            const unsigned r4 = (CLEAN ? rm : reinterpret_cast<const unsigned*>(S.rmask)[q]) & 0x80808080u;
            if (r4) {
#pragma unroll
                for (int i = 0; i < 4; ++i)
                    if ((r4 >> (8 * i + 7)) & 1u) { if (owned(L, v + i)) a = __dadd_rn(a, (double)S.sink[v + i]); }
            }
        } else if (sizeof(T) == 8) {
            const double2 s0 = reinterpret_cast<const double2*>(S.sink)[2 * q];
            const double2 s1 = reinterpret_cast<const double2*>(S.sink)[2 * q + 1];
            if (owned(L, v)) a = __dadd_rn(a, s0.x);
            if (owned(L, v + 1)) a = __dadd_rn(a, s0.y);
            if (owned(L, v + 2)) a = __dadd_rn(a, s1.x);
            if (owned(L, v + 3)) a = __dadd_rn(a, s1.y);
        } else {
#pragma unroll
            for (int i = 0; i < 4; ++i) if (owned(L, v + i)) a = __dadd_rn(a, (double)S.sink[v + i]);
        }
    }
    if (blockIdx.x == 0 && threadIdx.x < (L.n & 3u)) {
        const unsigned v = (n4 << 2) + threadIdx.x;
        mask[v] = S.height[v] >= MGC_HINF ? 1 : 0;
        if (owned(L, v) && (!LAZY || (S.rmask[v] & 0x80u))) a = __dadd_rn(a, (double)S.sink[v]);
    }
#pragma unroll
    for (int o = 16; o > 0; o >>= 1) a = __dadd_rn(a, __shfl_down_sync(0xffffffffu, a, o));
    const unsigned tid = threadIdx.x;
    if ((tid & 31) == 0) sh[tid >> 5] = a;
    __syncthreads();
    if (tid == 0) {
        double t = sh[0];
#pragma unroll
        for (int w = 1; w < 8; ++w) t = __dadd_rn(t, sh[w]);
        partials[blockIdx.x] = t;
    }
}

template <int ND, typename T, bool CHECK_RMASK>
__global__ void __launch_bounds__(256) k_debug_invariants(Lattice L, State<T> S, double* __restrict__ out)
{
    const unsigned v = blockIdx.x * blockDim.x + threadIdx.x;
    double e = 0.0, a = 0.0;
    unsigned long long bad = 0;
    if (v < L.n && owned(L, v)) {
        e = (double)S.excess[v];
        if (!(e >= 0.0)) bad++;
        const double tr = (double)S.tr[v];
        const unsigned m = S.rmask[v];
        const bool lazy = CHECK_RMASK;
        if (tr < 0) {
            a = (!lazy || (m & 0x80u)) ? (double)S.sink[v] : 0.0;
            if (!(a >= 0.0) || a > -tr) bad++;
            if (CHECK_RMASK && (((m & 0x40u) != 0) != ((-tr) - a > 0))) bad++;
        }
#pragma unroll
        for (int k = 0; k < 2 * ND; ++k) {
            const double c = (double)S.cap[k][v];
            if (c < 0.0) bad++;
            if (CHECK_RMASK && (((m >> k) & 1u) != (c > 0 ? 1u : 0u))) bad++;
        }
    }
#pragma unroll
    for (int o = 16; o > 0; o >>= 1) {
        e += __shfl_down_sync(0xffffffffu, e, o);
        a += __shfl_down_sync(0xffffffffu, a, o);
        bad += __shfl_down_sync(0xffffffffu, bad, o);
    }
    if ((threadIdx.x & 31) == 0) {
        if (e != 0.0) atomicAdd(out, e);
        if (a != 0.0) atomicAdd(out + 1, a);
        if (bad) atomicAdd(out + 2, (double)bad);
    }
}
```

Measured before the change: 43350.

## Cut host waits: defer mask readout, fold resets into kernels, count syncs

Routes every host synchronisation through counting helpers and avoids some of them: a cudaEventQuery is tried before blocking, and mgc_set_stream returns early when the stream is unchanged. The readout kernel is split by template so the energy-only path can skip writing the mask; the mask is produced lazily, or written straight to a caller device buffer. Several per-build memsets are folded into the window-min kernel, which now ping-pongs between two global-min slots so resets need no separate launches. The intent is to reduce host round-trips and launch overhead per solve, at the cost of more state flags (mask_ready, tcount_host) that must stay consistent.

```diff
diff --git a/include/medpy_b200_graphcut.h b/include/medpy_b200_graphcut.h
--- a/include/medpy_b200_graphcut.h
+++ b/include/medpy_b200_graphcut.h
@@ -78,6 +78,7 @@
     double ms_relabel_first;
     int64_t relabel_passes_first;
     int64_t build_blocks_refused;
+    int64_t host_waits;
 } mgc_stats;
 
 
diff --git a/medpy_b200/csrc/gc_api.cu b/medpy_b200/csrc/gc_api.cu
--- a/medpy_b200/csrc/gc_api.cu
+++ b/medpy_b200/csrc/gc_api.cu
@@ -83,7 +83,7 @@
 {
     if (b.bytes >= bytes) return MGC_OK;
     if (b.p) {
-        if (g->stream) cudaStreamSynchronize(g->stream);
+        if (g->stream) wait_stream(g);
         if (g->up_stream) cudaStreamSynchronize(g->up_stream);
         pool_free(g->device, b.bytes, b.p);
         g->device_bytes -= (int64_t)round_up(b.bytes);
@@ -122,7 +122,7 @@
     CK(cudaMemcpyAsync(dst, src, bytes, cudaMemcpyHostToDevice, g->up_stream));
     CK(cudaEventRecord(g->ev_up, g->up_stream));
     CK(cudaStreamWaitEvent(g->stream, g->ev_up, 0));
-    CK(cudaEventSynchronize(g->ev_up));
+    CK(wait_event(g, g->ev_up));
     return MGC_OK;
 }
 
@@ -210,13 +210,15 @@
     g->warm_state = false;
     g->solved = false;
     g->host_mask_valid = false;
+    g->mask_ready = false;
+    g->tcount_host = false;
 }
 }
 
 void resolve_term_span(mgc_graph* g)
 {
     if (!g->terms_open) return;
-    if (cudaEventSynchronize(g->ev_terms[1]) == cudaSuccess) {
+    if (cudaEventQuery(g->ev_terms[1]) == cudaSuccess || wait_event(g, g->ev_terms[1]) == cudaSuccess) {
         float ms = 0;
         if (cudaEventElapsedTime(&ms, g->ev_terms[0], g->ev_terms[1]) == cudaSuccess) g->st.ms_terms += ms;
         if (g->boundary_timed && cudaEventElapsedTime(&ms, g->ev_b[0], g->ev_b[1]) == cudaSuccess) g->st.ms_boundary = ms;
@@ -229,7 +231,7 @@
 {
     if (!g->bad_pending) return MGC_OK;
     g->bad_pending = false;
-    CK(cudaEventSynchronize(g->ev_bad));
+    CK(wait_event(g, g->ev_bad));
     if (*g->h_bad) FAIL(MGC_E_WEIGHT, "Negative or zero weights are not allowed.");
     return MGC_OK;
 }
@@ -441,7 +443,7 @@
         if (rc) return rc;
         double mm[2];
         CK(cudaMemcpyAsync(mm, g->d_scalars + 2, sizeof(mm), cudaMemcpyDeviceToHost, g->stream));
-        CK(cudaStreamSynchronize(g->stream));
+        CK(wait_stream(g));
         P.norm = (kind == MGC_BOUNDARY_MAXIMUM_LINEAR) ? mm[1] : mm[0];
     }
     *out = P;
@@ -490,7 +492,7 @@
 {
     if (!g) return;
     cudaSetDevice(g->device);
-    if (g->stream) cudaStreamSynchronize(g->stream);
+    if (g->stream) wait_stream(g);
     for (auto& b : g->owned_bufs) pool_free(g->device, b.bytes, b.p);
     for (auto& b : g->scratch) if (b.p) pool_free(g->device, b.bytes, b.p);
     if (g->raw.p) pool_free(g->device, g->raw.bytes, g->raw.p);
@@ -657,7 +659,8 @@
 int mgc_set_stream(mgc_graph* g, void* cuda_stream)
 {
     if (!g) return MGC_E_ARG;
-    CK(cudaStreamSynchronize(g->stream));
+    if ((cudaStream_t)cuda_stream == g->stream) return MGC_OK;
+    CK(wait_stream(g));
     if (g->own_stream) { cudaStreamDestroy(g->stream); g->own_stream = false; }
     g->stream = (cudaStream_t)cuda_stream;
     return MGC_OK;
@@ -666,7 +669,7 @@
 int mgc_synchronize(mgc_graph* g)
 {
     if (!g) return MGC_E_ARG;
-    CK(cudaStreamSynchronize(g->stream));
+    CK(wait_stream(g));
     return MGC_OK;
 }
 
@@ -795,7 +798,7 @@
     int bad = 0;
     CK(cudaMemcpyAsync(&bad, g->d_flags, sizeof(int), cudaMemcpyDeviceToHost, g->stream));
     t.stop(4u);
-    CK(cudaStreamSynchronize(g->stream));
+    CK(wait_stream(g));
     if (bad) FAIL(MGC_E_WEIGHT, "Negative or zero weights are not allowed.");
     return MGC_OK;
 }
@@ -829,7 +832,7 @@
     int bad = 0;
     CK(cudaMemcpyAsync(&bad, g->d_flags, sizeof(int), cudaMemcpyDeviceToHost, g->stream));
     t.stop(3u);
-    CK(cudaStreamSynchronize(g->stream));
+    CK(wait_stream(g));
     invalidate(g);
     g->has_nlinks = true;
     if (bad) FAIL(MGC_E_WEIGHT, "Negative or zero weights are not allowed.");
@@ -841,10 +844,17 @@
     if (!g || !out) return MGC_E_ARG;
     if (!g->solved) FAIL(MGC_E_STATE, "call maxflow first");
     CK(cudaSetDevice(g->device));
-    const size_t owned_n = (size_t)(g->L.own1 - g->L.own0) * g->L.plane;
-    const uint8_t* src = g->mask_dev + (size_t)g->L.own0 * g->L.plane;
-    CK(cudaMemcpyAsync(out, src, owned_n, mem == MGC_MEM_DEVICE ? cudaMemcpyDeviceToDevice : cudaMemcpyDeviceToHost, g->stream));
-    CK(cudaStreamSynchronize(g->stream));
+    if (mem == MGC_MEM_DEVICE && !g->slab) {
+        int rc = mask_launch(g, out);
+        if (rc) return rc;
+    } else {
+        int rc = mask_produce(g);
+        if (rc) return rc;
+        const size_t owned_n = (size_t)(g->L.own1 - g->L.own0) * g->L.plane;
+        const uint8_t* src = g->mask_dev + (size_t)g->L.own0 * g->L.plane;
+        CK(cudaMemcpyAsync(out, src, owned_n, mem == MGC_MEM_DEVICE ? cudaMemcpyDeviceToDevice : cudaMemcpyDeviceToHost, g->stream));
+    }
+    CK(wait_stream(g));
     return MGC_OK;
 }
 
@@ -854,9 +864,12 @@
     if (!g->solved) FAIL(MGC_E_STATE, "call maxflow first");
     if (node < 0 || node >= (int64_t)g->L.n) FAIL(MGC_E_ARG, "node id out of range");
     if (!g->host_mask_valid) {
+        CK(cudaSetDevice(g->device));
+        int rc = mask_produce(g);
+        if (rc) return rc;
         g->host_mask.resize(g->L.n);
         CK(cudaMemcpyAsync(g->host_mask.data(), g->mask_dev, g->L.n, cudaMemcpyDeviceToHost, g->stream));
-        CK(cudaStreamSynchronize(g->stream));
+        CK(wait_stream(g));
         g->host_mask_valid = true;
     }
     *segment = g->host_mask[(size_t)node] ? MGC_SOURCE : MGC_SINK;
@@ -882,7 +895,7 @@
         if (cn < 0 || cn >= g->L.dim[d]) continue;
         if (i + off == j) {
             CK(cudaMemcpyAsync(cap, g->S.cap[k] + i, sizeof(double), cudaMemcpyDeviceToHost, g->stream));
-            CK(cudaStreamSynchronize(g->stream));
+            CK(wait_stream(g));
             caps_resolve(g);
             return MGC_OK;
         }
@@ -899,7 +912,7 @@
     { int rc0 = push_state_all(g); if (rc0) return rc0; }
     if (!g->state_init || !g->flow_started) {
         CK(cudaMemcpyAsync(trcap, g->S.tr + node, sizeof(double), cudaMemcpyDeviceToHost, g->stream));
-        CK(cudaStreamSynchronize(g->stream));
+        CK(wait_stream(g));
         return MGC_OK;
     }
     double e = 0, s = 0;
@@ -907,11 +920,11 @@
     CK(cudaMemcpyAsync(&e, g->S.excess + node, sizeof(double), cudaMemcpyDeviceToHost, g->stream));
     CK(cudaMemcpyAsync(&s, g->S.sink + node, sizeof(double), cudaMemcpyDeviceToHost, g->stream));
     if (g->nd == 3) CK(cudaMemcpyAsync(&rm, g->S.rmask + node, 1, cudaMemcpyDeviceToHost, g->stream));
-    CK(cudaStreamSynchronize(g->stream));
+    CK(wait_stream(g));
     if (!(rm & 0x80u)) s = 0;
     double tr = 0;
     CK(cudaMemcpyAsync(&tr, g->S.tr + node, sizeof(double), cudaMemcpyDeviceToHost, g->stream));
-    CK(cudaStreamSynchronize(g->stream));
+    CK(wait_stream(g));
     *trcap = (tr < 0 && -tr - s > 0) ? -(-tr - s) : e;
     return MGC_OK;
 }
diff --git a/medpy_b200/csrc/gc_build.cuh b/medpy_b200/csrc/gc_build.cuh
--- a/medpy_b200/csrc/gc_build.cuh
+++ b/medpy_b200/csrc/gc_build.cuh
@@ -801,3 +801,4 @@
 #define WIN_DEFERRED 2
 #define WIN_DROPPED 3
 #define WIN_NDROP 4
+#define WIN_GMIN2 5
diff --git a/medpy_b200/csrc/gc_build_api.cu b/medpy_b200/csrc/gc_build_api.cu
--- a/medpy_b200/csrc/gc_build_api.cu
+++ b/medpy_b200/csrc/gc_build_api.cu
@@ -281,13 +281,10 @@
         if (t->fg || t->fg_bits) { rc = ensure_scratch(g, g->mark_planes[0], plane_bytes); if (rc) return rc; A.fg_plane = (unsigned*)g->mark_planes[0].p; }
         if (t->bg || t->bg_bits) { rc = ensure_scratch(g, g->mark_planes[1], plane_bytes); if (rc) return rc; A.bg_plane = (unsigned*)g->mark_planes[1].p; }
         A.cmat = g->cmat;
-        CK(cudaMemsetAsync(g->d_flags + 3, 0, sizeof(int), g->stream));
         CK(cudaMemsetAsync(g->win_ctl + WIN_NDROP, 0, sizeof(int), g->stream));
     }
 
     CK(cudaMemsetAsync(g->d_tcount, 0, 256, g->stream));
-    CK(cudaMemsetAsync(g->d_flags, 0, sizeof(int), g->stream));
-    CK(cudaMemsetAsync(g->d_flags + 7, 0, sizeof(int), g->stream));
     { int rcd = dirty_clear(g); if (rcd) return rcd; }
     g->pl_sel[0] = g->pl_sel[1] = 0;
     cudaEventRecord(g->ev_b[0], g->stream);
@@ -334,7 +331,7 @@
         A.z_tile0 = prev_l0;
         rc = build_launch_any(g, lazy, t->image->dtype, imap, A, P, prev_nl);
         if (rc) { cudaStreamSynchronize(g->up_stream); return rc; }
-        CK(cudaEventSynchronize(g->ev_up));
+        CK(wait_event(g, g->ev_up));
     }
     cudaEventRecord(g->ev_b[1], g->stream);
     {
@@ -363,11 +360,16 @@
     g->state_init = true;
     g->solved = false;
     g->host_mask_valid = false;
+    g->mask_ready = false;
     g->labels_fresh = true;
     g->sweep_mode = -1;
     g->init_timed = false;
     g->st.ms_init = 0.0;
     span.stop(0x17u);
+    if (g->h_bad) {
+        CK(cudaMemcpyAsync(g->h_bad + 5, g->d_tcount, sizeof(int), cudaMemcpyDeviceToHost, g->stream));
+        g->tcount_host = true;
+    }
     if (g->defer_check && g->h_bad) {
         CK(cudaMemcpyAsync(g->h_bad, g->d_flags, sizeof(int), cudaMemcpyDeviceToHost, g->stream));
         CK(cudaEventRecord(g->ev_bad, g->stream));
@@ -376,7 +378,7 @@
     }
     int bad = 0;
     CK(cudaMemcpyAsync(&bad, g->d_flags, sizeof(int), cudaMemcpyDeviceToHost, g->stream));
-    CK(cudaStreamSynchronize(g->stream));
+    CK(wait_stream(g));
     if (bad) FAIL(MGC_E_WEIGHT, "Negative or zero weights are not allowed.");
     return MGC_OK;
 }
diff --git a/medpy_b200/csrc/gc_fold.cu b/medpy_b200/csrc/gc_fold.cu
--- a/medpy_b200/csrc/gc_fold.cu
+++ b/medpy_b200/csrc/gc_fold.cu
@@ -143,7 +143,7 @@
     CK(cudaEventRecord(g->ev_fold[1], g->stream));
     int h_ctl[2] = {0, 0};
     CK(cudaMemcpyAsync(h_ctl, d_ctl, sizeof(h_ctl), cudaMemcpyDeviceToHost, g->stream));
-    CK(cudaStreamSynchronize(g->stream));
+    CK(wait_stream(g));
     if (h_ctl[1] & FOLD_ERR_RANGE) FAIL(MGC_E_ARG, "node id out of range");
     if (h_ctl[1] & FOLD_ERR_PAIR) FAIL(MGC_E_ARG, "node ids are not lattice neighbours");
     if (h_ctl[1] & FOLD_ERR_NONFINITE) FAIL(MGC_E_ARG, nonfinite);
@@ -160,7 +160,7 @@
         if (rc) return rc;
         int bits = 0;
         CK(cudaMemcpyAsync(&bits, d_ctl + 1, sizeof(int), cudaMemcpyDeviceToHost, g->stream));
-        CK(cudaStreamSynchronize(g->stream));
+        CK(wait_stream(g));
         if (bits & FOLD_ERR_PAIRSUM)
             FAIL(MGC_E_WEIGHT, "an n-link decrement exceeds what its arc pair holds: r(i->j) + r(j->i), which equals "
                                "c(i->j) + c(j->i), is below cap + rev_cap");
@@ -192,7 +192,7 @@
     g->st.kernel_launches += 3;
     CK(cudaGetLastError());
     CK(cudaEventRecord(g->ev_fold[3], g->stream));
-    CK(cudaEventSynchronize(g->ev_fold[3]));
+    CK(wait_event(g, g->ev_fold[3]));
     {
         float ms0 = 0, ms1 = 0;
         if (cudaEventElapsedTime(&ms0, g->ev_fold[0], g->ev_fold[1]) == cudaSuccess &&
@@ -204,6 +204,7 @@
     g->sweep_mode = -1;
     g->solved = false;
     g->host_mask_valid = false;
+    g->mask_ready = false;
     g->st.seed_folds++;
     return MGC_OK;
 }
diff --git a/medpy_b200/csrc/gc_handle.cuh b/medpy_b200/csrc/gc_handle.cuh
--- a/medpy_b200/csrc/gc_handle.cuh
+++ b/medpy_b200/csrc/gc_handle.cuh
@@ -46,7 +46,7 @@
 
     cudaStream_t stream = nullptr;
     bool own_stream = false;
-    cudaEvent_t ev[6] = {};
+    cudaEvent_t ev[9] = {};
     cudaStream_t up_stream = nullptr;
     cudaEvent_t ev_up = nullptr;
     cudaEvent_t ev_slot[5] = {};
@@ -57,6 +57,7 @@
     bool defer_check = false;
     bool bad_pending = false;
     int* h_bad = nullptr;
+    bool tcount_host = false;
     cudaEvent_t ev_bad = nullptr;
     cudaEvent_t ev_b[2] = {};
 
@@ -96,6 +97,7 @@
     double energy = 0.0;
     std::vector<uint8_t> host_mask;
     bool host_mask_valid = false;
+    bool mask_ready = false;
 
     Tiles TL{};
     Tiles4 TL4{};
@@ -110,6 +112,8 @@
     int* win_items = nullptr;
     int* win_ctl = nullptr;
     int* drop_items = nullptr;
+    int win_gslot = WIN_GMIN;
+    int* win_stale = nullptr;
     bool labels_fresh = false;
     int n_ctas = 264;
     int coop_bfs_grid = 0;
@@ -169,7 +173,7 @@
 int tile_solver_options(mgc_graph* g);
 void push_tma_setup(mgc_graph* g);
 int materialise_zeros(mgc_graph* g);
-int caps_launch(mgc_graph* g, WorkList wl);
+int caps_launch(mgc_graph* g, WorkList wl, bool zeroed = false);
 int push_state_all(mgc_graph* g);
 double caps_resolve(mgc_graph* g);
 int dirty_clear(mgc_graph* g);
@@ -179,7 +183,9 @@
 int push_tiles(mgc_graph* g, int passes);
 int count_active_tiles_enqueue(mgc_graph* g, unsigned long long* dst);
 int count_active_tiles(mgc_graph* g, int64_t* out);
-int readout(mgc_graph* g, double* energy_part);
+int readout(mgc_graph* g, double* energy_part, bool with_mask);
+int mask_launch(mgc_graph* g, uint8_t* dst);
+int mask_produce(mgc_graph* g);
 
 int warm_prepare(mgc_graph* g);
 
@@ -189,6 +195,9 @@
     explicit Nvtx(const char* name) { nvtxRangePushA(name); }
     ~Nvtx() { nvtxRangePop(); }
 };
+
+inline cudaError_t wait_stream(mgc_graph* g) { g->st.host_waits++; return cudaStreamSynchronize(g->stream); }
+inline cudaError_t wait_event(mgc_graph* g, cudaEvent_t e) { g->st.host_waits++; return cudaEventSynchronize(e); }
 
 inline unsigned nblocks(const mgc_graph* g) { return (g->L.n + 255u) / 256u; }
 inline unsigned rblocks(const mgc_graph* g) { const unsigned nb = nblocks(g); return nb < REDUCE_BLOCKS ? nb : REDUCE_BLOCKS; }
diff --git a/medpy_b200/csrc/gc_pybind.cpp b/medpy_b200/csrc/gc_pybind.cpp
--- a/medpy_b200/csrc/gc_pybind.cpp
+++ b/medpy_b200/csrc/gc_pybind.cpp
@@ -51,8 +51,9 @@
 ArrayRef make_ref(const py::object& obj, int want_dtype , const char* what)
 {
     ArrayRef r;
-    if (py::hasattr(obj, "__cuda_array_interface__")) {
-        py::dict d = obj.attr("__cuda_array_interface__");
+    py::object cai = py::getattr(obj, "__cuda_array_interface__", py::none());
+    if (!cai.is_none()) {
+        py::dict d = cai;
         py::tuple data = d["data"];
         r.a.data = reinterpret_cast<const void*>(data[0].cast<uintptr_t>());
         r.a.mem = MGC_MEM_DEVICE;
@@ -385,6 +386,7 @@
         d["relabel_passes"] = s.relabel_passes; d["ms_relabel_first"] = s.ms_relabel_first;
         d["relabel_passes_first"] = s.relabel_passes_first;
         d["build_blocks_refused"] = s.build_blocks_refused;
+        d["host_waits"] = s.host_waits;
         return d;
     }
     int64_t slab_plane_elems() { int64_t n = 0; check(mgc_slab_plane_elems(g_, &n), g_); return n; }
diff --git a/medpy_b200/csrc/gc_slab.cu b/medpy_b200/csrc/gc_slab.cu
--- a/medpy_b200/csrc/gc_slab.cu
+++ b/medpy_b200/csrc/gc_slab.cu
@@ -251,7 +251,7 @@
 {
     if (!g || !energy_part) return MGC_E_ARG;
     CK(cudaSetDevice(g->device));
-    int rc = readout(g, energy_part);
+    int rc = readout(g, energy_part, true);
     if (rc) return rc;
     g->energy = *energy_part;
     g->st.energy = g->energy;
@@ -309,7 +309,7 @@
     g->ph_used = 0; g->ph_kind.clear();
     auto timed_sync = [&]() -> cudaError_t {
         const auto t0 = std::chrono::steady_clock::now();
-        const cudaError_t e = cudaStreamSynchronize(g->stream);
+        const cudaError_t e = wait_stream(g);
         g->slab_phase_ms[5] += std::chrono::duration<double, std::milli>(std::chrono::steady_clock::now() - t0).count();
         return e;
     };
diff --git a/medpy_b200/csrc/gc_solve.cu b/medpy_b200/csrc/gc_solve.cu
--- a/medpy_b200/csrc/gc_solve.cu
+++ b/medpy_b200/csrc/gc_solve.cu
@@ -95,12 +95,12 @@
     return MGC_OK;
 }
 
-int caps_launch(mgc_graph* g, WorkList wl)
+int caps_launch(mgc_graph* g, WorkList wl, bool zeroed)
 {
     if (g->caps_ev_used + 2 > g->caps_ev.size()) g->caps_ev.resize(g->caps_ev_used + 2, nullptr);
     for (size_t i = g->caps_ev_used; i < g->caps_ev_used + 2; ++i) if (!g->caps_ev[i]) CK(cudaEventCreate(&g->caps_ev[i]));
     CK(cudaEventRecord(g->caps_ev[g->caps_ev_used], g->stream));
-    CK(cudaMemsetAsync(g->d_flags + 4, 0, 2 * sizeof(int), g->stream));
+    if (!zeroed) CK(cudaMemsetAsync(g->d_flags + 4, 0, 2 * sizeof(int), g->stream));
     k_caps_claim<<<(unsigned)g->n_ctas * 4u, 256, 0, g->stream>>>(g->TL, g->cmat, wl, g->caps_list, g->d_flags + 4);
     int* count = g->d_flags + 4;
     int* done = g->d_flags + 3;
@@ -126,7 +126,8 @@
 double caps_resolve(mgc_graph* g)
 {
     double total = 0.0;
-    if (g->caps_ev_used && cudaEventSynchronize(g->caps_ev[g->caps_ev_used - 1]) == cudaSuccess) {
+    const cudaEvent_t last = g->caps_ev_used ? g->caps_ev[g->caps_ev_used - 1] : nullptr;
+    if (last && (cudaEventQuery(last) == cudaSuccess || wait_event(g, last) == cudaSuccess)) {
         for (size_t i = 0; i + 1 < g->caps_ev_used; i += 2) {
             float ms = 0;
             if (cudaEventElapsedTime(&ms, g->caps_ev[i], g->caps_ev[i + 1]) == cudaSuccess) total += ms;
@@ -141,7 +142,7 @@
 int read_tcount(mgc_graph* g, int idx, int* out)
 {
     CK(cudaMemcpyAsync(out, g->d_tcount + idx, sizeof(int), cudaMemcpyDeviceToHost, g->stream));
-    CK(cudaStreamSynchronize(g->stream));
+    CK(wait_stream(g));
     return MGC_OK;
 }
 }
@@ -161,6 +162,7 @@
     { int rc0 = push_state_all(g); if (rc0) return rc0; }
     CK(cudaMemsetAsync(g->d_tcount, 0, 256, g->stream));
     g->pl_sel[0] = g->pl_sel[1] = 0;
+    g->tcount_host = false;
     const bool warm = warm_wanted(g);
     cudaEventRecord(g->ev[4], g->stream);
     if (g->nd == 4) {
@@ -196,6 +198,7 @@
         CK(cudaMemsetAsync(g->d_tcount + CTL_RLCUR, 0, sizeof(int), g->stream));
         return MGC_OK;
     }
+    g->tcount_host = false;
     CK(cudaMemsetAsync(g->d_tcount, 0, 2 * sizeof(int), g->stream));
     CK(cudaMemsetAsync(g->rflag, 0, (size_t)g->TL.ntiles * sizeof(int), g->stream));
     if (g->nd == 4) {
@@ -261,7 +264,10 @@
     g->relp_pending = false;
     if (g->use_sweeps && g->TL.ntiles >= 64 && g->sweep_mode != 0) {
         int pending = 0;
-        int rc = read_tcount(g, 0, &pending);
+        int rc = MGC_OK;
+        if (g->tcount_host && !g->bad_pending) pending = ((volatile int*)g->h_bad)[5];
+        else rc = read_tcount(g, 0, &pending);
+        g->tcount_host = false;
         if (rc) return rc;
         if (g->sweep_mode < 0) g->sweep_mode = pending > g->TL.ntiles / g->sweep_frac ? 1 : 0;
         if (pending > g->TL.ntiles / g->sweep_frac) {
@@ -296,7 +302,7 @@
     if (want_any) {
         int relp = 0;
         CK(cudaMemcpyAsync(&relp, g->d_tcount + CTL_RELP, sizeof(int), cudaMemcpyDeviceToHost, g->stream));
-        CK(cudaStreamSynchronize(g->stream));
+        CK(wait_stream(g));
         if (relp != 0) *any = 1;
         g->relp_last = relp;
         g->st.relabel_passes += relp;
@@ -307,12 +313,12 @@
 }
 
 namespace {
-int relabel_passes_fetch(mgc_graph* g, bool* enqueued)
+int relabel_passes_fetch(mgc_graph* g, bool* enqueued, int slot = 4)
 {
     *enqueued = false;
     if (!g->relp_pending) return MGC_OK;
     if (!g->h_bad) { g->relp_pending = false; return MGC_OK; }
-    CK(cudaMemcpyAsync(g->h_bad + 4, g->d_tcount + CTL_RELP, sizeof(int), cudaMemcpyDeviceToHost, g->stream));
+    CK(cudaMemcpyAsync(g->h_bad + slot, g->d_tcount + CTL_RELP, sizeof(int), cudaMemcpyDeviceToHost, g->stream));
     *enqueued = true;
     return MGC_OK;
 }
@@ -333,11 +339,14 @@
 {
     const WorkList cur = pl(g, color, a);
     *now = WorkList{g->win_items, g->win_ctl + WIN_NOW};
-    CK(cudaMemsetAsync(g->win_ctl + WIN_GMIN, 0x7f, sizeof(int), g->stream));
-    CK(cudaMemsetAsync(g->win_ctl + WIN_NOW, 0, sizeof(int), g->stream));
-    k_window_min<double><<<g->n_ctas * 2, TILE_VOX, 0, g->stream>>>(g->L, g->TL, g->S, lazy_cmat(g), g->caps_tin, cur, g->win_tmin, g->win_ctl);
+    const int gslot = g->win_gslot;
+    const WinResets r{cursor(g), g->d_flags + 4, g->win_stale};
+    k_window_min<double><<<g->n_ctas * 2, TILE_VOX, 0, g->stream>>>(g->L, g->TL, g->S, lazy_cmat(g), g->caps_tin, cur, g->win_tmin,
+                                                                    g->win_ctl, gslot, r);
     k_window_split<<<g->n_ctas, 256, 0, g->stream>>>(cur, g->win_tmin, lazy_cmat(g), g->pflag, *now, pl(g, color, 1 - a),
-                                                     g->drop_items, g->win_ctl, g->labels_capped ? 1 : 0);
+                                                     g->drop_items, g->win_ctl, gslot, g->labels_capped ? 1 : 0);
+    g->win_gslot = gslot == WIN_GMIN ? WIN_GMIN2 : WIN_GMIN;
+    g->win_stale = cur.count;
     g->st.kernel_launches += 2;
     CK(cudaGetLastError());
     return MGC_OK;
@@ -348,15 +357,16 @@
     g->flow_started = true;
     const int a = g->pl_sel[color], oa = g->pl_sel[1 - color];
     WorkList cur = pl(g, color, a);
-    if (g->sweep_mode == 0 && g->nd == 3 && !g->slab) {
+    const bool window = g->sweep_mode == 0 && g->nd == 3 && !g->slab;
+    if (window) {
         const int rc = window_filter(g, color, a, &cur);
         if (rc) return rc;
     }
     if (g->caps_lazy) {
-        const int rc = g->sweep_mode == 1 ? push_state_all(g) : caps_launch(g, cur);
+        const int rc = g->sweep_mode == 1 ? push_state_all(g) : caps_launch(g, cur, window);
         if (rc) return rc;
     }
-    CK(cudaMemsetAsync(cursor(g), 0, sizeof(int), g->stream));
+    if (!window) CK(cudaMemsetAsync(cursor(g), 0, sizeof(int), g->stream));
     const int capped = g->labels_capped ? 1 : 0;
     if (g->nd == 4) {
         k_push_tile4<double><<<g->n_ctas, T4_VOX, 0, g->stream>>>(g->L, g->TL4, g->S, g->smask, g->iters_now, g->pflag, cur,
@@ -369,7 +379,7 @@
     } else
     k_push_tile<double><<<g->n_ctas, TILE_VOX, 0, g->stream>>>(g->L, g->TL, g->S, g->iters_now, g->pflag, cur,
                                                                cursor(g), pl(g, color, 1 - a), pl(g, 1 - color, oa), capped);
-    CK(cudaMemsetAsync(g->d_tcount + 2 + color * 2 + a, 0, sizeof(int), g->stream));
+    if (!window) CK(cudaMemsetAsync(g->d_tcount + 2 + color * 2 + a, 0, sizeof(int), g->stream));
     g->pl_sel[color] = 1 - a;
     g->st.kernel_launches++;
     return MGC_OK;
@@ -397,7 +407,7 @@
     if (rc) return rc;
     if (g->slab) return MGC_OK;
     cudaEventRecord(g->ev[3], g->stream);
-    CK(cudaEventSynchronize(g->ev[3]));
+    CK(wait_event(g, g->ev[3]));
     { float ms = 0; cudaEventElapsedTime(&ms, g->ev[2], g->ev[3]); g->st.ms_push += (double)ms - caps_resolve(g); }
     return MGC_OK;
 }
@@ -424,7 +434,7 @@
     if (rc) return rc;
     unsigned long long c = 0;
     CK(cudaMemcpyAsync(&c, g->d_count, sizeof(c), cudaMemcpyDeviceToHost, g->stream));
-    CK(cudaStreamSynchronize(g->stream));
+    CK(wait_stream(g));
     *out = (int64_t)c;
     g->st.active_last = (int64_t)c;
     return MGC_OK;
@@ -441,7 +451,7 @@
     else            k_debug_invariants<4, double, false><<<nblocks(g), 256, 0, g->stream>>>(g->L, g->S, d);
     double h[3] = {0, 0, 0};
     CK(cudaMemcpyAsync(h, d, sizeof(h), cudaMemcpyDeviceToHost, g->stream));
-    CK(cudaStreamSynchronize(g->stream));
+    CK(wait_stream(g));
     if (h[2] != 0.0) {
         g->err = "debug check: " + std::to_string((long long)h[2]) + " invariant violation(s) (negative capacity / excess, absorbed flow out of range or stale residual mask)";
         return MGC_E_STATE;
@@ -465,15 +475,24 @@
         rc = init_tiles(g);
         if (rc) return rc;
     }
-    if (g->win_ctl) CK(cudaMemsetAsync(g->win_ctl + WIN_DEFERRED, 0, 2 * sizeof(int), g->stream));
+    if (g->win_ctl) {
+        CK(cudaMemsetAsync(g->win_ctl + WIN_DEFERRED, 0, 2 * sizeof(int), g->stream));
+        CK(cudaMemsetAsync(g->win_ctl + WIN_GMIN, 0x7f, sizeof(int), g->stream));
+        g->win_gslot = WIN_GMIN;
+        g->win_stale = nullptr;
+    }
     int passes = g->passes0;
     int64_t rounds = 0;
     bool push_open = false;
     int passes_done = 0;
     unsigned long long active_fallback = 0;
     unsigned long long* h_active = g->h_bad ? (unsigned long long*)g->h_bad + 1 : &active_fallback;
+    bool first_open = false;
+    bool first_relp = false;
     for (;;) {
-        cudaEventRecord(g->ev[2], g->stream);
+        const bool test = rounds > 0 || !g->skip_first_test;
+        const bool defer = !test && !push_open && !g->init_timed;
+        cudaEventRecord(g->ev[defer ? 6 : 2], g->stream);
         {
             Nvtx range("mgc:global_relabel");
             rc = relabel_tiles_begin(g);
@@ -482,45 +501,61 @@
             rc = relabel_tiles_run(g, &any, false, rounds == 0 && g->skip_first_test);
             if (rc) return rc;
         }
-        cudaEventRecord(g->ev[3], g->stream);
+        cudaEventRecord(g->ev[defer ? 7 : 3], g->stream);
         g->st.global_relabels++;
         bool relp_copy = false;
-        rc = relabel_passes_fetch(g, &relp_copy);
+        rc = relabel_passes_fetch(g, &relp_copy, defer ? 6 : 4);
         if (rc) return rc;
-        const bool test = rounds > 0 || !g->skip_first_test;
-        if (test) {
-            rc = count_active_tiles_enqueue(g, g->d_count);
-            if (rc) return rc;
-            CK(cudaMemcpyAsync(h_active, g->d_count, sizeof(unsigned long long), cudaMemcpyDeviceToHost, g->stream));
-        }
-        CK(cudaEventSynchronize(g->ev[3]));
-        if (test || relp_copy) CK(cudaStreamSynchronize(g->stream));
-        float ms = 0;
-        const double caps_ms = caps_resolve(g);
-        if (g->init_timed) {
-            if (cudaEventElapsedTime(&ms, g->ev[4], g->ev[5]) == cudaSuccess) g->st.ms_init = ms;
-            g->init_timed = false;
-        }
-        cudaEventElapsedTime(&ms, g->ev[2], g->ev[3]);
-        const double t_rel = ms;
-        g->st.ms_relabel += ms;
-        const int relp = relabel_passes_collect(g);
-        if (rounds == 0) { g->st.ms_relabel_first += ms; g->st.relabel_passes_first += relp; }
-        double t_pass = 0.0;
-        if (push_open) {
-            cudaEventElapsedTime(&ms, g->ev[4], g->ev[5]);
-            const double push_ms = (double)ms - caps_ms;
-            g->st.ms_push += push_ms;
-            t_pass = push_ms / (passes_done > 0 ? passes_done : 1);
-            push_open = false;
-            int want = t_pass > 1e-4 ? (int)(t_rel / t_pass + 0.999) : passes * 2;
-            if (want < 1) want = 1;
-            if (want > passes * 2) want = passes * 2;
-            passes = want > g->passes_max ? g->passes_max : want;
-        }
-        if (test) {
-            g->st.active_last = (int64_t)*h_active;
-            if (*h_active == 0ull) break;
+        if (defer) {
+            first_open = true;
+            first_relp = relp_copy;
+            g->relp_pending = false;
+        } else {
+            if (test) {
+                rc = count_active_tiles_enqueue(g, g->d_count);
+                if (rc) return rc;
+                CK(cudaMemcpyAsync(h_active, g->d_count, sizeof(unsigned long long), cudaMemcpyDeviceToHost, g->stream));
+            }
+            if (test || relp_copy) CK(wait_stream(g));
+            else CK(wait_event(g, g->ev[3]));
+            float ms = 0;
+            const double caps_ms = caps_resolve(g);
+            if (g->init_timed) {
+                if (cudaEventElapsedTime(&ms, g->ev[4], g->ev[5]) == cudaSuccess) g->st.ms_init = ms;
+                g->init_timed = false;
+            }
+            if (first_open) {
+                cudaEventElapsedTime(&ms, g->ev[6], g->ev[7]);
+                g->st.ms_relabel += ms;
+                g->st.ms_relabel_first += ms;
+                if (first_relp) {
+                    const int p = ((volatile int*)g->h_bad)[6];
+                    g->st.relabel_passes += p;
+                    g->st.relabel_passes_first += p;
+                }
+                first_open = false;
+            }
+            cudaEventElapsedTime(&ms, g->ev[2], g->ev[3]);
+            const double t_rel = ms;
+            g->st.ms_relabel += ms;
+            const int relp = relabel_passes_collect(g);
+            if (rounds == 0) { g->st.ms_relabel_first += ms; g->st.relabel_passes_first += relp; }
+            double t_pass = 0.0;
+            if (push_open) {
+                cudaEventElapsedTime(&ms, g->ev[4], g->ev[5]);
+                const double push_ms = (double)ms - caps_ms;
+                g->st.ms_push += push_ms;
+                t_pass = push_ms / (passes_done > 0 ? passes_done : 1);
+                push_open = false;
+                int want = t_pass > 1e-4 ? (int)(t_rel / t_pass + 0.999) : passes * 2;
+                if (want < 1) want = 1;
+                if (want > passes * 2) want = passes * 2;
+                passes = want > g->passes_max ? g->passes_max : want;
+            }
+            if (test) {
+                g->st.active_last = (int64_t)*h_active;
+                if (*h_active == 0ull) break;
+            }
         }
         if (++rounds > g->max_rounds) FAIL(MGC_E_NOCONV, "push-relabel did not converge within the round cap");
         g->iters_now = rounds == 1 ? g->tile_iters_first : g->tile_iters;
@@ -539,24 +574,53 @@
 }
 }
 
-int readout(mgc_graph* g, double* energy_part)
+namespace {
+template <int OUT>
+void readout_launch(mgc_graph* g, uint8_t* mask)
+{
+    const bool clean = g->nd == 3 && !g->slab && g->TL.dflag && g->sweep_mode != 1 && g->L.dim[2] % 4 == 0;
+    if (clean) k_readout<double, true, true, OUT><<<rblocks(g), 256, 0, g->stream>>>(g->L, g->S, mask, g->partials, g->TL.dflag,
+                                                                                     g->TL.nt[1], g->TL.nt[2]);
+    else if (g->nd == 3) k_readout<double, true, false, OUT><<<rblocks(g), 256, 0, g->stream>>>(g->L, g->S, mask, g->partials);
+    else                 k_readout<double, false, false, OUT><<<rblocks(g), 256, 0, g->stream>>>(g->L, g->S, mask, g->partials);
+    g->st.kernel_launches++;
+}
+}
+
+int mask_launch(mgc_graph* g, uint8_t* dst)
+{
+    Nvtx range("mgc:mask");
+    readout_launch<READOUT_MASK>(g, dst);
+    CK(cudaGetLastError());
+    return MGC_OK;
+}
+
+int mask_produce(mgc_graph* g)
+{
+    if (g->mask_ready) return MGC_OK;
+    int rc = mask_launch(g, g->mask_dev);
+    if (rc) return rc;
+    g->mask_ready = true;
+    return MGC_OK;
+}
+
+int readout(mgc_graph* g, double* energy_part, bool with_mask)
 {
     Nvtx range("mgc:readout");
-    const bool clean = g->nd == 3 && !g->slab && g->TL.dflag && g->sweep_mode != 1 && g->L.dim[2] % 4 == 0;
-    if (clean) k_readout<double, true, true><<<rblocks(g), 256, 0, g->stream>>>(g->L, g->S, g->mask_dev, g->partials, g->TL.dflag,
-                                                                                g->TL.nt[1], g->TL.nt[2]);
-    else if (g->nd == 3) k_readout<double, true><<<rblocks(g), 256, 0, g->stream>>>(g->L, g->S, g->mask_dev, g->partials);
-    else                 k_readout<double, false><<<rblocks(g), 256, 0, g->stream>>>(g->L, g->S, g->mask_dev, g->partials);
+    if (with_mask) readout_launch<READOUT_MASK | READOUT_ENERGY>(g, g->mask_dev);
+    else           readout_launch<READOUT_ENERGY>(g, nullptr);
+    g->mask_ready = with_mask;
     CK(cudaMemsetAsync(g->d_scalars + 1, 0, sizeof(double), g->stream));
     sum_partials(g, g->partials, rblocks(g), g->d_scalars + 1);
-    g->st.kernel_launches += 2;
+    g->st.kernel_launches++;
     double sc[2] = {0, 0};
     int fl[5] = {0, 0, 0, 0, 0};
     int win[2] = {0, 0};
     CK(cudaMemcpyAsync(sc, g->d_scalars, sizeof(sc), cudaMemcpyDeviceToHost, g->stream));
     CK(cudaMemcpyAsync(fl, g->d_flags + 3, sizeof(fl), cudaMemcpyDeviceToHost, g->stream));
     if (g->win_ctl) CK(cudaMemcpyAsync(win, g->win_ctl + WIN_DEFERRED, sizeof(win), cudaMemcpyDeviceToHost, g->stream));
-    CK(cudaStreamSynchronize(g->stream));
+    CK(cudaEventRecord(g->ev[8], g->stream));
+    CK(wait_stream(g));
     g->st.flow_const = sc[0];
     g->st.tiles_materialised = fl[0];
     g->st.build_blocks_refused = fl[4];
@@ -571,22 +635,6 @@
     return MGC_OK;
 }
 
-namespace {
-struct Timer {
-    mgc_graph* g;
-    double* acc;
-    Timer(mgc_graph* g_, double* acc_) : g(g_), acc(acc_) { cudaEventRecord(g->ev[0], g->stream); }
-    void stop_sync()
-    {
-        cudaEventRecord(g->ev[1], g->stream);
-        cudaEventSynchronize(g->ev[1]);
-        float ms = 0;
-        cudaEventElapsedTime(&ms, g->ev[0], g->ev[1]);
-        *acc += ms;
-    }
-};
-}
-
 extern "C" {
 
 int mgc_maxflow(mgc_graph* g, double* energy)
@@ -597,29 +645,26 @@
     if (g->solved) { if (energy) *energy = g->energy; return MGC_OK; }
     { int rc0 = check_pending(g); if (rc0) return rc0; }
     resolve_term_span(g);
-    {
-        Timer t(g, &g->st.ms_solve);
-        int rc = warm_prepare(g); if (rc) return rc;
-        if (g->debug_checks) {
-            rc = materialise_zeros(g); if (rc) return rc;
-            if (!g->state_init) { rc = init_tiles(g); if (rc) return rc; }
-            rc = debug_invariants(g, false); if (rc) return rc;
-        }
-        rc = solve_tiles(g);
-        if (rc) return rc;
-        rc = debug_invariants(g, true);
-        if (rc) return rc;
-        t.stop_sync();
-    }
-    {
-        Timer t(g, &g->st.ms_readout);
-        double e = 0.0;
-        int rc = readout(g, &e);
-        if (rc) return rc;
-        g->energy = e;
-        g->st.energy = e;
-        t.stop_sync();
-    }
+    cudaEventRecord(g->ev[0], g->stream);
+    int rc = warm_prepare(g); if (rc) return rc;
+    if (g->debug_checks) {
+        rc = materialise_zeros(g); if (rc) return rc;
+        if (!g->state_init) { rc = init_tiles(g); if (rc) return rc; }
+        rc = debug_invariants(g, false); if (rc) return rc;
+    }
+    rc = solve_tiles(g);
+    if (rc) return rc;
+    rc = debug_invariants(g, true);
+    if (rc) return rc;
+    cudaEventRecord(g->ev[1], g->stream);
+    double e = 0.0;
+    rc = readout(g, &e, false);
+    if (rc) return rc;
+    float ms = 0;
+    if (cudaEventElapsedTime(&ms, g->ev[0], g->ev[1]) == cudaSuccess) g->st.ms_solve += ms;
+    if (cudaEventElapsedTime(&ms, g->ev[1], g->ev[8]) == cudaSuccess) g->st.ms_readout += ms;
+    g->energy = e;
+    g->st.energy = e;
     caps_resolve(g);
     g->solved = true;
     if (energy) *energy = g->energy;
diff --git a/medpy_b200/csrc/gc_solve_kernels.cuh b/medpy_b200/csrc/gc_solve_kernels.cuh
--- a/medpy_b200/csrc/gc_solve_kernels.cuh
+++ b/medpy_b200/csrc/gc_solve_kernels.cuh
@@ -206,11 +206,26 @@
 }
 
 
+struct WinResets {
+    int* cursor;
+    int* caps;
+    int* stale;
+};
+
 template <typename T>
 __global__ void __launch_bounds__(TILE_VOX) k_window_min(Lattice L, Tiles TL, State<T> S, const int* __restrict__ cmat, LazyTin tin,
-                                                         WorkList cur, int* __restrict__ tmin, int* __restrict__ ctl)
+                                                         WorkList cur, int* __restrict__ tmin, int* __restrict__ ctl, int gslot,
+                                                         WinResets r)
 {
     __shared__ int s_min[TILE_VOX / 32];
+    if (blockIdx.x == 0 && threadIdx.x == 0) {
+        ctl[WIN_NOW] = 0;
+        ctl[gslot == WIN_GMIN ? WIN_GMIN2 : WIN_GMIN] = 0x7f7f7f7f;
+        *r.cursor = 0;
+        r.caps[0] = 0;
+        r.caps[1] = 0;
+        if (r.stale) *r.stale = 0;
+    }
     const int n = *cur.count;
     for (int i = blockIdx.x; i < n; i += gridDim.x) {
         const int t = cur.items[i];
@@ -226,7 +241,7 @@
             m = __reduce_min_sync(0xffffffffu, m);
             if (threadIdx.x == 0) {
                 tmin[i] = m;
-                if (m < MGC_HINF) atomicMin(ctl + WIN_GMIN, m);
+                if (m < MGC_HINF) atomicMin(ctl + gslot, m);
             }
         }
         __syncthreads();
@@ -246,10 +261,10 @@
 
 __global__ void __launch_bounds__(256) k_window_split(WorkList cur, const int* __restrict__ tmin, const int* __restrict__ cmat,
                                                       int* __restrict__ pflag, WorkList now, WorkList later,
-                                                      int* __restrict__ drop_items, int* __restrict__ ctl, int labels_capped)
+                                                      int* __restrict__ drop_items, int* __restrict__ ctl, int gslot, int labels_capped)
 {
     const int n = *cur.count;
-    const int gmin = ctl[WIN_GMIN];
+    const int gmin = ctl[gslot];
     const int lane = threadIdx.x & 31;
     for (int base = (blockIdx.x * blockDim.x + threadIdx.x) & ~31; base < n; base += gridDim.x * blockDim.x) {
         const int i = base + lane;
diff --git a/medpy_b200/csrc/gc_solver.cuh b/medpy_b200/csrc/gc_solver.cuh
--- a/medpy_b200/csrc/gc_solver.cuh
+++ b/medpy_b200/csrc/gc_solver.cuh
@@ -1,69 +1,89 @@
 #pragma once
 #include "gc_common.cuh"
 
-template <typename T, bool LAZY, bool CLEAN = false>
+#define READOUT_MASK 1
+#define READOUT_ENERGY 2
+template <typename T, bool LAZY, bool CLEAN = false, int OUT = READOUT_MASK | READOUT_ENERGY>
 __global__ void __launch_bounds__(256) k_readout(Lattice L, State<T> S, uint8_t* __restrict__ mask, double* __restrict__ partials,
                                                  const int* __restrict__ dflag = nullptr, int nty = 0, int ntx = 0)
 {
+    constexpr bool MASK = (OUT & READOUT_MASK) != 0, ENERGY = (OUT & READOUT_ENERGY) != 0;
     __shared__ double sh[8];
     double a = 0.0;
     const unsigned step = gridDim.x * blockDim.x;
     const unsigned n4 = L.n >> 2;
-    for (unsigned q = blockIdx.x * blockDim.x + threadIdx.x; q < n4; q += step) {
-        const unsigned v = q << 2;
-        uchar4 m;
-        unsigned rm = 0;
-        bool clean = false;
-        if (CLEAN) {
-            rm = reinterpret_cast<const unsigned*>(S.rmask)[q];
-            const unsigned gz = div_stride(L, v, 0), r = v - gz * L.stride[0];
-            const unsigned gy = div_stride(L, r, 1), gx = r - gy * L.stride[1];
-            clean = dflag[((int)(gz >> 3) * nty + (int)(gy >> 3)) * ntx + (int)(gx >> 3)] == 0;
+    constexpr bool READ_RM = LAZY ? ENERGY || (MASK && CLEAN) : (MASK && CLEAN);
+    constexpr unsigned RU = READ_RM ? 4u : 1u;
+    for (unsigned q0 = blockIdx.x * blockDim.x + threadIdx.x; q0 < n4; q0 += RU * step) {
+        unsigned rmv[RU];
+#pragma unroll
+        for (unsigned u = 0; u < RU; ++u) {
+            const unsigned qu = q0 + u * step;
+            rmv[u] = (READ_RM && qu < n4) ? reinterpret_cast<const unsigned*>(S.rmask)[qu] : 0u;
         }
-        if (clean) {
-            const bool own = owned(L, v);
-            m.x = (own && (rm & 0x40u)) ? 0 : 1; m.y = (own && ((rm >> 8) & 0x40u)) ? 0 : 1;
-            m.z = (own && ((rm >> 16) & 0x40u)) ? 0 : 1; m.w = (own && ((rm >> 24) & 0x40u)) ? 0 : 1;
-        } else {
-            const int4 h = reinterpret_cast<const int4*>(S.height)[q];
-            m.x = h.x >= MGC_HINF ? 1 : 0; m.y = h.y >= MGC_HINF ? 1 : 0;
-            m.z = h.z >= MGC_HINF ? 1 : 0; m.w = h.w >= MGC_HINF ? 1 : 0;
-        }
-        reinterpret_cast<uchar4*>(mask)[q] = m;
-        if (LAZY) {
-            const unsigned r4 = (CLEAN ? rm : reinterpret_cast<const unsigned*>(S.rmask)[q]) & 0x80808080u;
-            if (r4) {
 #pragma unroll
-                for (int i = 0; i < 4; ++i)
-                    if ((r4 >> (8 * i + 7)) & 1u) { if (owned(L, v + i)) a = __dadd_rn(a, (double)S.sink[v + i]); }
+        for (unsigned u = 0; u < RU; ++u) {
+            const unsigned q = q0 + u * step;
+            if (q >= n4) break;
+            const unsigned v = q << 2;
+            const unsigned rm = rmv[u];
+            if (MASK) {
+                uchar4 m;
+                bool clean = false;
+                if (CLEAN) {
+                    const unsigned gz = div_stride(L, v, 0), r = v - gz * L.stride[0];
+                    const unsigned gy = div_stride(L, r, 1), gx = r - gy * L.stride[1];
+                    clean = dflag[((int)(gz >> 3) * nty + (int)(gy >> 3)) * ntx + (int)(gx >> 3)] == 0;
+                }
+                if (clean) {
+                    const bool own = owned(L, v);
+                    m.x = (own && (rm & 0x40u)) ? 0 : 1; m.y = (own && ((rm >> 8) & 0x40u)) ? 0 : 1;
+                    m.z = (own && ((rm >> 16) & 0x40u)) ? 0 : 1; m.w = (own && ((rm >> 24) & 0x40u)) ? 0 : 1;
+                } else {
+                    const int4 h = reinterpret_cast<const int4*>(S.height)[q];
+                    m.x = h.x >= MGC_HINF ? 1 : 0; m.y = h.y >= MGC_HINF ? 1 : 0;
+                    m.z = h.z >= MGC_HINF ? 1 : 0; m.w = h.w >= MGC_HINF ? 1 : 0;
+                }
+                reinterpret_cast<uchar4*>(mask)[q] = m;
             }
-        } else if (sizeof(T) == 8) {
-            const double2 s0 = reinterpret_cast<const double2*>(S.sink)[2 * q];
-            const double2 s1 = reinterpret_cast<const double2*>(S.sink)[2 * q + 1];
-            if (owned(L, v)) a = __dadd_rn(a, s0.x);
-            if (owned(L, v + 1)) a = __dadd_rn(a, s0.y);
-            if (owned(L, v + 2)) a = __dadd_rn(a, s1.x);
-            if (owned(L, v + 3)) a = __dadd_rn(a, s1.y);
-        } else {
+            if (!ENERGY) continue;
+            if (LAZY) {
+                const unsigned r4 = rm & 0x80808080u;
+                if (r4) {
 #pragma unroll
-            for (int i = 0; i < 4; ++i) if (owned(L, v + i)) a = __dadd_rn(a, (double)S.sink[v + i]);
+                    for (int i = 0; i < 4; ++i)
+                        if ((r4 >> (8 * i + 7)) & 1u) { if (owned(L, v + i)) a = __dadd_rn(a, (double)S.sink[v + i]); }
+                }
+            } else if (sizeof(T) == 8) {
+                const double2 s0 = reinterpret_cast<const double2*>(S.sink)[2 * q];
+                const double2 s1 = reinterpret_cast<const double2*>(S.sink)[2 * q + 1];
+                if (owned(L, v)) a = __dadd_rn(a, s0.x);
+                if (owned(L, v + 1)) a = __dadd_rn(a, s0.y);
+                if (owned(L, v + 2)) a = __dadd_rn(a, s1.x);
+                if (owned(L, v + 3)) a = __dadd_rn(a, s1.y);
+            } else {
+#pragma unroll
+                for (int i = 0; i < 4; ++i) if (owned(L, v + i)) a = __dadd_rn(a, (double)S.sink[v + i]);
+            }
         }
     }
     if (blockIdx.x == 0 && threadIdx.x < (L.n & 3u)) {
         const unsigned v = (n4 << 2) + threadIdx.x;
-        mask[v] = S.height[v] >= MGC_HINF ? 1 : 0;
-        if (owned(L, v) && (!LAZY || (S.rmask[v] & 0x80u))) a = __dadd_rn(a, (double)S.sink[v]);
+        if (MASK) mask[v] = S.height[v] >= MGC_HINF ? 1 : 0;
+        if (ENERGY && owned(L, v) && (!LAZY || (S.rmask[v] & 0x80u))) a = __dadd_rn(a, (double)S.sink[v]);
     }
+    if constexpr (ENERGY) {
 #pragma unroll
-    for (int o = 16; o > 0; o >>= 1) a = __dadd_rn(a, __shfl_down_sync(0xffffffffu, a, o));
-    const unsigned tid = threadIdx.x;
-    if ((tid & 31) == 0) sh[tid >> 5] = a;
-    __syncthreads();
-    if (tid == 0) {
-        double t = sh[0];
+        for (int o = 16; o > 0; o >>= 1) a = __dadd_rn(a, __shfl_down_sync(0xffffffffu, a, o));
+        const unsigned tid = threadIdx.x;
+        if ((tid & 31) == 0) sh[tid >> 5] = a;
+        __syncthreads();
+        if (tid == 0) {
+            double t = sh[0];
 #pragma unroll
-        for (int w = 1; w < 8; ++w) t = __dadd_rn(t, sh[w]);
-        partials[blockIdx.x] = t;
+            for (int w = 1; w < 8; ++w) t = __dadd_rn(t, sh[w]);
+            partials[blockIdx.x] = t;
+        }
     }
 }
 
```

Result: faster. 45260 (median of 6 runs) (+4.4%).
